# zuds-survey/zuds-pipeline

Hardware: AMD Instinct MI355X
Metric: Mpix/s resample->coadd->subtract, 3072x3072 frames (higher is better)
Workload: dtype f32; 1 GPU; configs[1]+[2]: 32x 3072x3072 TPV frames/GPU, mesh background + weight rescale + Lanczos-3 resample + WEIGHTED coadd (+ AND mask coadd, int16 masks); then 1 science frame/GPU: align ref, hotpants 3x3 regions x 10x10 stamps, r=10, ko=4, subtract; frames_per_gpu=32, size=3072, mask_dtype=int16, combine=WEIGHTED, subtract=True

## Files before the change

### include/zudsmi.h

```cpp
#ifndef ZUDSMI_H
#define ZUDSMI_H

#include <stdint.h>

#ifdef __cplusplus
extern "C" {
#endif

typedef struct zm_ctx zm_ctx;

#define ZM_NPV 40

typedef struct zm_wcs {
    double crpix[2];
    double crval[2];
    double cd[4];
    double pv1[ZM_NPV];
    double pv2[ZM_NPV];
    int32_t naxis[2];
    int32_t flags;
    int32_t pad_;
} zm_wcs;

enum { ZM_RESAMPLE_NEAREST = 0, ZM_RESAMPLE_BILINEAR = 1, ZM_RESAMPLE_LANCZOS3 = 3 };
// ... 130 lines not shown
int zm_aperture_photometry_dev(zm_ctx* ctx, const float* img, const float* rms,
                               const int32_t* mask, int nx, int ny, int npos,
                               const double* x, const double* y, double radius,
                               double* out_flux, double* out_err, int32_t* out_flags);

typedef struct zm_dframe {
    const float* img;
    const float* wgt;
    const void* mask;
    zm_wcs wcs;
    double flxscale;
    int32_t mask_type;
    int32_t pad_;
} zm_dframe;

int zm_coadd_dev(zm_ctx* ctx, int nframes, const zm_dframe* frames,
                 const zm_wcs* wout, const zm_coadd_params* params,
                 int partial, float* out_img, float* out_wgt, int32_t* out_mask,
                 float* out_mask_wgt);
int zm_coadd_finalize_dev(zm_ctx* ctx, float* s1_to_img, const float* s0,
                          int64_t npix);
int zm_mask_accum_dev(zm_ctx* ctx, int32_t* acc, const int32_t* m, int64_t npix,
                      int kind, int first);
int zm_mask_finalize_dev(zm_ctx* ctx, int32_t* acc, float* cov, int64_t npix);
#define ZM_COMM_ID_BYTES 128
typedef struct zm_comm zm_comm;
int zm_comm_unique_id(void* id128);
int zm_comm_init(zm_ctx* ctx, int nranks, int rank, const void* id128, zm_comm** out);
int zm_comm_destroy(zm_comm* comm);
int zm_coadd_reduce_dev(zm_ctx* ctx, zm_comm* comm, float* s1s0, int64_t npix);
int zm_mask_reduce_dev(zm_ctx* ctx, zm_comm* comm, int32_t* mask, int nx, int ny, int kind,
                       float* cov);
#define ZM_COMM_MAX_RANKS 64
typedef struct {
    int32_t world, rank;
    int64_t band_px;
    int64_t my_px;
    int64_t send_off[ZM_COMM_MAX_RANKS];
    int64_t send_cnt[ZM_COMM_MAX_RANKS];
    int64_t recv_off[ZM_COMM_MAX_RANKS];
    int64_t recv_cnt[ZM_COMM_MAX_RANKS];
    int64_t gather_off[ZM_COMM_MAX_RANKS];
} zm_mask_plan;
int zm_comm_band_bounds(int nrows, int world, int32_t* bounds);
int zm_comm_mask_plan(int nx, int ny, int world, int rank, zm_mask_plan* plan);
int zm_resample_stack_dev(zm_ctx* ctx, int nframes, const zm_dframe* frames,
                          const zm_wcs* wout, const zm_coadd_params* params,
                          float* stack, int32_t* out_mask_partial);
int zm_combine_stack_dev(zm_ctx* ctx, int nframes, const float* stack,
                         int64_t frame_stride_px, int64_t npix,
                         const zm_coadd_params* params, float* out_img,
                         float* out_wgt);
int zm_subtract_dev(zm_ctx* ctx, const float* sci, const float* sci_rms,
                    const float* ref, const float* ref_rms, const uint8_t* bpm,
                    int nx, int ny, const zm_hp_params* params, float* out_diff,
                    float* out_rms, zm_hp_info* out_info_host);
int zm_subtract_info(zm_ctx* ctx, zm_hp_info* out_info);
#define ZM_SUB_BATCH_MAX 64
typedef struct zm_sub_job {
    const float* sci;
    const float* sci_rms;
    const float* ref;
    const float* ref_rms;
    const uint8_t* bpm;
    const zm_hp_params* params;
    float* out_diff;
    float* out_rms;
} zm_sub_job;
int zm_subtract_batch_dev(zm_ctx* ctx, int njobs, const zm_sub_job* jobs, int nx, int ny,
                          zm_hp_info* out_info_host);
int zm_subtract_batch(zm_ctx* ctx, int njobs, const zm_sub_job* jobs, int nx, int ny,
                      zm_hp_info* out_info);
int zm_background_dev(zm_ctx* ctx, const float* img, const float* wgt, int nx,
                      int ny, int mesh, int filtersize, float* out_bkg,
                      float* out_rms, float* out_sub, double* out_stats_host);
int zm_resample_dev(zm_ctx* ctx, const float* img, const float* wgt,
                    const int32_t* mask, const zm_wcs* win, const zm_wcs* wout,
                    int kernel, double fscale, float* out_img, float* out_wgt,
                    int32_t* out_mask);

int zm_align_pair_dev(zm_ctx* ctx, const float* img_a, const float* img_b, const int32_t* mask,
                      const zm_wcs* win, const zm_wcs* wout, int kernel, double fscale_a, double fscale_b,
                      float* out_a, float* out_b, int32_t* out_mask);
int zm_resample_i16(zm_ctx* ctx, const float* img, const float* wgt,
                    const int16_t* mask, const zm_wcs* win, const zm_wcs* wout,
                    int kernel, double fscale, float* out_img, float* out_wgt,
                    int32_t* out_mask);
int zm_resample_i16_dev(zm_ctx* ctx, const float* img, const float* wgt,
                        const int16_t* mask, const zm_wcs* win, const zm_wcs* wout,
                        int kernel, double fscale, float* out_img, float* out_wgt,
                        int32_t* out_mask);
int zm_mask_widen_dev(zm_ctx* ctx, const int16_t* in, int64_t n, int32_t* out);

int zm_rms_from_weight_dev(zm_ctx* ctx, const float* wgt, const uint8_t* bad,
                           int64_t n, float big_rms, float* out);
int zm_weight_from_rms_dev(zm_ctx* ctx, const float* rms, const uint8_t* bad,
                           const float* img, float satur, int64_t n, float* out);
int zm_false_weight_dev(zm_ctx* ctx, const void* mask, int mask_type, int32_t badsum, int border,
                        int nx, int ny, float* out_wgt, uint8_t* out_bpm);
int zm_mask_bad_dev(zm_ctx* ctx, const int32_t* a, const int32_t* b,
                    int32_t badsum, int64_t n, int32_t* out_or, uint8_t* out_bpm);
int zm_mask_flag_dev(zm_ctx* ctx, int32_t* mask, const float* img, float value,
                     int32_t bit, int64_t n);
int zm_add_scalar_dev(zm_ctx* ctx, float* img, float v, int64_t n);
int zm_copy_probe_dev(zm_ctx* ctx, const void* src, void* dst, int64_t nbytes);

int zm_find_stars(zm_ctx* ctx, const float* img, const uint8_t* bad, int nx, int ny,
                  float thresh_lo, float thresh_hi, int isolation, int border,
                  int max_out, int* out_x, int* out_y, float* out_peak, int* out_n);
int zm_star_fwhm(zm_ctx* ctx, const float* img, int nx, int ny, int nstar,
                 const int* x, const int* y, int half, double* out_fwhm,
                 double* out_cx, double* out_cy);
int zm_negpix_test(zm_ctx* ctx, const float* img, int nx, int ny, int npos,
                   const double* x, const double* y, double median, double sigma,
                   int32_t* out_bad);
int zm_find_stars_dev(zm_ctx* ctx, const float* img, const uint8_t* bad, int nx, int ny,
                      float thresh_lo, float thresh_hi, int isolation, int border,
                      int max_out, int* out_x, int* out_y, float* out_peak, int* out_n);
int zm_star_fwhm_dev(zm_ctx* ctx, const float* img, int nx, int ny, int nstar,
                     const int* x, const int* y, int half, double* out_fwhm,
                     double* out_cx, double* out_cy);
int zm_candidate_cuts_dev(zm_ctx* ctx, const float* d_img, const float* d_rms, const int32_t* d_mask,
                          int32_t bad_bits, int nx, int ny, int npos, const double* x, const double* y,
                          double* out_bpmcut, double* out_rmscut, int32_t* out_negpix, double* out_stats);

typedef struct zm_extract_params {
    float detect_thresh;
    float satur_level;
    int32_t detect_minarea;
    int32_t filter;
    double aper_radius;
} zm_extract_params;
void zm_extract_params_default(zm_extract_params* p);

#define ZM_EXTRACT_CHAIN 1

typedef struct zm_object {
    int32_t number;
    int32_t npix;
    int32_t xmin, xmax, ymin, ymax;
    int32_t flags;
    int32_t flags_weight;
    int32_t imaflags_iso;
    int32_t first;
    int32_t nthresh;
    int32_t pad_;
    double x_image, y_image;
    double x2, y2, xy;
    double a_image, b_image, theta_image, elongation;
    double fwhm_image;
    double flux_iso, flux_max;
    double peak;
    double flux_aper, fluxerr_aper;
    double x_world, y_world;
} zm_object;

int zm_extract_dev(zm_ctx* ctx, const float* img, const float* sigma, const uint8_t* bad,
                   const int32_t* flag, int nx, int ny, const zm_wcs* wcs,
                   const zm_extract_params* params, int max_objects, zm_object* out_rows,
                   int32_t* segm_dev, float* filtered_dev, int* out_nwritten, int* out_nfound,
                   int* out_status);
int zm_extract(zm_ctx* ctx, const float* img, const float* sigma, const uint8_t* bad,
               const int32_t* flag, int nx, int ny, const zm_wcs* wcs,
               const zm_extract_params* params, int max_objects, zm_object* out_rows,
               int32_t* out_segm, float* out_filtered, int* out_nwritten, int* out_nfound,
               int* out_status);
// ... 113 lines not shown
```

### zuds-pipeline_amd/_lib.py

```python
import ctypes as C
from pathlib import Path

import numpy as np

HERE = Path(__file__).resolve().parent
LIBPATH = HERE / 'lib' / 'libzudsmi.so'

NPV = 40

RESAMPLE = {'NEAREST': 0, 'BILINEAR': 1, 'LANCZOS3': 3}
COMBINE = {'WEIGHTED': 0, 'MEDIAN': 1, 'CLIPPED': 2, 'AVERAGE': 3}
MASKCOMB = {'AND': 0, 'OR': 1}


class ZMError(RuntimeError):
    """A libzudsmi call returned non-zero (message from zm_last_error)."""


class zm_wcs(C.Structure):
    _fields_ = [('crpix', C.c_double * 2), ('crval', C.c_double * 2),
                ('cd', C.c_double * 4), ('pv1', C.c_double * NPV),
                ('pv2', C.c_double * NPV), ('naxis', C.c_int32 * 2),
                ('flags', C.c_int32), ('pad_', C.c_int32)]

# ... 61 lines not shown


class zm_extract_params(C.Structure):
    _fields_ = [('detect_thresh', C.c_float), ('satur_level', C.c_float),
                ('detect_minarea', C.c_int32), ('filter', C.c_int32),
                ('aper_radius', C.c_double)]


class zm_object(C.Structure):
    _fields_ = [('number', C.c_int32), ('npix', C.c_int32), ('xmin', C.c_int32), ('xmax', C.c_int32),
                ('ymin', C.c_int32), ('ymax', C.c_int32), ('flags', C.c_int32), ('flags_weight', C.c_int32),
                ('imaflags_iso', C.c_int32), ('first', C.c_int32), ('nthresh', C.c_int32), ('pad_', C.c_int32),
                ('x_image', C.c_double), ('y_image', C.c_double), ('x2', C.c_double), ('y2', C.c_double),
                ('xy', C.c_double), ('a_image', C.c_double), ('b_image', C.c_double), ('theta_image', C.c_double),
                ('elongation', C.c_double), ('fwhm_image', C.c_double), ('flux_iso', C.c_double),
                ('flux_max', C.c_double), ('peak', C.c_double), ('flux_aper', C.c_double),
                ('fluxerr_aper', C.c_double), ('x_world', C.c_double), ('y_world', C.c_double)]


class zm_measure_params(C.Structure):
    _fields_ = [('kron_fact', C.c_double), ('kron_min_radius', C.c_double), ('filter', C.c_int32), ('pad_', C.c_int32)]


class zm_object_ext(C.Structure):
    _fields_ = [('number', C.c_int32), ('npix_auto', C.c_int32), ('nskip_auto', C.c_int32), ('flags_auto', C.c_int32),
                ('flags_win', C.c_int32), ('niter_win', C.c_int32),
                ('kron_radius', C.c_double), ('flux_auto', C.c_double), ('fluxerr_auto', C.c_double),
                ('mag_auto', C.c_double), ('magerr_auto', C.c_double), ('sigma_win', C.c_double),
                ('xwin_image', C.c_double), ('ywin_image', C.c_double),
                ('x2win', C.c_double), ('y2win', C.c_double), ('xywin', C.c_double),
                ('errx2win', C.c_double), ('erry2win', C.c_double), ('errxywin', C.c_double),
                ('awin_image', C.c_double), ('bwin_image', C.c_double), ('thetawin_image', C.c_double),
                ('errawin_image', C.c_double), ('errbwin_image', C.c_double), ('errthetawin_image', C.c_double),
                ('errx2', C.c_double), ('erry2', C.c_double), ('errxy', C.c_double),
                ('xwin_world', C.c_double), ('ywin_world', C.c_double),
                ('erra_world', C.c_double), ('errb_world', C.c_double), ('errtheta_world', C.c_double)]


class zm_stamp_plane(C.Structure):
    _fields_ = [('img', C.c_void_p), ('wcs', zm_wcs), ('fscale', C.c_double),
                ('on_grid', C.c_int32), ('pad_', C.c_int32)]


class zm_rb_layer(C.Structure):
    _fields_ = [('type', C.c_int32), ('activation', C.c_int32), ('cin', C.c_int32), ('cout', C.c_int32),
                ('pool', C.c_int32), ('ksize', C.c_int32), ('stride', C.c_int32), ('padding', C.c_int32),
                ('w_off', C.c_int64), ('b_off', C.c_int64)]


RB_CHUNK = 128
RB_CONV2D, RB_MAXPOOL, RB_FLATTEN, RB_DENSE = 1, 2, 3, 4
RB_ACTIVATION = {'linear': 0, 'relu': 1, 'sigmoid': 2}
RB_VALID, RB_SAME = 0, 1
STAMP_MAX, STAMP_PLANES_MAX = 256, 8
STAMP_NOT_FINITE, STAMP_NO_OVERLAP = 1, 2
EXTRACT_CHAIN = 1
HP_UNSOLVED, HP_TIMEOUT, HP_PENDING = 1, 2, 4


_P = C.c_void_p
_SIGS = {
    'zm_ctx_create': (C.c_int, [C.c_int, C.POINTER(_P)]),
    'zm_ctx_destroy': (C.c_int, [_P]),
    'zm_ctx_set_stream': (C.c_int, [_P, _P]),
    'zm_ctx_synchronize': (C.c_int, [_P]),
    'zm_ctx_create_on_stream': (C.c_int, [C.c_int, _P, C.POINTER(C.c_void_p)]),
    'zm_ctx_set_share': (C.c_int, [_P, C.c_int]),
    'zm_ctx_query': (C.c_int, [_P, C.c_char_p, C.POINTER(C.c_int64)]),
    'zm_ctx_set_conventions': (C.c_int, [_P, C.c_int, C.c_int]),
    'zm_last_error': (C.c_char_p, []),
    'zm_version': (C.c_char_p, []),
    'zm_autogrid': (C.c_int, [C.c_int, C.POINTER(zm_wcs), C.POINTER(zm_wcs)]),
    'zm_wcs_pix2sky': (C.c_int, [C.POINTER(zm_wcs), C.c_int, _P, _P, _P, _P]),
    'zm_wcs_sky2pix': (C.c_int, [C.POINTER(zm_wcs), C.c_int, _P, _P, _P, _P]),
    'zm_wcs_map': (C.c_int, [C.POINTER(zm_wcs), C.POINTER(zm_wcs), C.c_int,
                             _P, _P, _P, _P]),
    'zm_flux_scale': (C.c_int, [C.POINTER(zm_wcs), C.POINTER(zm_wcs),
                                C.c_double, C.POINTER(C.c_double)]),
    'zm_resample': (C.c_int, [_P, _P, _P, _P, C.POINTER(zm_wcs),
                              C.POINTER(zm_wcs), C.c_int, C.c_double,
                              _P, _P, _P]),
    'zm_align_pair_dev': (C.c_int, [_P, _P, _P, _P, C.POINTER(zm_wcs), C.POINTER(zm_wcs), C.c_int, C.c_double,
                                    C.c_double, _P, _P, _P]),
    'zm_resample_dev': (C.c_int, [_P, _P, _P, _P, C.POINTER(zm_wcs),
                                  C.POINTER(zm_wcs), C.c_int, C.c_double,
                                  _P, _P, _P]),
    'zm_resample_i16': (C.c_int, [_P, _P, _P, _P, C.POINTER(zm_wcs),
                                  C.POINTER(zm_wcs), C.c_int, C.c_double,
                                  _P, _P, _P]),
    'zm_resample_i16_dev': (C.c_int, [_P, _P, _P, _P, C.POINTER(zm_wcs),
                                      C.POINTER(zm_wcs), C.c_int, C.c_double,
                                      _P, _P, _P]),
    'zm_mask_widen_dev': (C.c_int, [_P, _P, C.c_int64, _P]),
    'zm_coadd_params_default': (None, [C.POINTER(zm_coadd_params)]),
    'zm_coadd': (C.c_int, [_P, C.c_int, C.POINTER(zm_frame), C.POINTER(zm_wcs),
                           C.POINTER(zm_coadd_params), _P, _P, _P, _P]),
    'zm_coadd_dev': (C.c_int, [_P, C.c_int, C.POINTER(zm_frame),
                               C.POINTER(zm_wcs), C.POINTER(zm_coadd_params),
                               C.c_int, _P, _P, _P, _P]),
    'zm_coadd_finalize_dev': (C.c_int, [_P, _P, _P, C.c_int64]),
    'zm_resample_stack_dev': (C.c_int, [_P, C.c_int, C.POINTER(zm_frame),
                                        C.POINTER(zm_wcs),
                                        C.POINTER(zm_coadd_params), _P, _P]),
    'zm_combine_stack_dev': (C.c_int, [_P, C.c_int, _P, C.c_int64, C.c_int64,
                                       C.POINTER(zm_coadd_params), _P, _P]),
    'zm_background': (C.c_int, [_P, _P, _P, C.c_int, C.c_int, C.c_int, C.c_int,
                                _P, _P, _P, _P]),
    'zm_background_dev': (C.c_int, [_P, _P, _P, C.c_int, C.c_int, C.c_int,
                                    C.c_int, _P, _P, _P, _P]),
    'zm_hp_params_default': (None, [C.POINTER(zm_hp_params)]),
    'zm_subtract': (C.c_int, [_P, _P, _P, _P, _P, _P, C.c_int, C.c_int,
                              C.POINTER(zm_hp_params), _P, _P,
                              C.POINTER(zm_hp_info)]),
    'zm_subtract_dev': (C.c_int, [_P, _P, _P, _P, _P, _P, C.c_int, C.c_int,
                                  C.POINTER(zm_hp_params), _P, _P,
                                  C.POINTER(zm_hp_info)]),
    'zm_subtract_info': (C.c_int, [_P, C.POINTER(zm_hp_info)]),
    'zm_subtract_batch_dev': (C.c_int, [_P, C.c_int, C.POINTER(zm_sub_job), C.c_int, C.c_int,
                                        C.POINTER(zm_hp_info)]),
    'zm_subtract_batch': (C.c_int, [_P, C.c_int, C.POINTER(zm_sub_job), C.c_int, C.c_int,
                                    C.POINTER(zm_hp_info)]),
    'zm_median_mad': (C.c_int, [_P, _P, _P, C.c_int64, C.POINTER(C.c_double),
                                C.POINTER(C.c_double)]),
    'zm_median_mad_dev': (C.c_int, [_P, _P, _P, C.c_int64, C.POINTER(C.c_double),
                                    C.POINTER(C.c_double)]),
    'zm_find_stars': (C.c_int, [_P, _P, _P, C.c_int, C.c_int, C.c_float, C.c_float, C.c_int, C.c_int,
                                C.c_int, _P, _P, _P, C.POINTER(C.c_int)]),
    'zm_star_fwhm': (C.c_int, [_P, _P, C.c_int, C.c_int, C.c_int, _P, _P, C.c_int, _P, _P, _P]),
    'zm_find_stars_dev': (C.c_int, [_P, _P, _P, C.c_int, C.c_int, C.c_float, C.c_float, C.c_int, C.c_int,
                                    C.c_int, _P, _P, _P, C.POINTER(C.c_int)]),
    'zm_star_fwhm_dev': (C.c_int, [_P, _P, C.c_int, C.c_int, C.c_int, _P, _P, C.c_int, _P, _P, _P]),
    'zm_negpix_test': (C.c_int, [_P, _P, C.c_int, C.c_int, C.c_int, _P, _P, C.c_double, C.c_double, _P]),
    'zm_candidate_cuts_dev': (C.c_int, [_P, _P, _P, _P, C.c_int32, C.c_int, C.c_int, C.c_int, _P, _P, _P, _P, _P, _P]),
    'zm_fits_decode_dev': (C.c_int, [_P, _P, C.c_int, C.c_double, C.c_double, C.c_int64, C.c_int, _P]),
    'zm_fits_encode_dev': (C.c_int, [_P, _P, C.c_int, C.c_int64, _P]),
    'zm_mask_accum_dev': (C.c_int, [_P, _P, _P, C.c_int64, C.c_int, C.c_int]),
    'zm_mask_finalize_dev': (C.c_int, [_P, _P, _P, C.c_int64]),
    'zm_comm_unique_id': (C.c_int, [_P]),
    'zm_comm_init': (C.c_int, [_P, C.c_int, C.c_int, _P, C.POINTER(C.c_void_p)]),
    'zm_comm_destroy': (C.c_int, [_P]),
    'zm_coadd_reduce_dev': (C.c_int, [_P, _P, _P, C.c_int64]),
    'zm_mask_reduce_dev': (C.c_int, [_P, _P, _P, C.c_int, C.c_int, C.c_int, _P]),
    'zm_comm_band_bounds': (C.c_int, [C.c_int, C.c_int, _P]),
    'zm_comm_mask_plan': (C.c_int, [C.c_int, C.c_int, C.c_int, C.c_int, C.POINTER(zm_mask_plan)]),
    'zm_median_mad2_dev': (C.c_int, [_P, _P, _P, _P, _P, C.c_int64, C.POINTER(C.c_double)]),
    'zm_median_mad2_async_dev': (C.c_int, [_P, _P, _P, _P, _P, C.c_int64, _P]),
    'zm_rms_from_weight_dev': (C.c_int, [_P, _P, _P, C.c_int64, C.c_float, _P]),
    'zm_weight_from_rms_dev': (C.c_int, [_P, _P, _P, _P, C.c_float, C.c_int64, _P]),
    'zm_false_weight_dev': (C.c_int, [_P, _P, C.c_int, C.c_int32, C.c_int, C.c_int, C.c_int, _P, _P]),
    'zm_mask_bad_dev': (C.c_int, [_P, _P, _P, C.c_int32, C.c_int64, _P, _P]),
    'zm_mask_flag_dev': (C.c_int, [_P, _P, _P, C.c_float, C.c_int32, C.c_int64]),
    'zm_add_scalar_dev': (C.c_int, [_P, _P, C.c_float, C.c_int64]),
    'zm_copy_probe_dev': (C.c_int, [_P, _P, _P, C.c_int64]),
    'zm_aperture_photometry': (C.c_int, [_P, _P, _P, _P, C.c_int, C.c_int, C.c_int, _P, _P,
                                         C.c_double, _P, _P, _P]),
    'zm_aperture_photometry_dev': (C.c_int, [_P, _P, _P, _P, C.c_int, C.c_int, C.c_int, _P, _P,
                                             C.c_double, _P, _P, _P]),
    'zm_extract_params_default': (None, [C.POINTER(zm_extract_params)]),
    'zm_extract_dev': (C.c_int, [_P, _P, _P, _P, _P, C.c_int, C.c_int, C.POINTER(zm_wcs), C.POINTER(zm_extract_params),
                                 C.c_int, _P, _P, _P, C.POINTER(C.c_int), C.POINTER(C.c_int), C.POINTER(C.c_int)]),
    'zm_extract': (C.c_int, [_P, _P, _P, _P, _P, C.c_int, C.c_int, C.POINTER(zm_wcs), C.POINTER(zm_extract_params),
                             C.c_int, _P, _P, _P, C.POINTER(C.c_int), C.POINTER(C.c_int), C.POINTER(C.c_int)]),
    'zm_measure_params_default': (None, [C.POINTER(zm_measure_params)]),
    'zm_extract_measure_dev': (C.c_int, [_P, _P, _P, _P, _P, C.c_int, C.c_int, C.POINTER(zm_wcs),
                                         C.POINTER(zm_measure_params), C.c_int, _P, _P]),
    'zm_extract_measure': (C.c_int, [_P, _P, _P, _P, _P, C.c_int, C.c_int, C.POINTER(zm_wcs),
                                     C.POINTER(zm_measure_params), C.c_int, _P, _P]),
    'zm_stamp_origin': (C.c_int, [C.POINTER(zm_wcs), C.c_int, _P, _P, C.c_int, _P, _P, _P]),
    'zm_stamps_dev': (C.c_int, [_P, C.c_int, C.POINTER(zm_stamp_plane), C.POINTER(zm_wcs), C.c_int, C.c_int, _P, _P,
                                C.c_int, _P, _P]),
    'zm_stamps': (C.c_int, [_P, C.c_int, C.POINTER(zm_stamp_plane), C.POINTER(zm_wcs), C.c_int, C.c_int, _P, _P,
                            C.c_int, _P, _P]),
    'zm_rb_model_create': (C.c_int, [_P, C.c_int, C.c_int, C.c_int, C.POINTER(zm_rb_layer), _P, C.c_int64, C.POINTER(C.c_void_p)]),
    'zm_rb_model_destroy': (C.c_int, [_P]),
    'zm_rb_score_dev': (C.c_int, [_P, _P, C.c_int, _P, _P, C.c_int, _P, _P]),
    'zm_rb_score': (C.c_int, [_P, _P, C.c_int, _P, _P, C.c_int, _P, _P]),
    'zm_associate_dev': (C.c_int, [_P, C.c_int, _P, _P, _P, _P, C.c_double, _P, _P, _P, _P, _P, _P, _P]),
    'zm_associate': (C.c_int, [_P, C.c_int, _P, _P, _P, _P, C.c_double, _P, _P, _P, _P, _P, _P, _P]),
    'zm_crossmatch_dev': (C.c_int, [_P, C.c_int, _P, _P, C.c_int, _P, _P, C.c_double, _P, _P]),
    'zm_crossmatch': (C.c_int, [_P, C.c_int, _P, _P, C.c_int, _P, _P, C.c_double, _P, _P]),
    'zm_assoc_stats': (C.c_int, [_P, _P]),
    'zm_timing_enable': (C.c_int, [_P, C.c_int]),
    'zm_timing_filter': (C.c_int, [_P, C.c_char_p]),
    'zm_timing_reset': (C.c_int, [_P]),
    'zm_timing_read': (C.c_int, [_P, C.c_char_p, C.POINTER(C.c_double),
                                 C.POINTER(C.c_int64)]),
    'zm_debug_lanczos3': (None, [C.c_float, _P]),
}

_lib = None


def exported_symbols():
    return [k for k in _SIGS if k != 'zm_debug_lanczos3']


def _one_hip_runtime():
    import importlib.util
    import os
    import sys
    if 'torch' in sys.modules:
        return
    try:
        spec = importlib.util.find_spec('torch')
    except (ImportError, ValueError):
        spec = None
    if not spec or not spec.origin:
        return
    if not os.environ.get('ZM_NO_TORCH'):
        try:
            import torch
            return
        except Exception:
            pass
    d = os.path.join(os.path.dirname(spec.origin), 'lib')
    for name in ('libhsa-runtime64.so', 'libamdhip64.so'):
        p = os.path.join(d, name)
        if os.path.exists(p):
            try:
                C.CDLL(p, mode=C.RTLD_GLOBAL)
            except OSError:
                return


def lib():
    global _lib
    if _lib is not None:
        return _lib
    _one_hip_runtime()
    if not LIBPATH.exists():
        raise ZMError(f'{LIBPATH} is missing: run __graft_entry__.build() '
                      f'(python zuds-pipeline_amd/build.py). There is no CPU '
                      f'fallback for this path.')
    L = C.CDLL(str(LIBPATH))
    for name, (res, args) in _SIGS.items():
        try:
            fn = getattr(L, name)
        except AttributeError:
            raise ZMError(f'{LIBPATH} does not export {name}; rebuild it '
                          f'(python zuds-pipeline_amd/build.py --force)')
        fn.restype = res
        fn.argtypes = args
    _lib = L
    return L


def check(rc, what=''):
    if rc != 0:
        msg = lib().zm_last_error().decode('utf-8', 'replace')
        raise ZMError(f'{what}: {msg} (rc={rc})' if what else f'{msg} (rc={rc})')


def ptr(a):
    if a is None:
        return None
    if isinstance(a, int):
        return a
    return a.ctypes.data


def as_f32(a):
    return None if a is None else np.ascontiguousarray(a, dtype=np.float32)


def as_i32(a):
    return None if a is None else np.ascontiguousarray(a, dtype=np.int32)


def as_mask(a):
    if a is None:
        return None, MASKTYPE_I32
    a = np.asarray(a)
    if a.dtype == np.int16:
        return np.ascontiguousarray(a), MASKTYPE_I16
    return np.ascontiguousarray(a, dtype=np.int32), MASKTYPE_I32


# ... 19 lines not shown
```

### zuds-pipeline_amd/csrc/api_coadd.hip

```cpp
#include <algorithm>
#include <cmath>
#include <cstdlib>

#include "zm_internal.h"
#include "wcs_math.h"

extern "C" void zm_coadd_params_default(zm_coadd_params* p) {
    if (!p) return;
    memset(p, 0, sizeof(*p));
    p->combine = ZM_COMBINE_CLIPPED;
    p->mask_combine = ZM_MASK_AND;
    p->resample = ZM_RESAMPLE_LANCZOS3;
    p->subtract_back = 1;
    p->back_size = 128;
    p->back_filtersize = 3;
    p->rescale_weights = 1;
    p->clip_sigma = 4.0;
    p->clip_ampfrac = 0.3;
    p->weight_thresh = 1e-30;
}

static int check_wcs(const zm_wcs* w, const char* what) {
    ZM_CHECK(w != nullptr, "%s: WCS is NULL", what);
    ZM_CHECK(w->naxis[0] > 0 && w->naxis[1] > 0, "%s: NAXIS must be positive (got %d x %d)", what,
// ... 372 lines not shown
                                    const zm_coadd_params* params, float* out_img,
                                    float* out_wgt) {
    ZM_CHECK(ctx && stack && params && out_img && out_wgt, "zm_combine_stack_dev: null argument");
    ZM_HIP(hipSetDevice(ctx->device));
    return zm_launch_combine(ctx, nframes, (const float2*)stack, frame_stride_px, npix,
                             params->combine, (float)params->clip_sigma,
                             (float)params->clip_ampfrac, out_img, out_wgt, 0);
}

extern "C" int zm_coadd_dev(zm_ctx* ctx, int nframes, const zm_dframe* frames,
                            const zm_wcs* wout, const zm_coadd_params* params, int partial,
                            float* out_img, float* out_wgt, int32_t* out_mask,
                            float* out_mask_wgt) {
    ZM_CHECK(ctx && frames && wout && params && out_img && out_wgt, "zm_coadd_dev: null argument");
    ZM_CHECK(nframes >= 1, "zm_coadd_dev: need at least one frame");
    ZM_HIP(hipSetDevice(ctx->device));
    ZM_TRY(check_wcs(wout, "output grid"));
    const int64_t opix = (int64_t)wout->naxis[0] * wout->naxis[1];
    if (fused_ok(ctx, params))
        return coadd_fused(ctx, nframes, frames, wout, params, partial, out_img, out_wgt, out_mask, out_mask_wgt);
    float2* stack = nullptr;
    ZM_TRY(ctx->get("stack", sizeof(float2) * (size_t)opix * nframes, (void**)&stack));
    ZM_TRY(resample_frames(ctx, nframes, frames, wout, params, stack, out_mask, -1,
                           params->mask_combine));
    ZM_TRY(zm_launch_combine(ctx, nframes, stack, opix, opix, params->combine,
                             (float)params->clip_sigma, (float)params->clip_ampfrac, out_img,
                             out_wgt, partial));
    if (out_mask && !partial) ZM_TRY(zm_launch_mask_finalize(ctx, out_mask, out_mask_wgt, opix));
    return 0;
}

extern "C" int zm_mask_accum_dev(zm_ctx* ctx, int32_t* acc, const int32_t* m, int64_t npix, int kind,
                                 int first) {
    ZM_CHECK(ctx && acc && m, "zm_mask_accum_dev: null argument");
    ZM_CHECK(kind == ZM_MASK_AND || kind == ZM_MASK_OR, "zm_mask_accum_dev: unknown combine %d", kind);
    ZM_HIP(hipSetDevice(ctx->device));
    return zm_launch_mask_accum(ctx, acc, m, npix, kind, first);
}

extern "C" int zm_mask_finalize_dev(zm_ctx* ctx, int32_t* acc, float* cov, int64_t npix) {
    ZM_CHECK(ctx && acc, "zm_mask_finalize_dev: null argument");
    ZM_HIP(hipSetDevice(ctx->device));
    return zm_launch_mask_finalize(ctx, acc, cov, npix);
}

extern "C" int zm_resample_dev(zm_ctx* ctx, const float* img, const float* wgt,
                               const int32_t* mask, const zm_wcs* win, const zm_wcs* wout,
                               int kernel, double fscale, float* out_img, float* out_wgt,
                               int32_t* out_mask) {
    ZM_CHECK(ctx && win && wout, "zm_resample_dev: null argument");
    ZM_CHECK(img || mask, "zm_resample_dev: need an image or a mask");
    ZM_CHECK(!img || (out_img && out_wgt), "zm_resample_dev: out_img/out_wgt required");
    ZM_CHECK(!mask || out_mask, "zm_resample_dev: out_mask required");
    ZM_HIP(hipSetDevice(ctx->device));
    ZM_TRY(check_wcs(win, "input frame"));
    ZM_TRY(check_wcs(wout, "output grid"));
    ZM_CHECK(kernel == ZM_RESAMPLE_LANCZOS3 || kernel == ZM_RESAMPLE_BILINEAR ||
             kernel == ZM_RESAMPLE_NEAREST, "zm_resample_dev: unknown RESAMPLING_TYPE %d", kernel);
    const int onx = wout->naxis[0], ony = wout->naxis[1];
    const int nx = win->naxis[0], ny = win->naxis[1];
    const int64_t opix = (int64_t)onx * ony;
    const int lnx = (onx - 1) / ZM_LATTICE_STEP + 2, lny = (ony - 1) / ZM_LATTICE_STEP + 2;
    zm_map_params mp_host;
    zm_make_map(wout, win, &mp_host);
    int lds = std::min(plan_lds(&mp_host, onx, ony, ntaps_of(kernel)), 8000);
    double2* lat = nullptr;
    ZM_TRY(ctx->get("lattice", sizeof(double2) * (size_t)lnx * lny, (void**)&lat));
    ZM_TRY(zm_launch_lattice(ctx, &mp_host, lnx, lny, lat));
    if (img) {
        const int spitch = (nx + 1) & ~1;
        float2 *src = nullptr, *dst = nullptr;
        ZM_TRY(ctx->get("prep", sizeof(float2) * (size_t)spitch * ny, (void**)&src));
        ZM_TRY(ctx->get("stack", sizeof(float2) * (size_t)opix, (void**)&dst));
        ZM_TRY(zm_launch_prep(ctx, img, wgt, nx, ny, nullptr, 0, 0, 0, nullptr, 1e-30f, src, spitch));
        ZM_TRY(zm_launch_resample(ctx, src, nx, ny, spitch, lat, lnx, lny, kernel, (float)fscale,
                                  dst, onx, ony, lds, mask, out_mask, mask ? 1 : 0, 0, 1, out_img, out_wgt));
    } else if (mask) {
        ZM_TRY(zm_launch_resample_mask(ctx, mask, nx, ny, lat, lnx, lny, kernel, out_mask, onx,
                                       ony, 0));
    }
    return 0;
}

extern "C" int zm_align_pair_dev(zm_ctx* ctx, const float* img_a, const float* img_b, const int32_t* mask,
                                 const zm_wcs* win, const zm_wcs* wout, int kernel, double fscale_a, double fscale_b,
                                 float* out_a, float* out_b, int32_t* out_mask) {
    ZM_CHECK(ctx && img_a && img_b && win && wout && out_a && out_b, "zm_align_pair_dev: null argument");
    ZM_CHECK(!mask || out_mask, "zm_align_pair_dev: out_mask required");
    ZM_CHECK(kernel == ZM_RESAMPLE_LANCZOS3 || kernel == ZM_RESAMPLE_BILINEAR, "zm_align_pair_dev: LANCZOS3 or BILINEAR (got %d)", kernel);
    ZM_CHECK(fscale_b != 0.0, "zm_align_pair_dev: fscale_b must not be 0");
    ZM_CHECK(ctx->edge == ZM_EDGE_ZERO && ctx->mask_resample == ZM_MASKRES_OR, "zm_align_pair_dev: default conventions only");
    ZM_HIP(hipSetDevice(ctx->device));
    ZM_TRY(check_wcs(win, "input frame"));
    ZM_TRY(check_wcs(wout, "output grid"));
    const int onx = wout->naxis[0], ony = wout->naxis[1];
    const int nx = win->naxis[0], ny = win->naxis[1];
    const int lnx = (onx - 1) / ZM_LATTICE_STEP + 2, lny = (ony - 1) / ZM_LATTICE_STEP + 2;
    zm_map_params mp_host;
    zm_make_map(wout, win, &mp_host);
    const int lds = std::min(plan_lds(&mp_host, onx, ony, ntaps_of(kernel)), 8000);
    double2* lat = nullptr;
    ZM_TRY(ctx->get("lattice", sizeof(double2) * (size_t)lnx * lny, (void**)&lat));
    ZM_TRY(zm_launch_lattice(ctx, &mp_host, lnx, lny, lat));
    const int spitch = (nx + 1) & ~1;
    float2* src = nullptr;
    ZM_TRY(ctx->get("prep", sizeof(float2) * (size_t)spitch * ny, (void**)&src));
    ZM_TRY(zm_launch_prep_pair(ctx, img_a, img_b, nx, ny, src, spitch));
    return zm_launch_resample(ctx, src, nx, ny, spitch, lat, lnx, lny, kernel, (float)fscale_a, nullptr, onx, ony, lds,
                              mask, out_mask, mask ? 1 : 0, 0, 1, out_a, out_b, (float)fscale_b);
}

extern "C" int zm_resample_i16_dev(zm_ctx* ctx, const float* img, const float* wgt, const int16_t* mask,
                                   const zm_wcs* win, const zm_wcs* wout, int kernel, double fscale,
                                   float* out_img, float* out_wgt, int32_t* out_mask) {
    ZM_CHECK(ctx && win && wout, "zm_resample_i16_dev: null argument");
    ZM_HIP(hipSetDevice(ctx->device));
    int32_t* w = nullptr;
    if (mask) {
        ZM_TRY(check_wcs(win, "input frame"));
        const int64_t n = (int64_t)win->naxis[0] * win->naxis[1];
        ZM_TRY(ctx->get("mask_widen", sizeof(int32_t) * (size_t)n, (void**)&w));
        ZM_TRY(zm_launch_mask_widen(ctx, mask, n, w));
    }
    return zm_resample_dev(ctx, img, wgt, w, win, wout, kernel, fscale, out_img, out_wgt, out_mask);
}

static int resample_host(zm_ctx* ctx, const float* img, const float* wgt, const void* mask, int mask_type,
                         const zm_wcs* win, const zm_wcs* wout, int kernel, double fscale,
                         float* out_img, float* out_wgt, int32_t* out_mask);
extern "C" int zm_resample(zm_ctx* ctx, const float* img, const float* wgt, const int32_t* mask,
                           const zm_wcs* win, const zm_wcs* wout, int kernel, double fscale,
                           float* out_img, float* out_wgt, int32_t* out_mask) {
    return resample_host(ctx, img, wgt, mask, ZM_MASKTYPE_I32, win, wout, kernel, fscale, out_img, out_wgt, out_mask);
}
extern "C" int zm_resample_i16(zm_ctx* ctx, const float* img, const float* wgt, const int16_t* mask,
                               const zm_wcs* win, const zm_wcs* wout, int kernel, double fscale,
                               float* out_img, float* out_wgt, int32_t* out_mask) {
    return resample_host(ctx, img, wgt, mask, ZM_MASKTYPE_I16, win, wout, kernel, fscale, out_img, out_wgt, out_mask);
}
static int resample_host(zm_ctx* ctx, const float* img, const float* wgt, const void* mask, int mask_type,
                         const zm_wcs* win, const zm_wcs* wout, int kernel, double fscale,
                         float* out_img, float* out_wgt, int32_t* out_mask) {
    ZM_CHECK(ctx && win && wout, "zm_resample: null argument");
    ZM_HIP(hipSetDevice(ctx->device));
    ZM_TRY(check_wcs(win, "input frame"));
    ZM_TRY(check_wcs(wout, "output grid"));
    const size_t ipix = (size_t)win->naxis[0] * win->naxis[1];
    const size_t opix = (size_t)wout->naxis[0] * wout->naxis[1];
    const size_t mb = mask_type == ZM_MASKTYPE_I16 ? 2 : 4;
    float *d_img = nullptr, *d_wgt = nullptr, *d_oimg = nullptr, *d_owgt = nullptr;
    void* d_mask = nullptr;
    int32_t* d_omask = nullptr;
    if (img) {
        ZM_TRY(ctx->get("h_img", ipix * 4, (void**)&d_img));
        ZM_HIP(hipMemcpyAsync(d_img, img, ipix * 4, hipMemcpyHostToDevice, ctx->stream));
        if (wgt) {
            ZM_TRY(ctx->get("h_wgt", ipix * 4, (void**)&d_wgt));
            ZM_HIP(hipMemcpyAsync(d_wgt, wgt, ipix * 4, hipMemcpyHostToDevice, ctx->stream));
        }
        ZM_TRY(ctx->get("h_oimg", opix * 4, (void**)&d_oimg));
        ZM_TRY(ctx->get("h_owgt", opix * 4, (void**)&d_owgt));
    }
    if (mask) {
        ZM_TRY(ctx->get("h_mask", ipix * mb, &d_mask));
        ZM_HIP(hipMemcpyAsync(d_mask, mask, ipix * mb, hipMemcpyHostToDevice, ctx->stream));
        ZM_TRY(ctx->get("h_omask", opix * 4, (void**)&d_omask));
    }
    if (mask_type == ZM_MASKTYPE_I16)
        ZM_TRY(zm_resample_i16_dev(ctx, d_img, d_wgt, (const int16_t*)d_mask, win, wout, kernel, fscale, d_oimg,
                                   d_owgt, d_omask));
    else
        ZM_TRY(zm_resample_dev(ctx, d_img, d_wgt, (const int32_t*)d_mask, win, wout, kernel, fscale, d_oimg, d_owgt,
                               d_omask));
    if (img) {
        ZM_HIP(hipMemcpyAsync(out_img, d_oimg, opix * 4, hipMemcpyDeviceToHost, ctx->stream));
        ZM_HIP(hipMemcpyAsync(out_wgt, d_owgt, opix * 4, hipMemcpyDeviceToHost, ctx->stream));
    }
    if (mask)
        ZM_HIP(hipMemcpyAsync(out_mask, d_omask, opix * 4, hipMemcpyDeviceToHost, ctx->stream));
    ZM_HIP(hipStreamSynchronize(ctx->stream));
    return 0;
}

extern "C" int zm_coadd(zm_ctx* ctx, int nframes, const zm_frame* frames, const zm_wcs* wout,
                        const zm_coadd_params* params, float* out_img, float* out_wgt,
                        int32_t* out_mask, float* out_mask_wgt) {
    ZM_CHECK(ctx && frames && wout && params && out_img && out_wgt, "zm_coadd: null argument");
    ZM_CHECK(nframes >= 1, "zm_coadd: need at least one frame");
    ZM_HIP(hipSetDevice(ctx->device));
    ZM_TRY(check_wcs(wout, "output grid"));
    std::vector<zm_dframe> df(nframes);
    size_t total = 0;
// ... 55 lines not shown
```

### zuds-pipeline_amd/csrc/ctx.hip

```cpp
#include <cstdarg>

#include "zm_internal.h"

static thread_local char g_err[1024] = "";

void zm_set_error(const char* fmt, ...) {
    va_list ap;
    va_start(ap, fmt);
    vsnprintf(g_err, sizeof(g_err), fmt, ap);
    va_end(ap);
}

extern "C" const char* zm_last_error(void) { return g_err; }
extern "C" const char* zm_version(void) { return "zudsmi 0.1.0 (gfx950)"; }

int zm_ctx::get(const char* name, size_t bytes, void** out) {
    auto it = scratch.find(name);
    if (it != scratch.end() && it->second.second >= bytes) {
        *out = it->second.first;
        return 0;
    }
    if (it != scratch.end()) {
        ZM_HIP(hipStreamSynchronize(stream));
        ZM_HIP(hipFree(it->second.first));
// ... 59 lines not shown
    ZM_HIP(hipSetDevice(device));
    zm_ctx* c = new zm_ctx();
    c->device = device;
    ZM_HIP(hipStreamCreateWithFlags(&c->stream, hipStreamNonBlocking));
    c->own_stream = true;
    *out = c;
    return 0;
}

extern "C" int zm_ctx_create_on_stream(int device, void* hip_stream, zm_ctx** out) {
    ZM_CHECK(out != nullptr && hip_stream != nullptr, "zm_ctx_create_on_stream: null argument");
    int ndev = 0;
    hipError_t e = hipGetDeviceCount(&ndev);
    if (e != hipSuccess || ndev == 0) {
        zm_set_error("zm_ctx_create_on_stream: no HIP device available (%s)",
                     e != hipSuccess ? hipGetErrorString(e) : "device count 0");
        return 3;
    }
    ZM_CHECK(device >= 0 && device < ndev, "zm_ctx_create_on_stream: device %d out of range [0,%d)", device, ndev);
    ZM_HIP(hipSetDevice(device));
    zm_ctx* c = new zm_ctx();
    c->device = device;
    c->stream = (hipStream_t)hip_stream;
    c->own_stream = false;
    *out = c;
    return 0;
}

extern "C" int zm_ctx_destroy(zm_ctx* ctx) {
    if (!ctx) return 0;
    (void)hipSetDevice(ctx->device);
    (void)hipStreamSynchronize(ctx->stream);
    ctx->release_all();
    if (ctx->aux) { (void)hipStreamSynchronize(ctx->aux); (void)hipStreamDestroy(ctx->aux); }
    if (ctx->own_stream && ctx->stream) (void)hipStreamDestroy(ctx->stream);
    delete ctx;
    return 0;
}

extern "C" int zm_ctx_set_stream(zm_ctx* ctx, void* hip_stream) {
    ZM_CHECK(ctx != nullptr, "zm_ctx_set_stream: ctx is NULL");
    ZM_HIP(hipSetDevice(ctx->device));
    if (ZM_DEVENV("ZM_SET_STREAM_SYNC")) ZM_HIP(hipStreamSynchronize(ctx->stream));
    if (hip_stream != nullptr && (hipStream_t)hip_stream == ctx->stream) return 0;
    if (hip_stream == nullptr && ctx->own_stream) return 0;
    hipStream_t old = ctx->stream, next = (hipStream_t)hip_stream;
    const bool old_owned = ctx->own_stream;
    if (next == nullptr) ZM_HIP(hipStreamCreateWithFlags(&next, hipStreamNonBlocking));
    if (old) {
        hipEvent_t* ev = nullptr;
        ZM_TRY(zm_get_sync_events(ctx, 11, &ev));
        ZM_HIP(hipEventRecord(ev[10], old));
        ZM_HIP(hipStreamWaitEvent(next, ev[10], 0));
    }
    if (old_owned && old) ZM_HIP(hipStreamDestroy(old));
    ctx->stream = next;
    ctx->own_stream = hip_stream == nullptr;
    return 0;
}

extern "C" int zm_ctx_set_share(zm_ctx* ctx, int nctx) {
    ZM_CHECK(ctx != nullptr, "zm_ctx_set_share: ctx is NULL");
    ZM_CHECK(nctx >= 1 && nctx <= 64, "zm_ctx_set_share: %d contexts (1 .. 64)", nctx);
    ctx->share = nctx;
    return 0;
}

extern "C" int zm_ctx_set_conventions(zm_ctx* ctx, int edge, int mask_resample) {
    ZM_CHECK(ctx != nullptr, "zm_ctx_set_conventions: ctx is NULL");
    ZM_CHECK(edge == ZM_EDGE_ZERO || edge == ZM_EDGE_TRUNCATE, "zm_ctx_set_conventions: unknown edge rule %d", edge);
    ZM_CHECK(mask_resample == ZM_MASKRES_OR || mask_resample == ZM_MASKRES_LANCZOS_ROUND,
             "zm_ctx_set_conventions: unknown mask rule %d", mask_resample);
    ctx->edge = edge;
    ctx->mask_resample = mask_resample;
    return 0;
}

extern "C" int zm_ctx_query(zm_ctx* ctx, const char* what, int64_t* out) {
    ZM_CHECK(ctx && what && out, "zm_ctx_query: null argument");
    if (!strcmp(what, "fused_form")) *out = ctx->ff_last_form;
    else if (!strcmp(what, "dev_build")) *out = ZM_DEV_BUILD;
    else if (!strcmp(what, "edge")) *out = ctx->edge;
    else if (!strcmp(what, "mask_resample")) *out = ctx->mask_resample;
    else ZM_CHECK(false, "zm_ctx_query: unknown item \"%s\"", what);
    return 0;
}

hipStream_t zm_ctx_aux(zm_ctx* ctx) {
    if (!ctx->aux) {
        (void)hipSetDevice(ctx->device);
        if (hipStreamCreateWithFlags(&ctx->aux, hipStreamNonBlocking) != hipSuccess) ctx->aux = nullptr;
    }
    return ctx->aux;
}

int zm_get_sync_events(zm_ctx* ctx, int n, hipEvent_t** out) {
    while ((int)ctx->sync_events.size() < n) {
        hipEvent_t e = nullptr;
        ZM_HIP(hipEventCreateWithFlags(&e, hipEventDisableTiming));
        ctx->sync_events.push_back(e);
    }
    *out = ctx->sync_events.data();
    return 0;
}

extern "C" int zm_ctx_synchronize(zm_ctx* ctx) {
    ZM_CHECK(ctx != nullptr, "zm_ctx_synchronize: ctx is NULL");
    ZM_HIP(hipSetDevice(ctx->device));
    ZM_HIP(hipStreamSynchronize(ctx->stream));
    return 0;
}

zm_scope_timer::zm_scope_timer(zm_ctx* c, const char* n) : ctx(c), name(n) {
    if (!ctx->timing) return;
    if (!ctx->timing_only.empty() && ctx->timing_only != n) return;
    auto take = [&]() -> hipEvent_t {
        if (!ctx->event_pool.empty()) {
            hipEvent_t e = ctx->event_pool.back();
            ctx->event_pool.pop_back();
            return e;
        }
        hipEvent_t e = nullptr;
        (void)hipEventCreate(&e);
        return e;
    };
    a = take();
    b = take();
    (void)hipEventRecord(a, ctx->stream);
}

zm_scope_timer::~zm_scope_timer() {
    if (!ctx->timing || !a) return;
    (void)hipEventRecord(b, ctx->stream);
    ctx->timers[name].pending.push_back({a, b});
}

extern "C" int zm_timing_enable(zm_ctx* ctx, int on) {
    ZM_CHECK(ctx != nullptr, "zm_timing_enable: ctx is NULL");
    ctx->timing = on != 0;
    return 0;
}

static int drain(zm_ctx* ctx, zm_timer_slot& s) {
    for (auto& p : s.pending) {
        ZM_HIP(hipEventSynchronize(p.second));
        float ms = 0.f;
        ZM_HIP(hipEventElapsedTime(&ms, p.first, p.second));
        s.total_ms += ms;
        s.launches += 1;
        ctx->event_pool.push_back(p.first);
        ctx->event_pool.push_back(p.second);
    }
    s.pending.clear();
    return 0;
}

extern "C" int zm_timing_filter(zm_ctx* ctx, const char* only_or_null) {
    ZM_CHECK(ctx != nullptr, "zm_timing_filter: ctx is NULL");
    ctx->timing_only = only_or_null ? only_or_null : "";
    return 0;
}

extern "C" int zm_timing_reset(zm_ctx* ctx) {
    ZM_CHECK(ctx != nullptr, "zm_timing_reset: ctx is NULL");
    for (auto& kv : ctx->timers) {
        ZM_TRY(drain(ctx, kv.second));
// ... 21 lines not shown
```

### zuds-pipeline_amd/csrc/hotpants.hip

```cpp
#include "hp_dev.h"
#include <sched.h>
#include "chol_diag.h"

__global__ void k_hp_valid(const float* __restrict__ sci, const float* __restrict__ ref,
                           const uint8_t* __restrict__ bpm, int64_t n, float il, float iu,
                           float tl, float tu, uint8_t* __restrict__ bad,
                           const double* __restrict__ lim, double nsig) {
    int64_t p = (int64_t)blockIdx.x * blockDim.x + threadIdx.x;
    if (lim) {
        il = (float)(lim[0] - nsig * lim[1]);
        tl = (float)(lim[3] - nsig * lim[4]);
    }
    if (p >= n) return;
    float s = sci[p], t = ref[p];
    bool ok = (s == s) && (t == t) && fabsf(s) < 3e38f && fabsf(t) < 3e38f;
    ok = ok && s >= il && s <= iu && t >= tl && t <= tu;
    if (bpm) ok = ok && bpm[p] == 0;
    bad[p] = ok ? 0 : 1;
}

#define HP_ROWMAX 16384
__global__ __launch_bounds__(256) void k_hp_rowany(const uint8_t* __restrict__ in, int nx, int ny, int hw,
                                                   uint8_t* __restrict__ out) {
    extern __shared__ int ra_pre[];
// ... 24 lines not shown
        out[(size_t)y * nx + x] = (ra_pre[b + 1] - ra_pre[a]) > 0;
    }
}

__global__ __launch_bounds__(256) void k_hp_valid_rows(const float* __restrict__ sci, const float* __restrict__ ref,
                                                       const uint8_t* __restrict__ bpm, int nx, int ny, float il, float iu,
                                                       float tl, float tu, const double* __restrict__ lim, double nsig,
                                                       int hw1, int hw2, uint8_t* __restrict__ bad,
                                                       uint8_t* __restrict__ out1, uint8_t* __restrict__ out2) {
    extern __shared__ int ra_pre[];
    __shared__ int wsum[HP_ROWMAX / 64], wtot[4];
    if (lim) {
        il = (float)(lim[0] - nsig * lim[1]);
        tl = (float)(lim[3] - nsig * lim[4]);
    }
    const int y = blockIdx.x, tid = threadIdx.x;
    const size_t r0 = (size_t)y * nx;
    const int lane = tid & 63, wave = tid >> 6;
    const int nch = (nx + 255) / 256;
    for (int c = 0; c < nch; ++c) {
        const int x = 256 * c + tid;
        bool b = false;
        if (x < nx) {
            const float s = sci[r0 + x], t = ref[r0 + x];
            bool ok = (s == s) && (t == t) && fabsf(s) < 3e38f && fabsf(t) < 3e38f;
            ok = ok && s >= il && s <= iu && t >= tl && t <= tu;
            if (bpm) ok = ok && bpm[r0 + x] == 0;
            b = !ok;
            bad[r0 + x] = b ? 1 : 0;
        }
        const unsigned long long m = __ballot(b);
        if (x < nx) ra_pre[x + 1] = __popcll(m & ((2ull << lane) - 1ull));
        if (lane == 0) wsum[4 * c + wave] = __popcll(m);
    }
    if (tid == 0) ra_pre[0] = 0;
    __syncthreads();
    {
        const int v = tid < 4 * nch ? wsum[tid] : 0;
        int inc = v;
#pragma unroll
        for (int o = 1; o < 64; o <<= 1) {
            const int t = __shfl_up(inc, o);
            if (lane >= o) inc += t;
        }
        if (lane == 63) wtot[wave] = inc;
        __syncthreads();
        int off = inc - v;
        for (int w = 0; w < wave; ++w) off += wtot[w];
        if (tid < 4 * nch) wsum[tid] = off;
    }
    __syncthreads();
    for (int c = 0; c < nch; ++c) {
        const int x = 256 * c + tid;
        if (x < nx) ra_pre[x + 1] += wsum[4 * c + wave];
    }
    __syncthreads();
    for (int x = tid; x < nx; x += 256) {
        const int a1 = max(x - hw1, 0), b1 = min(x + hw1, nx - 1);
        const int a2 = max(x - hw2, 0), b2 = min(x + hw2, nx - 1);
        out1[r0 + x] = (ra_pre[b1 + 1] - ra_pre[a1]) > 0;
        out2[r0 + x] = (ra_pre[b2 + 1] - ra_pre[a2]) > 0;
    }
}

#define HP_COLSTRIP 96
__global__ __launch_bounds__(256) void k_hp_colany(const uint8_t* __restrict__ in, int nx, int ny, int hw,
                                                   int edge, uint8_t* __restrict__ out) {
    const int x = blockIdx.x * blockDim.x + threadIdx.x;
    const int y0 = blockIdx.y * HP_COLSTRIP, y1 = min(y0 + HP_COLSTRIP, ny);
    if (x >= nx) return;
    int cnt = 0;
    for (int j = max(y0 - hw, 0); j <= min(y0 + hw, ny - 1); ++j) cnt += in[(size_t)j * nx + x] ? 1 : 0;
    for (int y = y0; y < y1; ++y) {
        uint8_t v = cnt > 0;
        if (edge && (x < hw || x >= nx - hw || y < hw || y >= ny - hw)) v = 1;
        out[(size_t)y * nx + x] = v;
        const int add = y + 1 + hw, sub = y - hw;
        if (add < ny) cnt += in[(size_t)add * nx + x] ? 1 : 0;
        if (sub >= 0) cnt -= in[(size_t)sub * nx + x] ? 1 : 0;
    }
}

#define HP_COLSTRIP4 32
__global__ __launch_bounds__(256) void k_hp_colany4(const uint8_t* __restrict__ in, int nx, int ny, int hw,
                                                    int edge, uint8_t* __restrict__ out) {
    const int x = (blockIdx.x * blockDim.x + threadIdx.x) * 4;
    const int y0 = blockIdx.y * HP_COLSTRIP4, y1 = min(y0 + HP_COLSTRIP4, ny);
    if (x >= nx) return;
    const unsigned* in4 = reinterpret_cast<const unsigned*>(in + x);
    const size_t pitch = (size_t)nx / 4;
    auto nz = [](unsigned w, int k) -> int { return ((w >> (8 * k)) & 0xffu) ? 1 : 0; };
    int cnt[4] = {0, 0, 0, 0};
    {
        const int j0 = max(y0 - hw, 0), j1 = min(y0 + hw, ny - 1);
        for (int jb = j0; jb <= j1; jb += 8) {
            unsigned w[8];
#pragma unroll
            for (int u = 0; u < 8; ++u) w[u] = (jb + u <= j1) ? in4[(size_t)(jb + u) * pitch] : 0u;
#pragma unroll
            for (int u = 0; u < 8; ++u)
#pragma unroll
                for (int k = 0; k < 4; ++k) cnt[k] += nz(w[u], k);
        }
    }
    for (int yb = y0; yb < y1; yb += 8) {
        unsigned wa[8], ws[8];
#pragma unroll
        for (int u = 0; u < 8; ++u) {
            const int add = yb + u + 1 + hw, sub = yb + u - hw;
            wa[u] = (add < ny) ? in4[(size_t)add * pitch] : 0u;
            ws[u] = (sub >= 0) ? in4[(size_t)sub * pitch] : 0u;
        }
#pragma unroll
        for (int u = 0; u < 8; ++u) {
            const int y = yb + u;
            if (y < y1) {
                unsigned o = 0;
#pragma unroll
                for (int k = 0; k < 4; ++k) {
                    unsigned v = cnt[k] > 0;
                    if (edge && (x + k < hw || x + k >= nx - hw || y < hw || y >= ny - hw)) v = 1;
                    o |= v << (8 * k);
                }
                *reinterpret_cast<unsigned*>(out + (size_t)y * nx + x) = o;
            }
#pragma unroll
            for (int k = 0; k < 4; ++k) cnt[k] += nz(wa[u], k) - nz(ws[u], k);
        }
    }
}

__global__ __launch_bounds__(256) void k_hp_cells(const hp_plan P, const float* __restrict__ ref,
                                                  const uint8_t* __restrict__ bad,
                                                  const uint8_t* __restrict__ dirty,
                                                  int2* __restrict__ centres) {
    __shared__ double red[4];
    __shared__ float bval[4];
    __shared__ int bidx[4];
    __shared__ int2 chosen[HP_MAXNSS];
    const int cell = blockIdx.x, tid = threadIdx.x;
    const int r = cell / P.ncellr, c = cell - r * P.ncellr;
    const int sy = c / P.nsx, sx = c - sy * P.nsx;
    const int cw = (P.rx1[r] - P.rx0[r]) / P.nsx, ch = (P.ry1[r] - P.ry0[r]) / P.nsy;
    const int cx0 = P.rx0[r] + sx * cw, cy0 = P.ry0[r] + sy * ch;
    const int n = cw * ch;
    double m = 0.0, s = 0.0;
    for (int pass = 0; pass < 4; ++pass) {
        double s0 = 0, s1 = 0;
        for (int k = tid; k < n; k += 256) {
            int yy = k / cw, xx = k - yy * cw;
            size_t idx = (size_t)(cy0 + yy) * P.nx + cx0 + xx;
            if (bad[idx]) continue;
            double v = ref[idx];
            if (pass == 0 || fabs(v - m) <= 3.0 * s) { s0 += 1.0; s1 += v; }
        }
        s0 = block_sum256(s0, red);
        s1 = block_sum256(s1, red);
        if (s0 < 1.0) break;
        double mn = s1 / s0;
        double s2 = 0;
        for (int k = tid; k < n; k += 256) {
            int yy = k / cw, xx = k - yy * cw;
            size_t idx = (size_t)(cy0 + yy) * P.nx + cx0 + xx;
            if (bad[idx]) continue;
            double v = ref[idx];
            if (pass == 0 || fabs(v - m) <= 3.0 * s) s2 += (v - mn) * (v - mn);
        }
        s2 = block_sum256(s2, red);
// ... 2016 lines not shown
    if (guard && *guard == 0) return;
    const int reg = blockIdx.y % nreg;
    if (HPJ_REGION_IDLE(J, round, reg, ncell, ncellr)) return;
    const double* __restrict__ dd = J.dsc + (size_t)reg * n;
    const double* __restrict__ A0 = J.A0 + (size_t)reg * (size_t)(n + 1) * n;
    const double* __restrict__ rhs0 = J.rhs0 + (size_t)reg * n;
    double* __restrict__ A = J.A + (size_t)reg * (size_t)(n + 1) * lda;
#pragma unroll 1
    for (int k = 0; k < HSB_ROWS; ++k) {
        const int c1 = blockIdx.x * HSB_ROWS + k;
        if (c1 >= n) break;
        const double r1 = 1.0 / dd[c1];
        for (int c2 = threadIdx.x; c2 <= c1; c2 += 256) {
            const double r2 = 1.0 / dd[c2];
            double v = __dmul_rn(A0[(size_t)c1 * n + c2], __dmul_rn(r1, r2));
            if (c1 == c2) v = __dadd_rn(v, HP_RIDGE);
            A[(size_t)c1 * lda + c2] = v;
        }
        if (threadIdx.x == 0) A[(size_t)n * lda + c1] = __dmul_rn(rhs0[c1], r1);
    }
}

__global__ __launch_bounds__(CT_THREADS) void k_chol_tp(int n, int lda, int ldt, double* Aall, double* ATall, int* fail,
                                                        long long* prof, const int* __restrict__ guard) {
    chol_tp_body(n, lda, ldt, Aall, ATall, fail, prof, guard);
}
__global__ __launch_bounds__(CT_THREADS) void k_chol_tp_b(int n, int lda, int ldt, const hp_job* __restrict__ jobs, int round,
                                                          int ncell, int ncellr) {
    const hp_job& J = jobs[blockIdx.z];
    if (HPJ_REGION_IDLE(J, round, (int)blockIdx.x, ncell, ncellr)) return;
    chol_tp_body(n, lda, ldt, J.A, J.AT, HPJ_FAIL(J), nullptr, HPJ_GUARD(J, round));
}

__global__ __launch_bounds__(CBC_THREADS) void k_chol_back_cols(int n, int lda, const double* __restrict__ Aall,
                                                                const double* __restrict__ dall,
                                                                double* __restrict__ xall, const int* __restrict__ guard) {
    chol_back_cols_body(n, lda, Aall, dall, xall, guard);
}
__global__ __launch_bounds__(CBC_THREADS) void k_chol_back_cols_b(int n, int lda, const hp_job* __restrict__ jobs, int round,
                                                                  int ncell, int ncellr) {
    const hp_job& J = jobs[blockIdx.z];
    if (HPJ_REGION_IDLE(J, round, (int)blockIdx.x, ncell, ncellr)) return;
    chol_back_cols_body(n, lda, J.A, J.dsc, J.rhs, HPJ_GUARD(J, round));
}

__global__ __launch_bounds__(64) void k_hp_merit(const hp_plan P, const double* __restrict__ G,
                                                 const double* __restrict__ phi, const double* __restrict__ vbar,
                                                 const int* __restrict__ active, const double* __restrict__ xsol,
                                                 double* __restrict__ merit, const int* __restrict__ guard,
                                                 int* __restrict__ needlist) {
    hp_merit_body(P, G, phi, vbar, active, xsol, merit, guard, needlist);
}
__global__ __launch_bounds__(64) void k_hp_merit_b(const hp_plan P, const hp_job* __restrict__ jobs, int round) {
    const hp_job& J = jobs[blockIdx.z];
    hp_merit_body(P, J.G, J.phi, J.vbar, J.active, J.rhs, J.merit, HPJ_GUARD(J, round), J.needlist);
}

__global__ __launch_bounds__(64) void k_hp_reject_wave(const hp_plan P, const double* __restrict__ merit,
                                                       const int2* __restrict__ centres, int* __restrict__ active,
                                                       int* __restrict__ need, int* __restrict__ chg,
                                                       int* __restrict__ nrej, double* __restrict__ stats,
                                                       const int* __restrict__ guard, int* __restrict__ round_flag,
                                                       int* __restrict__ needlist, const int* __restrict__ tmo,
                                                       const hp_sig sig) {
    hp_reject_wave_body(P, merit, centres, active, need, chg, nrej, stats, guard, round_flag, needlist, tmo);
    hp_round_signal(sig, round_flag, gridDim.x);
}
__global__ __launch_bounds__(64) void k_hp_reject_wave_b(const hp_plan P, const hp_job* __restrict__ jobs, int round) {
    const hp_job& J = jobs[blockIdx.z];
    hp_reject_wave_body(P, J.merit, J.centres, J.active, J.need, J.chg, HPJ_NREJ(J), J.stats, HPJ_GUARD(J, round),
                        J.rflags + round, J.needlist);
}

__global__ void k_hp_flag(int32_t* __restrict__ mask, const float* __restrict__ img, float value, int32_t bit,
                          int64_t n, const int* __restrict__ tmo, int nreg) {
    int gaveup = 0;
    for (int r = 0; r < nreg; ++r) gaveup |= tmo[r];
    if (gaveup) return;
    int64_t p = (int64_t)blockIdx.x * blockDim.x + threadIdx.x;
    if (p >= n) return;
    if (img[p] == value) mask[p] |= bit;
}

extern "C" void zm_hp_params_default(zm_hp_params* p) {
    if (!p) return;
    memset(p, 0, sizeof(*p));
    p->tu = 5e3; p->tl = 0.0; p->iu = 5e3; p->il = 0.0;
    p->r = 10.0; p->rss = 15.0;
    p->fin = sqrt(50000.0); p->fi = 1e-30;
    p->nsx = p->nsy = 10; p->nrx = p->nry = 1;
    p->ko = 4; p->bgo = 0; p->nss = 3; p->normalize = 0;
    p->ft = 20.0; p->ks = 2.0;
    p->ngauss = 3;
    p->deg[0] = 6; p->deg[1] = 4; p->deg[2] = 2;
    p->sigma[0] = 0.7; p->sigma[1] = 1.5; p->sigma[2] = 3.0;
    p->limits_dev = nullptr; p->limits_nsigma = 10.0;
}

static int make_plan(const zm_hp_params* hp, int nx, int ny, hp_plan* P, std::vector<double>* filt,
                     std::vector<double>* basis) {
    memset(P, 0, sizeof(*P));
    P->nx = nx; P->ny = ny;
    P->hwk = (int)hp->r; P->hwss = (int)hp->rss;
    ZM_CHECK(P->hwk >= 1 && P->hwk <= HP_MAX_HWK, "zm_subtract: kernel half width int(r) = %d outside [1, %d]", P->hwk, HP_MAX_HWK);
    ZM_CHECK(P->hwss >= 1 && P->hwss <= HP_MAX_HWSS, "zm_subtract: substamp half width int(rss) = %d outside [1, %d]", P->hwss, HP_MAX_HWSS);
    P->hw = P->hwk + P->hwss;
    P->step = 2 * P->hwk + 1; P->sw = 2 * P->hwss + 1; P->pw = 2 * P->hw + 1;
    P->npix = P->sw * P->sw;
    P->npixp = (P->npix + GR_KT - 1) / GR_KT * GR_KT;
    ZM_CHECK(hp->ngauss >= 1 && hp->ngauss <= 4, "zm_subtract: ngauss %d outside [1, 4]", hp->ngauss);
    ZM_CHECK(hp->ko >= 0 && hp->ko <= 6, "zm_subtract: -ko %d outside [0, 6]", hp->ko);
    ZM_CHECK(hp->bgo >= 0 && hp->bgo <= 3, "zm_subtract: -bgo %d outside [0, 3]", hp->bgo);
    ZM_CHECK(hp->nss >= 1 && hp->nss <= HP_MAXNSS, "zm_subtract: nss %d outside [1, %d]", hp->nss, HP_MAXNSS);
    ZM_CHECK(hp->nrx >= 1 && hp->nry >= 1 && hp->nrx * hp->nry <= HP_MAXREG, "zm_subtract: bad -nrx/-nry");
    ZM_CHECK(hp->nsx >= 1 && hp->nsy >= 1 && hp->nsx * hp->nsy <= 4096, "zm_subtract: bad -nsx/-nsy");
    P->ko = hp->ko; P->bgo = hp->bgo; P->nss = hp->nss; P->normalize = hp->normalize;
    P->nrx = hp->nrx; P->nry = hp->nry; P->nsx = hp->nsx; P->nsy = hp->nsy;
    P->nreg = hp->nrx * hp->nry; P->ncellr = hp->nsx * hp->nsy; P->ncell = P->nreg * P->ncellr;
    P->tu = hp->tu; P->tl = hp->tl; P->iu = hp->iu; P->il = hp->il; P->ft = hp->ft; P->ks = hp->ks;
    P->fi = (float)hp->fi; P->fin = (float)hp->fin;
    ZM_CHECK(nx / hp->nrx / hp->nsx >= 1 && ny / hp->nry / hp->nsy >= 1, "zm_subtract: stamps smaller than a pixel");
    for (int ry = 0; ry < hp->nry; ++ry)
        for (int rx = 0; rx < hp->nrx; ++rx) {
            int r = ry * hp->nrx + rx;
            P->rx0[r] = rx * (nx / hp->nrx);
            P->rx1[r] = rx == hp->nrx - 1 ? nx : (rx + 1) * (nx / hp->nrx);
            P->ry0[r] = ry * (ny / hp->nry);
            P->ry1[r] = ry == hp->nry - 1 ? ny : (ry + 1) * (ny / hp->nry);
        }
    const int step = P->step, hwk = P->hwk;
    std::vector<int> fidx;
    int nf1 = 0, nc = 0;
    std::vector<double> fsum;
    filt->clear();
    int base[4] = {0, 0, 0, 0};
    for (int g = 0; g < hp->ngauss; ++g) {
        ZM_CHECK(hp->deg[g] >= 0 && hp->deg[g] <= 8 && hp->sigma[g] > 0, "zm_subtract: bad basis");
        base[g] = nf1;
        P->gdeg[g] = hp->deg[g];
        P->gbase[g] = nf1;
        for (int a = 0; a <= hp->deg[g]; ++a) {
            double s = 0.0;
            for (int u = -hwk; u <= hwk; ++u) {
                double v = exp(-(double)u * u / (2.0 * hp->sigma[g] * hp->sigma[g])) * pow((double)u, (double)a);
                filt->push_back(v);
                s += v;
            }
            fsum.push_back(s);
            ++nf1;
        }
    }
    ZM_CHECK(nf1 <= HP_MAXF1, "zm_subtract: too many 1-D filters");
    P->nf1 = nf1;
    P->ngauss = hp->ngauss;
    for (int g = 0; g < hp->ngauss; ++g)
        for (int a = 0; a <= hp->deg[g]; ++a)
            for (int b = 0; b <= hp->deg[g] - a; ++b) {
                ZM_CHECK(nc < HP_MAXX, "zm_subtract: basis too large");
                if (a == 0 && b == 0) P->gterm0[g] = nc;
                P->tfx[nc] = base[g] + a;
                P->tfy[nc] = base[g] + b;
                bool ee = (a % 2 == 0) && (b % 2 == 0);
                P->tscale[nc] = ee ? 1.0 / (fsum[base[g] + a] * fsum[base[g] + b]) : 1.0;
                P->tsub0[nc] = (ee && nc > 0) ? 1 : 0;
                ++nc;
            }
    P->nc = nc;
    for (int f = 0; f < HP_MAXF1; ++f) { P->tf0[f] = 0; P->tfn[f] = 0; }
    for (int n = 0; n < nc; ++n) {
        const int f = P->tfx[n];
        if (P->tfn[f] == 0) P->tf0[f] = n;
        P->tfn[f] += 1;
    }
    int nkp = 0;
    for (int i = 0; i <= P->ko; ++i)
        for (int j = 0; j <= P->ko - i; ++j) { P->kpi[nkp] = i; P->kpj[nkp] = j; ++nkp; }
    P->nkp = nkp;
    int nbg = 0;
    for (int i = 0; i <= P->bgo; ++i)
        for (int j = 0; j <= P->bgo - i; ++j) { P->bpi[nbg] = i; P->bpj[nbg] = j; ++nbg; }
    P->nbg = nbg;
    P->nE = nc + nbg;
    P->nX = P->nE + 1;
    ZM_CHECK(P->nX <= HP_MAXX, "zm_subtract: %d basis + %d background terms exceed the %d-row Gram tile", nc, nbg, HP_MAXX);
    P->nunk = 1 + (nc - 1) * nkp + nbg;
    basis->assign((size_t)nc * step * step, 0.0);
    for (int n = 0; n < nc; ++n) {
        const double* fx = filt->data() + (size_t)P->tfx[n] * step;
        const double* fy = filt->data() + (size_t)P->tfy[n] * step;
        for (int v = 0; v < step; ++v)
            for (int u = 0; u < step; ++u) {
                double k = fy[v] * fx[u] * P->tscale[n];
                if (P->tsub0[n]) k -= (*basis)[(size_t)v * step + u];
                (*basis)[((size_t)n * step + v) * step + u] = k;
            }
    }
    return 0;
}

static __device__ __forceinline__ void hp_solved_body(int nreg, int nunk, const double* __restrict__ stats, const int* __restrict__ fail,
                            const int* __restrict__ tmo, const double* __restrict__ x,
                            unsigned long long* __restrict__ mask, double* __restrict__ x0out = nullptr) {
    unsigned long long m = 0;
    const int reg = threadIdx.x;
    if (reg < nreg) {
        const double x0 = x[(size_t)reg * nunk];
        if (x0out) x0out[reg] = x0;
        const bool ok = stats[2 * reg + 1] >= 1.0 && fail[reg] == 0 && tmo[reg] == 0 && isfinite(x0);
        m = ok ? 1ull << reg : 0ull;
    }
#pragma unroll
    for (int o = 32; o >= 1; o >>= 1) m |= __shfl_xor(m, o);
    if (threadIdx.x == 0) *mask = m;
}
__global__ void k_hp_solved(int nreg, int nunk, const double* __restrict__ stats, const int* __restrict__ fail,
                            const int* __restrict__ tmo, const double* __restrict__ x,
                            unsigned long long* __restrict__ mask, double* __restrict__ x0out = nullptr) {
    hp_solved_body(nreg, nunk, stats, fail, tmo, x, mask, x0out);
}


static int hp_launch_masks(zm_ctx* ctx, const hp_plan& P, const zm_hp_params* hp, const float* sci, const float* ref,
                           const uint8_t* bpm, uint8_t* bad, uint8_t* tmp8, uint8_t* dirty, uint8_t* outbad) {
    const int nx = P.nx, ny = P.ny;
    const int64_t np = (int64_t)nx * ny;
    hipStream_t st = ctx->stream;
    const dim3 b256(256);
    zm_scope_timer t(ctx, "hp_masks");
    ZM_CHECK(nx <= HP_ROWMAX, "zm_subtract: frames wider than %d pixels are not supported", HP_ROWMAX);
    const size_t rsh = sizeof(int) * ((size_t)nx + 1);
    dim3 gc(zm_div_up(nx, 256), zm_div_up(ny, HP_COLSTRIP));
    if (!ctx->hp_rset && rsh > 65536) {
        ZM_HIP(hipFuncSetAttribute((const void*)k_hp_rowany, hipFuncAttributeMaxDynamicSharedMemorySize,
                                   (int)(sizeof(int) * (HP_ROWMAX + 1))));
        ZM_HIP(hipFuncSetAttribute((const void*)k_hp_valid_rows, hipFuncAttributeMaxDynamicSharedMemorySize,
                                   (int)(sizeof(int) * (HP_ROWMAX + 1))));
        ctx->hp_rset = true;
    }
    const bool col4 = (nx % 4 == 0) && (((uintptr_t)tmp8 | (uintptr_t)dirty | (uintptr_t)outbad) & 3) == 0;
    dim3 gc4(zm_div_up(nx / 4, 256), zm_div_up(ny, HP_COLSTRIP4));
    static const bool split = ZM_DEVENV("ZM_HP_MASKS") && !strcmp(ZM_DEVENV("ZM_HP_MASKS"), "split");
    uint8_t* tmp8b = nullptr;
    if (!split) ZM_TRY(ctx->get("hp_tmp8b", np, (void**)&tmp8b));
    if (!split && (((uintptr_t)tmp8b & 3) == 0)) {
        hipLaunchKernelGGL(k_hp_valid_rows, dim3(ny), b256, rsh, st, sci, ref, bpm, nx, ny, (float)P.il, (float)P.iu,
                           (float)P.tl, (float)P.tu, hp->limits_dev, hp->limits_nsigma, P.hw, P.hwk, bad, tmp8, tmp8b);
        if (col4) {
            hipLaunchKernelGGL(k_hp_colany4, gc4, b256, 0, st, tmp8, nx, ny, P.hw, 1, dirty);
            hipLaunchKernelGGL(k_hp_colany4, gc4, b256, 0, st, tmp8b, nx, ny, P.hwk, 1, outbad);
        } else {
            hipLaunchKernelGGL(k_hp_colany, gc, b256, 0, st, tmp8, nx, ny, P.hw, 1, dirty);
            hipLaunchKernelGGL(k_hp_colany, gc, b256, 0, st, tmp8b, nx, ny, P.hwk, 1, outbad);
        }
    } else {
        hipLaunchKernelGGL(k_hp_valid, dim3((unsigned)((np + 255) / 256)), b256, 0, st, sci, ref, bpm, np,
                           (float)P.il, (float)P.iu, (float)P.tl, (float)P.tu, bad, hp->limits_dev, hp->limits_nsigma);
        hipLaunchKernelGGL(k_hp_rowany, dim3(ny), b256, rsh, st, bad, nx, ny, P.hw, tmp8);
        if (col4) hipLaunchKernelGGL(k_hp_colany4, gc4, b256, 0, st, tmp8, nx, ny, P.hw, 1, dirty);
        else hipLaunchKernelGGL(k_hp_colany, gc, b256, 0, st, tmp8, nx, ny, P.hw, 1, dirty);
        hipLaunchKernelGGL(k_hp_rowany, dim3(ny), b256, rsh, st, bad, nx, ny, P.hwk, tmp8);
        if (col4) hipLaunchKernelGGL(k_hp_colany4, gc4, b256, 0, st, tmp8, nx, ny, P.hwk, 1, outbad);
        else hipLaunchKernelGGL(k_hp_colany, gc, b256, 0, st, tmp8, nx, ny, P.hwk, 1, outbad);
    }
    ZM_HIP(hipGetLastError());
    return 0;
}

static int hp_launch_cells(zm_ctx* ctx, const hp_plan& P, const float* ref, const uint8_t* bad, const uint8_t* dirty,
                           int2* centres, int* active, int* need, int* ntotal) {
    hipStream_t st = ctx->stream;
    const dim3 b256(256);
    zm_scope_timer t(ctx, "hp_cells");
    int maxcell = 0;
    for (int r = 0; r < P.nreg; ++r)
        maxcell = std::max(maxcell, ((P.rx1[r] - P.rx0[r]) / P.nsx) * ((P.ry1[r] - P.ry0[r]) / P.nsy));
    const char* cf = getenv("ZM_CELLS_FORM");
    if (maxcell <= HC_THREADS * HC_PX && !(cf && !strcmp(cf, "global")))
        hipLaunchKernelGGL(k_hp_cells_reg, dim3(P.ncell), dim3(HC_THREADS), 0, st, P, ref, bad, dirty, centres);
    else
        hipLaunchKernelGGL(k_hp_cells, dim3(P.ncell), b256, 0, st, P, ref, bad, dirty, centres);
    hipLaunchKernelGGL(k_hp_init_active, dim3(zm_div_up(P.ncell, 256)), b256, 0, st, P, centres, active, need, ntotal);
    ZM_HIP(hipGetLastError());
    return 0;
}

static std::atomic<int> g_hp_fitting[64];
struct hp_fit_guard {
    std::atomic<int>* c;
    int others;
    explicit hp_fit_guard(std::atomic<int>* cc) : c(cc), others(cc->fetch_add(1)) {}
    bool shared() const { return c && (others > 0 || c->load(std::memory_order_relaxed) > 1); }
    void release() { if (c) c->fetch_sub(1); c = nullptr; }
    ~hp_fit_guard() { release(); }
};

#define HP_NIBUF_ (4 * HP_MAXREG + 4)
#define HP_SUMBYTES_ (sizeof(int) * HP_NIBUF_ + sizeof(double) * 3 * HP_MAXREG)
static void hp_fill_info(const char* h_sum, int nreg, int nunk, int rounds, int retries, zm_hp_info* info) {
    const int* h_int = reinterpret_cast<const int*>(h_sum);
    const double* h_stats = reinterpret_cast<const double*>(h_sum + sizeof(int) * HP_NIBUF_);
    const double* h_x0 = h_stats + 2 * HP_MAXREG;
    auto reg_solved = [&](int reg) {
        return h_stats[2 * reg + 1] >= 1.0 && h_int[2 * HP_MAXREG + reg] == 0 &&
               h_int[3 * HP_MAXREG + 4 + reg] == 0 && std::isfinite(h_x0[reg]);
    };
    memset(info, 0, sizeof(*info));
    double ks = 0, chi = 0;
    int nsolved = 0;
    for (int r = 0; r < nreg; ++r) {
        info->nstamps_total += h_int[HP_MAXREG + r];
        info->nstamps_used += (int)h_stats[2 * r + 1];
        if (reg_solved(r)) {
            ks += h_x0[r];
            chi += h_stats[2 * r];
            ++nsolved;
        }
    }
    info->niter = rounds;
    info->ncoeff = nunk;
    info->kernel_sum = nsolved ? ks / nsolved : 0.0;
    info->chi2 = nsolved ? chi / nsolved : 0.0;
    info->nmasked = h_int[3 * HP_MAXREG];
    info->status = (nsolved == nreg ? 0 : ZM_HP_UNSOLVED);
    info->nunsolved = nreg - nsolved;
    info->retries = retries;
}

extern "C" int zm_subtract_dev(zm_ctx* ctx, const float* sci, const float* sci_rms, const float* ref,
                               const float* ref_rms, const uint8_t* bpm, int nx, int ny,
                               const zm_hp_params* hp, float* out_diff, float* out_rms,
                               zm_hp_info* info) {
    ZM_CHECK(ctx && sci && sci_rms && ref && ref_rms && hp && out_diff && out_rms,
             "zm_subtract_dev: null argument");
    ZM_CHECK(nx > 0 && ny > 0, "zm_subtract_dev: empty image");
    ZM_HIP(hipSetDevice(ctx->device));
    hp_plan P;
    std::vector<double> filt, basis;
    ZM_TRY(make_plan(hp, nx, ny, &P, &filt, &basis));
    ZM_CHECK(nx > 2 * P.hw + 1 && ny > 2 * P.hw + 1, "zm_subtract_dev: image smaller than a substamp");
    const int64_t np = (int64_t)nx * ny;
    hipStream_t st = ctx->stream;

    uint8_t *bad = nullptr, *tmp8 = nullptr, *dirty = nullptr, *outbad = nullptr;
    ZM_TRY(ctx->get("hp_bad", np, (void**)&bad));
// ... 246 lines not shown
                        fprintf(stderr, "chol wg %3d:", wg);
                        for (int k = 0; k < nprof; ++k)
                            fprintf(stderr, " %s %.1f us", df ? nm8[k] : nm6[k], hp[(size_t)wg * nprof + k] * 0.01);
                        fprintf(stderr, "\n");
                    }
                    if (df && ZM_DEVENV("ZM_CHOL_PROF") && atoi(ZM_DEVENV("ZM_CHOL_PROF")) >= 2) {
                        const long long* ts = hp.data() + (size_t)8 * P.nreg * W;
                        for (int kb = 0; kb < nblkp; ++kb) {
                            fprintf(stderr, "chol kb %2d:", kb);
                            for (int e = 0; e < 6; ++e) fprintf(stderr, " %7.2f", (ts[kb * 8 + e] - ts[0]) * 0.01);
                            fprintf(stderr, "\n");
                        }
                    }
                }
                }
            }
            {
                const size_t bsh = sizeof(double) * (((size_t)P.nunk + 1) & ~(size_t)1) +
                                   sizeof(double) * CH_NB * (CH_NB + 1);
                if (!ctx->hp_bset && bsh > 65536) {
                    ZM_HIP(hipFuncSetAttribute((const void*)k_chol_back,
                                               hipFuncAttributeMaxDynamicSharedMemorySize, 160 * 1024 - 64));
                    ctx->hp_bset = true;
                }
                ZM_CHECK(bsh <= 160 * 1024 - 64, "zm_subtract: %d unknowns exceed the solver's LDS", P.nunk);
                if (P.nunk <= CBC_COLS)
                    hipLaunchKernelGGL(k_chol_back_cols, dim3(P.nreg), dim3(CBC_THREADS), 0, st, P.nunk, lda, A, dsc, rhs, guard);
                else
                    hipLaunchKernelGGL(k_chol_back, dim3(P.nreg), dim3(1024), bsh, st, P.nunk, lda, A, dsc, rhs, guard);
            }
            hipLaunchKernelGGL(k_hp_merit, dim3(P.ncell), dim3(64), 0, st, P, G, phi, vbar, active, rhs, merit, guard, needlist);
            const hp_sig sig = sig_off ? hp_sig{nullptr, nullptr, 0u} : hp_sig{rflags + 16 + rounds, ctx->hp_sig_d + rounds, seq};
            if (P.ncellr <= 256)
                hipLaunchKernelGGL(k_hp_reject_wave, dim3(P.nreg), dim3(64), 0, st, P, merit, centres, active, need,
                                   chg, nrej, stats, guard, rflags + rounds, needlist, (const int*)tmo, sig);
            else
                hipLaunchKernelGGL(k_hp_reject, dim3(P.nreg), b256, 0, st, P, merit, centres, active, need, chg,
                                   nrej, stats, guard, rflags + rounds, needlist, (const int*)tmo, sig);
            ZM_HIP(hipGetLastError());
        }
        if (sig_off) {
            ZM_HIP(hipMemcpyAsync(h_rflags + rounds, rflags + rounds, sizeof(int), hipMemcpyDeviceToHost, st));
            ZM_HIP(hipEventRecord(evs[1 + (rounds & 1)], st));
        }
        return 0;
    };
    auto wait_round = [&](int r, int* flag) -> int {
        if (sig_off) {
            ZM_HIP(hipEventSynchronize(evs[1 + (r & 1)]));
            *flag = h_rflags[r];
            return 0;
        }
        for (unsigned long spins = 1;; ++spins) {
            const unsigned long long w = __atomic_load_n(&ctx->hp_sig_h[r], __ATOMIC_ACQUIRE);
            if ((unsigned)(w >> 32) == seq && ((unsigned)w & HP_RFLAG_DONE)) {
                *flag = (int)((unsigned)w & ~HP_RFLAG_DONE);
                return 0;
            }
            if ((spins & 0x3ffff) == 0) {
                const hipError_t e = hipStreamQuery(st);
                if (e == hipSuccess) {
                    const unsigned long long w2 = __atomic_load_n(&ctx->hp_sig_h[r], __ATOMIC_ACQUIRE);
                    ZM_CHECK((unsigned)(w2 >> 32) == seq && ((unsigned)w2 & HP_RFLAG_DONE),
                             "zm_subtract: round %d finished without signalling the host", r);
                } else if (e != hipErrorNotReady) {
                    ZM_HIP(e);
                }
            }
            if (spins < 4096) __builtin_ia32_pause();
            else sched_yield();
        }
    };
    rounds = 0;
    ZM_TRY(enqueue_round(1));
    bool tmo_seen = false;
    for (int r = 1; r <= 8; ++r) {
        if (r < 8) ZM_TRY(enqueue_round(r + 1));
        int flag = 0;
        ZM_TRY(wait_round(r, &flag));
        rounds = r;
        tmo_seen = tmo_seen || (flag & HP_RFLAG_TMO);
        if ((flag & ~HP_RFLAG_TMO) == 0 || tmo_seen) break;
    }
    {
        zm_scope_timer t(ctx, "hp_apply");
        unsigned long long* smask = nullptr;
        ZM_TRY(ctx->get("hp_smask", sizeof(unsigned long long), (void**)&smask));
        hipLaunchKernelGGL(k_hp_solved, dim3(1), dim3(64), 0, st, P.nreg, P.nunk, stats, fail, tmo, rhs, smask, x0sum);
        {
            ZM_TRY(zm_hp_launch_apply(ctx, P, smask, sci, ref, sci_rms, ref_rms, outbad, d_filt, rhs, out_diff, out_rms, nmasked));
        }
    }
    if (hp->flag_mask_dev) {
        hipLaunchKernelGGL(k_hp_flag, dim3((unsigned)((np + 255) / 256)), b256, 0, st, hp->flag_mask_dev, out_diff, 1e-30f,
                           hp->flag_bit, np, tmo, P.nreg);
        ZM_HIP(hipGetLastError());
    }
    ZM_HIP(hipMemcpyAsync(h_sum, sumbuf, HP_SUMBYTES, hipMemcpyDeviceToHost, st));
    if (hp->async_info && !tmo_seen) {
        if (!ctx->hp_done) ZM_HIP(hipEventCreateWithFlags(&ctx->hp_done, hipEventDisableTiming));
        ZM_HIP(hipEventRecord(ctx->hp_done, st));
        ctx->hp_pending = true;
        ctx->hp_pend_rounds = rounds;
        ctx->hp_pend_retries = retries;
        ctx->hp_pend_nreg = P.nreg;
        ctx->hp_pend_nunk = P.nunk;
        fitting.release();
        if (info) {
            memset(info, 0, sizeof(*info));
            info->status = ZM_HP_PENDING;
            info->niter = rounds;
            info->ncoeff = P.nunk;
            info->retries = retries;
        }
        return 0;
    }
    ZM_HIP(hipStreamSynchronize(st));
    ntimeouts = 0;
    for (int reg = 0; reg < P.nreg; ++reg) ntimeouts += h_int[3 * HP_MAXREG + 4 + reg];
    if (ntimeouts == 0) break;
    if (!safe) {
        ++retries;
        if (getenv("ZM_VERBOSE"))
            fprintf(stderr, "zm_subtract: %d barrier time-out(s) in the fused factorisation; repeating the fit on the "
                            "one-workgroup form\n", ntimeouts);
    }
    }
    fitting.release();
    ctx->hp_pending = false;
    if (info) hp_fill_info(h_sum, P.nreg, P.nunk, rounds, retries, info);
    return 0;
}

extern "C" int zm_subtract_info(zm_ctx* ctx, zm_hp_info* info) {
    ZM_CHECK(ctx && info, "zm_subtract_info: null argument");
    ZM_CHECK(ctx->hp_pending, "zm_subtract_info: no subtraction with async_info is pending on this context");
    ZM_HIP(hipSetDevice(ctx->device));
    ZM_HIP(hipEventSynchronize(ctx->hp_done));
    ctx->hp_pending = false;
    char* h_sum = nullptr;
    ZM_TRY(ctx->get_pinned("hp_summary_h", HP_SUMBYTES_, (void**)&h_sum));
    const int* h_int = reinterpret_cast<const int*>(h_sum);
    for (int reg = 0; reg < ctx->hp_pend_nreg; ++reg)
        ZM_CHECK(h_int[3 * HP_MAXREG + 4 + reg] == 0, "zm_subtract_info: a barrier time-out went unnoticed (region %d)", reg);
    hp_fill_info(h_sum, ctx->hp_pend_nreg, ctx->hp_pend_nunk, ctx->hp_pend_rounds, ctx->hp_pend_retries, info);
    return 0;
}

static bool hp_plans_agree(const hp_plan& a, const hp_plan& b) {
    hp_plan x = a, y = b;
    x.tu = x.tl = x.iu = x.il = 0; y.tu = y.tl = y.iu = y.il = 0;
    x.fi = x.fin = 0; y.fi = y.fin = 0;
    return memcmp(&x, &y, sizeof(hp_plan)) == 0;
}

extern "C" int zm_subtract_batch_dev(zm_ctx* ctx, int njobs, const zm_sub_job* jobs, int nx, int ny,
                                     zm_hp_info* infos) {
    ZM_CHECK(ctx && jobs && njobs >= 1 && njobs <= ZM_SUB_BATCH_MAX, "zm_subtract_batch_dev: 1 .. %d jobs", ZM_SUB_BATCH_MAX);
    ZM_CHECK(nx > 0 && ny > 0, "zm_subtract_batch_dev: empty image");
    ZM_HIP(hipSetDevice(ctx->device));
    std::vector<hp_plan> Pj(njobs);
    std::vector<double> filt, basis, filt_j, basis_j;
    for (int j = 0; j < njobs; ++j) {
        const zm_sub_job& jb = jobs[j];
        ZM_CHECK(jb.sci && jb.sci_rms && jb.ref && jb.ref_rms && jb.params && jb.out_diff && jb.out_rms,
                 "zm_subtract_batch_dev: null argument in job %d", j);
        ZM_TRY(make_plan(jb.params, nx, ny, &Pj[j], j == 0 ? &filt : &filt_j, j == 0 ? &basis : &basis_j));
        ZM_CHECK(j == 0 || (hp_plans_agree(Pj[0], Pj[j]) && filt_j == filt),
                 "zm_subtract_batch_dev: job %d asks for a different fit (half widths, basis, orders, regions, stamps or "
                 "thresholds) than job 0 - batch jobs of one configuration", j);
    }
    const hp_plan& P = Pj[0];
    ZM_CHECK(nx > 2 * P.hw + 1 && ny > 2 * P.hw + 1, "zm_subtract_batch_dev: image smaller than a substamp");
    if (P.nkp > 15 || P.nunk > CBC_COLS || P.ncellr > 256 || njobs == 1 || P.hwk > 15 || hp_vectors_cfg(P.pw, P.sw, P.npix).big) {
        for (int j = 0; j < njobs; ++j)
            ZM_TRY(zm_subtract_dev(ctx, jobs[j].sci, jobs[j].sci_rms, jobs[j].ref, jobs[j].ref_rms, jobs[j].bpm, nx, ny,
                                   jobs[j].params, jobs[j].out_diff, jobs[j].out_rms, infos ? &infos[j] : nullptr));
        return 0;
    }
    const int64_t np = (int64_t)nx * ny;
    hipStream_t st = ctx->stream;
    const int lda = (P.nunk + 15) & ~15;
    const int ldt = (P.nunk + 1 + 15) & ~15;
    constexpr int HP_NIBUF = 4 * HP_MAXREG + 4;

    size_t off = 0;
    auto take = [&](size_t bytes) { const size_t o = off; off += (bytes + 255) & ~(size_t)255; return o; };
    const size_t o_bad = take(np), o_dirty = take(np), o_outbad = take(np);
    const size_t o_centres = take(sizeof(int2) * P.ncell * P.nss);
    const size_t o_active = take(sizeof(int) * P.ncell), o_need = take(sizeof(int) * P.ncell);
    const size_t o_needlist = take(sizeof(int) * ((size_t)P.ncell + 1));
    const size_t o_chg = take(sizeof(int) * (2 * (size_t)P.ncell + P.nreg));
    const size_t o_X = take(sizeof(double) * (size_t)P.ncell * P.nX * P.npixp);
    const size_t o_G = take(sizeof(double) * (size_t)P.ncell * HP_MAXX * HP_MAXX);
    const size_t o_Gp = take(sizeof(double) * (size_t)P.ncell * GR_SPLIT * HP_MAXX * HP_MAXX);
    const size_t o_Gold = take(sizeof(double) * (size_t)P.ncell * HP_MAXX * HP_MAXX);
    const size_t o_phi = take(sizeof(double) * (size_t)P.ncell * P.nkp);
    const size_t o_phiold = take(sizeof(double) * (size_t)P.ncell * P.nkp);
    const size_t o_vbar = take(sizeof(double) * P.ncell);
    const size_t o_A = take(sizeof(double) * (size_t)P.nreg * (P.nunk + 1) * lda);
    const size_t o_AT = take(sizeof(double) * (size_t)P.nreg * P.nunk * ldt);
    const size_t o_rhs = take(sizeof(double) * (size_t)P.nreg * P.nunk);
    const size_t o_A0 = take(sizeof(double) * (size_t)P.nreg * (P.nunk + 1) * P.nunk);
    const size_t o_rhs0 = take(sizeof(double) * (size_t)P.nreg * P.nunk);
    const size_t o_dsc = take(sizeof(double) * (size_t)P.nreg * P.nunk);
    const size_t o_merit = take(sizeof(double) * P.ncell);
    const size_t o_smask = take(sizeof(unsigned long long));
    const size_t slab = off;
    char* base = nullptr;
    ZM_TRY(ctx->get("hpb_slab", slab * (size_t)njobs, (void**)&base));
    uint8_t* tmp8 = nullptr;
    ZM_TRY(ctx->get("hp_tmp8", np, (void**)&tmp8));
    int *ibuf_all = nullptr, *rflags_all = nullptr, *h_rflags = nullptr;
    ZM_TRY(ctx->get("hpb_ibuf", sizeof(int) * HP_NIBUF * (size_t)njobs, (void**)&ibuf_all));
    ZM_TRY(ctx->get("hpb_rflags", sizeof(int) * 16 * (size_t)njobs, (void**)&rflags_all));
    double* sum_all = nullptr;
    ZM_TRY(ctx->get("hpb_sum", sizeof(double) * 3 * HP_MAXREG * (size_t)njobs, (void**)&sum_all));
    ZM_TRY(ctx->get_pinned("hpb_rflags_h", sizeof(int) * 32 * (size_t)njobs, (void**)&h_rflags));
    hp_job *h_jobs = nullptr, *d_jobs = nullptr;
    ZM_TRY(ctx->get_pinned("hpb_jobs_h", sizeof(hp_job) * (size_t)njobs * 9, (void**)&h_jobs));
    ZM_TRY(ctx->get("hpb_jobs", sizeof(hp_job) * (size_t)njobs * 9, (void**)&d_jobs));
    double* d_filt = nullptr;
    ZM_TRY(ctx->get("hp_filt", sizeof(double) * filt.size(), (void**)&d_filt));
    hipEvent_t* evs = nullptr;
    ZM_TRY(zm_get_sync_events(ctx, 3, &evs));
    ZM_HIP(hipStreamSynchronize(st));
    if (!(ctx->hp_filt_dev == (const void*)d_filt && ctx->hp_filt_host == filt)) {
        double* h_tab = nullptr;
// ... 225 lines not shown
```

### zuds-pipeline_amd/csrc/hp_apply.hip

```cpp
#include "hp_dev.h"

__device__ inline double xs_bg(const double* __restrict__ xsol, int reg, const hp_plan& P, int t) {
    return xsol[(size_t)reg * P.nunk + 1 + (size_t)(P.nc - 1) * P.nkp + t];
}

constexpr int apply_bank_passes(int pitch, int lpr, int r, int step) {
    int worst = 0;
    for (int half = 0; half < 2; ++half) {
        int cnt[64] = {};
        for (int l = 32 * half; l < 32 * half + 32; ++l) {
            const int row = l / lpr, strip = l % lpr;
            if (row >= step) continue;
            const int e = row * pitch + strip * r;
            ++cnt[(2 * e) % 64];
            ++cnt[(2 * e + 1) % 64];
        }
        for (int b = 0; b < 64; ++b) worst = cnt[b] > worst ? cnt[b] : worst;
    }
    return worst;
}
constexpr int apply_pitch(int width, int lpr, int r, int step) {
    int best = width, bw = apply_bank_passes(width, lpr, r, step);
    for (int p = width + 1; p <= width + 16; ++p) {
        const int w = apply_bank_passes(p, lpr, r, step);
        if (w < bw) { bw = w; best = p; }
    }
    return best;
}

constexpr int apply_pitch_n(int width, int lpr, int r, int step, int range) {
    int best = width, bw = apply_bank_passes(width, lpr, r, step);
    for (int p = width + 1; p <= width + range; ++p) {
        const int w = apply_bank_passes(p, lpr, r, step);
        if (w < bw) { bw = w; best = p; }
    }
    return best;
}

template <int HWK> struct apply_cfg {
    enum { STEP = 2 * HWK + 1,
           LPR = (STEP <= 11) ? 1 : (STEP <= 22 ? 2 : 3),
           R = (STEP + LPR - 1) / LPR,
           LPB = STEP * LPR,
           NB = 256 / LPB > 0 ? 256 / LPB : 1,
           TW = NB * STEP + 2 * HWK,
           TP = apply_pitch(NB * STEP + 2 * HWK, LPR, (STEP + LPR - 1) / LPR, STEP) };
};

template <int HWK>
__global__ __launch_bounds__(256) void k_hp_apply(const hp_plan P, const unsigned long long* __restrict__ solved_mask,
                                                  const float* __restrict__ sci,
                                                  const float* __restrict__ ref,
                                                  const float* __restrict__ srms,
                                                  const float* __restrict__ trms,
                                                  const uint8_t* __restrict__ outbad,
                                                  const double* __restrict__ filt,
                                                  const double* __restrict__ xsol,
                                                  float* __restrict__ diff,
                                                  float* __restrict__ noise,
                                                  int* __restrict__ nmasked) {
    const int reg = blockIdx.z;
    const int solved = (int)((*solved_mask >> reg) & 1ull);
    typedef apply_cfg<HWK> C;
    constexpr int STEP = C::STEP, R = C::R, LPR = C::LPR, LPB = C::LPB, NB = C::NB;
    constexpr int TW = C::TW;
    constexpr int TP = C::TP;
    constexpr int TH = STEP + 2 * HWK;
    typedef float ap_v2f __attribute__((ext_vector_type(2)));
    extern __shared__ float ap_smem[];
    ap_v2f* tTV = reinterpret_cast<ap_v2f*>(ap_smem);
    const int tvn = max(TH * TP, P.nunk + 2 * P.nc + (NB + 1) * P.nf1 * STEP + NB + 2 * NB * P.nkp);
    ap_v2f* kc = tTV + tvn;
    double* cf = reinterpret_cast<double*>(kc + NB * STEP * STEP);
    __shared__ int wmask[4];
    double* xs = reinterpret_cast<double*>(ap_smem);
    double* ts = xs + P.nunk;
    double* sb = ts + P.nc;
    double* fl = sb + P.nc;
    double* gf = fl + P.nf1 * STEP;
    double* s0v = gf + NB * P.nf1 * STEP;
    double* pxy = s0v + NB;
    const int tid = threadIdx.x;
    const int x0r = P.rx0[reg], x1r = P.rx1[reg], y0r = P.ry0[reg], y1r = P.ry1[reg];
    const int gx0 = x0r + blockIdx.x * NB * STEP;
    const int gy0 = y0r + blockIdx.y * STEP;
    if (gx0 >= x1r || gy0 >= y1r) return;
    const double xc = x0r + 0.5 * (x1r - x0r), hx = 0.5 * (x1r - x0r);
    const double yc = y0r + 0.5 * (y1r - y0r), hy = 0.5 * (y1r - y0r);
    const double* x = xsol + (size_t)reg * P.nunk;
    for (int e0 = tid; e0 < P.nunk; e0 += 256 * 4) {
        double t[4];
#pragma unroll
        for (int u = 0; u < 4; ++u) t[u] = (e0 + 256 * u < P.nunk) ? x[e0 + 256 * u] : 0.0;
#pragma unroll
        for (int u = 0; u < 4; ++u)
            if (e0 + 256 * u < P.nunk) xs[e0 + 256 * u] = t[u];
    }
    for (int e0 = tid; e0 < P.nf1 * STEP; e0 += 256 * 4) {
        double t[4];
#pragma unroll
        for (int u = 0; u < 4; ++u) t[u] = (e0 + 256 * u < P.nf1 * STEP) ? filt[e0 + 256 * u] : 0.0;
#pragma unroll
        for (int u = 0; u < 4; ++u)
            if (e0 + 256 * u < P.nf1 * STEP) fl[e0 + 256 * u] = t[u];
    }
    for (int e = tid; e < P.nc; e += 256) { ts[e] = P.tscale[e]; sb[e] = P.tsub0[e] ? 1.0 : 0.0; }
    for (int e = tid; e < NB * P.nkp; e += 256) {
        const int b = e / P.nkp, pp = e - b * P.nkp;
        const double fx = (gx0 + b * STEP + HWK - xc) / hx, fy = (gy0 + HWK - yc) / hy;
        pxy[2 * e] = ipowd(fx, P.kpi[pp]);
        pxy[2 * e + 1] = ipowd(fy, P.kpj[pp]);
    }
    __syncthreads();
    for (int e = tid; e < NB * P.nc; e += 256) {
        int b = e / P.nc, n = e - b * P.nc;
        double v;
        if (n == 0) v = xs[0];
        else {
            v = 0.0;
            const double* xb = xs + 1 + (n - 1) * P.nkp;
            const double* pb = pxy + 2 * b * P.nkp;
            for (int p = 0; p < P.nkp; ++p) v += xb[p] * pb[2 * p] * pb[2 * p + 1];
        }
        cf[e] = v;
    }
    __syncthreads();
    if (tid < NB) {
        double t = 0.0;
        for (int n = 0; n < P.nc; ++n) t += cf[tid * P.nc + n] * sb[n];
        s0v[tid] = t;
    }
    __syncthreads();
    for (int e = tid; e < NB * STEP * P.ngauss; e += 256) {
        const int g = e / (NB * STEP), r = e - g * NB * STEP;
        const int b = r / STEP, v = r - b * STEP;
        const double* cb = cf + b * P.nc;
        const int deg = P.gdeg[g], fb = P.gbase[g];
        int n = P.gterm0[g];
        for (int a = 0; a <= deg; ++a) {
            double acc = 0.0;
            for (int bb = 0; bb <= deg - a; ++bb, ++n) acc += cb[n] * ts[n] * fl[(fb + bb) * STEP + v];
            if (fb + a == P.tfx[0])
                acc -= s0v[b] * ts[0] * fl[P.tfy[0] * STEP + v];
            gf[((size_t)b * P.nf1 + fb + a) * STEP + v] = acc;
        }
    }
    __syncthreads();
    for (int e = tid; e < NB * STEP * STEP; e += 256) {
        const int b = e / (STEP * STEP), tap = e - b * STEP * STEP;
        const int v = tap / STEP, u = tap - v * STEP;
        const double* gb = gf + (size_t)b * P.nf1 * STEP + v;
        double acc = 0.0;
#pragma unroll 5
        for (int f = 0; f < P.nf1; ++f) acc += fl[f * STEP + u] * gb[f * STEP];
        const float k = (float)acc;
        kc[e] = (ap_v2f){k, k * k};
    }
    const double bg0 = xs[1 + (size_t)(P.nc - 1) * P.nkp];
    const float norm = P.normalize ? (float)(1.0 / xs[0]) : 1.f;
    __syncthreads();
    {
        constexpr int NIT = (TH * TW + 255) / 256;
        float tt[NIT], tr[NIT];
#pragma unroll
        for (int it = 0; it < NIT; ++it) {
            const int e = tid + 256 * it;
            const int yy = e / TW, xx = e - yy * TW;
            const int gx = gx0 - HWK + xx, gy = gy0 - HWK + yy;
            tt[it] = 0.f;
            tr[it] = 0.f;
            if (e < TH * TW && gx >= 0 && gx < P.nx && gy >= 0 && gy < P.ny) {
                const size_t idx = (size_t)gy * P.nx + gx;
                tt[it] = ref[idx];
                tr[it] = trms[idx];
            }
        }
#pragma unroll
        for (int it = 0; it < NIT; ++it) {
            const int e = tid + 256 * it;
            float t = tt[it], v = tr[it] * tr[it];
            if (!(fabsf(t) < 3e38f)) t = 0.f;
            if (!(fabsf(v) < 3e38f)) v = 0.f;
            if (e < TH * TW) tTV[(e / TW) * TP + e % TW] = (ap_v2f){t, v};
        }
    }
    __syncthreads();
    const int b = tid / LPB;
    const int l = tid - b * LPB;
    const int row = l / LPR, strip = l - row * LPR;
    const int ox0 = b * STEP + strip * R;
    const bool live = b < NB && gy0 + row < y1r && gy0 + row < P.ny;
    ap_v2f acc2[R];
#pragma unroll
    for (int q = 0; q < R; ++q) acc2[q] = (ap_v2f){0.f, 0.f};
    if (live) {
        const ap_v2f* kb = kc + b * STEP * STEP;
        for (int v = -HWK; v <= HWK; ++v) {
            const ap_v2f* rt = tTV + (row + HWK - v) * TP + ox0;
            ap_v2f w2[R + 2 * HWK];
#pragma unroll
            for (int q = 0; q < R + 2 * HWK; ++q) w2[q] = rt[q];
            const ap_v2f* kr = kb + (v + HWK) * STEP;
#pragma unroll
            for (int u = -HWK; u <= HWK; ++u) {
                const ap_v2f k2 = kr[u + HWK];
#pragma unroll
                for (int q = 0; q < R; ++q) acc2[q] = __builtin_elementwise_fma(k2, w2[q + HWK - u], acc2[q]);
            }
        }
    }
    constexpr int OW = NB * STEP;
    __syncthreads();
    if (live) {
#pragma unroll
        for (int q = 0; q < R; ++q)
            if (strip * R + q < STEP) tTV[row * OW + ox0 + q] = acc2[q];
    }
    __syncthreads();
    int masked = 0;
    {
        constexpr int NE = (STEP * OW + 255) / 256;
        float es[NE], er[NE];
        bool eb[NE], ein[NE];
#pragma unroll
        for (int it = 0; it < NE; ++it) {
            const int e = tid + 256 * it;
            const int orow = e / OW, ocol = e - orow * OW;
            const int gx = gx0 + ocol, gy = gy0 + orow;
            ein[it] = e < STEP * OW && gx < x1r && gx < P.nx && gy < y1r && gy < P.ny;
            es[it] = er[it] = 0.f;
            eb[it] = true;
            if (ein[it]) {
                const size_t idx = (size_t)gy * P.nx + gx;
                eb[it] = outbad[idx] != 0;
                es[it] = sci[idx];
                er[it] = srms[idx];
            }
        }
#pragma unroll
        for (int it = 0; it < NE; ++it) {
            if (!ein[it]) continue;
            const int e = tid + 256 * it;
            const int orow = e / OW, ocol = e - orow * OW;
            const int gx = gx0 + ocol, gy = gy0 + orow;
            const size_t idx = (size_t)gy * P.nx + gx;
            float d = P.fi, nz = P.fin;
            if (solved && !eb[it]) {
                double bg = bg0;
                if (P.nbg > 1) {
                    const double xf = (gx - xc) / hx, yf = (gy - yc) / hy;
                    bg = 0.0;
                    for (int t = 0; t < P.nbg; ++t)
                        bg += xs_bg(xsol, reg, P, t) * ipowd(xf, P.bpi[t]) * ipowd(yf, P.bpj[t]);
                }
                const ap_v2f a = tTV[e];
                d = (es[it] - a.x - (float)bg) * norm;
                nz = sqrtf(fmaxf(er[it] * er[it] + a.y, 0.f)) * fabsf(norm);
            } else {
                masked += 1;
            }
            diff[idx] = d;
            noise[idx] = nz;
        }
    }
#pragma unroll
    for (int o = 32; o >= 1; o >>= 1) masked += __shfl_xor(masked, o);
    if ((tid & 63) == 0) wmask[tid >> 6] = masked;
    __syncthreads();
    if (tid == 0) {
        const int tot = wmask[0] + wmask[1] + wmask[2] + wmask[3];
        if (tot) atomicAdd(nmasked, tot);
    }
}

template <int HWK> struct applyw_cfg {
    enum { STEP = 2 * HWK + 1,
           LPR = 64 / STEP > 0 ? 64 / STEP : 1,
           R = (STEP + LPR - 1) / LPR,
           NBW = 4,
           TW = NBW * STEP + 2 * HWK,
           TH = STEP + 2 * HWK,
           TP = apply_pitch_n(NBW * STEP + 2 * HWK, 64 / STEP > 0 ? 64 / STEP : 1,
                              (STEP + (64 / STEP > 0 ? 64 / STEP : 1) - 1) / (64 / STEP > 0 ? 64 / STEP : 1), STEP, 32) };
    enum { EFF = (100 * STEP * LPR / 64) * STEP / (LPR * R) };
};

#define HPK_MAXP 15
#define HPK_NBK 16
template <int HWK>
__global__ __launch_bounds__(256) void k_hp_kbasis(const hp_plan P, const double* __restrict__ filt,
                                                   const double* __restrict__ xsol, double* __restrict__ Mt) {
    constexpr int STEP = 2 * HWK + 1, NT = STEP * STEP;
    const int reg = blockIdx.y, p = blockIdx.x;
    const double* x = xsol + (size_t)reg * P.nunk;
    __shared__ double xq[HP_MAXX], sn[HP_MAXX], flt[HP_MAXF1 * STEP];
    __shared__ int txn[HP_MAXX], tyn[HP_MAXX], sbn[HP_MAXX];
    const int tid = threadIdx.x;
    for (int n = tid; n < P.nc; n += 256) {
        sn[n] = P.tscale[n];
        txn[n] = P.tfx[n] * STEP;
        tyn[n] = P.tfy[n] * STEP;
        sbn[n] = P.tsub0[n];
        xq[n] = (n >= 1 && p < P.nkp) ? x[1 + (size_t)(n - 1) * P.nkp + p] : 0.0;
    }
    for (int e = tid; e < P.nf1 * STEP; e += 256) flt[e] = filt[e];
    __syncthreads();
    for (int tap = tid; tap < NT; tap += 256) {
        const int v = tap / STEP, u = tap - v * STEP;
        const double b0 = sn[0] * flt[tyn[0] + v] * flt[txn[0] + u];
        double acc = 0.0;
        if (p == HPK_MAXP) {
            acc = x[0] * (b0 - (sbn[0] ? b0 : 0.0));
        } else if (p < P.nkp) {
#pragma unroll 8
            for (int n = 1; n < P.nc; ++n) {
                const double bn = sn[n] * flt[tyn[n] + v] * flt[txn[n] + u];
                acc += xq[n] * (bn - (sbn[n] ? b0 : 0.0));
            }
        }
        Mt[((size_t)reg * (HPK_MAXP + 1) + p) * NT + tap] = acc;
    }
}

template <int HWK>
__global__ __launch_bounds__(512) void k_hp_ktable(const hp_plan P, const double* __restrict__ Mt, int maxbx, int maxby,
                                                   float2* __restrict__ kcg) {
    constexpr int STEP = 2 * HWK + 1, NT = STEP * STEP, TPT = (NT + 511) / 512;
    __shared__ double W[HPK_NBK][HPK_MAXP + 1];
    const int reg = blockIdx.z, tid = threadIdx.x;
    const int x0r = P.rx0[reg], x1r = P.rx1[reg], y0r = P.ry0[reg], y1r = P.ry1[reg];
    const int bx0 = blockIdx.x * HPK_NBK;
    const int gx0 = x0r + bx0 * STEP, gy0 = y0r + blockIdx.y * STEP;
    if (gx0 >= x1r || gy0 >= y1r) return;
    const double xc = x0r + 0.5 * (x1r - x0r), hx = 0.5 * (x1r - x0r);
    const double yc = y0r + 0.5 * (y1r - y0r), hy = 0.5 * (y1r - y0r);
    for (int e = tid; e < HPK_NBK * (HPK_MAXP + 1); e += 512) {
        const int b = e / (HPK_MAXP + 1), pp = e - b * (HPK_MAXP + 1);
        double w = 0.0;
        if (pp < P.nkp) {
            const double fx = (gx0 + b * STEP + HWK - xc) / hx, fy = (gy0 + HWK - yc) / hy;
            w = ipowd(fx, P.kpi[pp]) * ipowd(fy, P.kpj[pp]);
        }
        W[b][pp] = w;
    }
    double m[TPT][HPK_MAXP + 1];
#pragma unroll
    for (int t = 0; t < TPT; ++t)
#pragma unroll
        for (int pp = 0; pp <= HPK_MAXP; ++pp) {
            const int tap = min(tid + 512 * t, NT - 1);
            m[t][pp] = Mt[((size_t)reg * (HPK_MAXP + 1) + pp) * NT + tap];
        }
    __syncthreads();
    for (int b = 0; b < HPK_NBK; ++b) {
        const int bx = bx0 + b;
        if (bx >= maxbx || gx0 + b * STEP >= x1r) break;
        float2* out = kcg + (((size_t)reg * maxby + blockIdx.y) * maxbx + bx) * NT;
        double w[HPK_MAXP];
#pragma unroll
        for (int pp = 0; pp < HPK_MAXP; ++pp) w[pp] = W[b][pp];
#pragma unroll
        for (int t = 0; t < TPT; ++t) {
            double acc = m[t][HPK_MAXP];
#pragma unroll
            for (int pp = 0; pp < HPK_MAXP; ++pp) acc = fma(w[pp], m[t][pp], acc);
            const float k = (float)acc;
            const int tap = tid + 512 * t;
            if (tap < NT) out[tap] = make_float2(k, k * k);
        }
    }
}

template <int HWK>
__global__ __launch_bounds__(256) void k_hp_apply_w(const hp_plan P, const unsigned long long* __restrict__ solved_mask,
                                                    const float* __restrict__ sci,
                                                    const float* __restrict__ ref,
                                                    const float* __restrict__ srms,
                                                    const float* __restrict__ trms,
                                                    const uint8_t* __restrict__ outbad,
                                                    const double* __restrict__ xsol,
                                                    const float2* __restrict__ kcg, int maxbx, int maxby,
                                                    float* __restrict__ diff,
                                                    float* __restrict__ noise,
                                                    int* __restrict__ nmasked) {
    const int reg = blockIdx.z;
    const int solved = (int)((*solved_mask >> reg) & 1ull);
    typedef applyw_cfg<HWK> C;
    constexpr int STEP = C::STEP, R = C::R, LPR = C::LPR, NB = C::NBW, TW = C::TW, TP = C::TP, TH = C::TH;
    typedef float ap_v2f __attribute__((ext_vector_type(2)));
    extern __shared__ float apw_smem[];
    ap_v2f* tTV = reinterpret_cast<ap_v2f*>(apw_smem);
    __shared__ int wmask[4];
    const int tid = threadIdx.x;
    const int x0r = P.rx0[reg], x1r = P.rx1[reg], y0r = P.ry0[reg], y1r = P.ry1[reg];
    const int gx0 = x0r + blockIdx.x * NB * STEP;
    const int gy0 = y0r + blockIdx.y * STEP;
    if (gx0 >= x1r || gy0 >= y1r) return;
    const double xc = x0r + 0.5 * (x1r - x0r), hx = 0.5 * (x1r - x0r);
    const double yc = y0r + 0.5 * (y1r - y0r), hy = 0.5 * (y1r - y0r);
    const double bg0 = xsol[(size_t)reg * P.nunk + 1 + (size_t)(P.nc - 1) * P.nkp];
    const float norm = P.normalize ? (float)(1.0 / xsol[(size_t)reg * P.nunk]) : 1.f;
    {
        constexpr int NIT = (TH * TW + 255) / 256;
        float tt[NIT], tr[NIT];
#pragma unroll
        for (int it = 0; it < NIT; ++it) {
            const int e = tid + 256 * it;
            const int yy = e / TW, xx = e - yy * TW;
            const int gx = gx0 - HWK + xx, gy = gy0 - HWK + yy;
            tt[it] = 0.f;
            tr[it] = 0.f;
            if (e < TH * TW && gx >= 0 && gx < P.nx && gy >= 0 && gy < P.ny) {
                const size_t idx = (size_t)gy * P.nx + gx;
                tt[it] = ref[idx];
                tr[it] = trms[idx];
            }
        }
#pragma unroll
        for (int it = 0; it < NIT; ++it) {
            const int e = tid + 256 * it;
            float t = tt[it], v = tr[it] * tr[it];
            if (!(fabsf(t) < 3e38f)) t = 0.f;
            if (!(fabsf(v) < 3e38f)) v = 0.f;
            if (e < TH * TW) tTV[(e / TW) * TP + e % TW] = (ap_v2f){t, v};
        }
    }
    __syncthreads();
    const int b = __builtin_amdgcn_readfirstlane(tid >> 6);
    const int l = tid & 63;
    const int row = l / LPR, strip = l - row * LPR;
    const int ox0 = b * STEP + strip * R;
    const bool live = row < STEP && gx0 + b * STEP < x1r && gy0 + row < y1r && gy0 + row < P.ny;
    ap_v2f acc2[R];
#pragma unroll
    for (int q = 0; q < R; ++q) acc2[q] = (ap_v2f){0.f, 0.f};
    {
        const int bxi = min((int)blockIdx.x * NB + b, maxbx - 1);
        const ap_v2f* kb = reinterpret_cast<const ap_v2f*>(kcg) +
                           (((size_t)reg * maxby + blockIdx.y) * maxbx + bxi) * (STEP * STEP);
        const int rowc = min(row, STEP - 1);
#pragma unroll 1
        for (int v = -HWK; v <= HWK; ++v) {
            const ap_v2f* rt = tTV + (rowc + HWK - v) * TP + ox0;
            ap_v2f w2[R + 2 * HWK];
#pragma unroll
            for (int q = 0; q < R + 2 * HWK; ++q) w2[q] = rt[(LPR * R == STEP) ? q : min(q, TW - 1 - ox0)];
            const ap_v2f* kr = kb + (v + HWK) * STEP;
#pragma unroll
            for (int u = -HWK; u <= HWK; ++u) {
                const ap_v2f k2 = kr[u + HWK];
#pragma unroll
                for (int q = 0; q < R; ++q) acc2[q] = __builtin_elementwise_fma(k2, w2[q + HWK - u], acc2[q]);
            }
        }
    }
    constexpr int OW = NB * STEP;
    __syncthreads();
    if (live) {
#pragma unroll
        for (int q = 0; q < R; ++q)
            if (strip * R + q < STEP) tTV[row * OW + ox0 + q] = acc2[q];
    }
    __syncthreads();
    int masked = 0;
    {
        constexpr int NE = (STEP * OW + 255) / 256;
        float es[NE], er[NE];
        bool eb[NE], ein[NE];
#pragma unroll
        for (int it = 0; it < NE; ++it) {
            const int e = tid + 256 * it;
            const int orow = e / OW, ocol = e - orow * OW;
            const int gx = gx0 + ocol, gy = gy0 + orow;
            ein[it] = e < STEP * OW && gx < x1r && gx < P.nx && gy < y1r && gy < P.ny;
            es[it] = er[it] = 0.f;
            eb[it] = true;
            if (ein[it]) {
                const size_t idx = (size_t)gy * P.nx + gx;
                eb[it] = outbad[idx] != 0;
                es[it] = sci[idx];
                er[it] = srms[idx];
            }
        }
#pragma unroll
        for (int it = 0; it < NE; ++it) {
            if (!ein[it]) continue;
            const int e = tid + 256 * it;
            const int orow = e / OW, ocol = e - orow * OW;
            const int gx = gx0 + ocol, gy = gy0 + orow;
            const size_t idx = (size_t)gy * P.nx + gx;
            float d = P.fi, nz = P.fin;
            if (solved && !eb[it]) {
                double bg = bg0;
                if (P.nbg > 1) {
                    const double xf = (gx - xc) / hx, yf = (gy - yc) / hy;
                    bg = 0.0;
                    for (int t = 0; t < P.nbg; ++t)
                        bg += xs_bg(xsol, reg, P, t) * ipowd(xf, P.bpi[t]) * ipowd(yf, P.bpj[t]);
                }
                const ap_v2f a = tTV[e];
                d = (es[it] - a.x - (float)bg) * norm;
                nz = sqrtf(fmaxf(er[it] * er[it] + a.y, 0.f)) * fabsf(norm);
            } else {
                masked += 1;
            }
            diff[idx] = d;
            noise[idx] = nz;
        }
    }
#pragma unroll
    for (int o = 32; o >= 1; o >>= 1) masked += __shfl_xor(masked, o);
    if ((tid & 63) == 0) wmask[tid >> 6] = masked;
    __syncthreads();
    if (tid == 0) {
        const int tot = wmask[0] + wmask[1] + wmask[2] + wmask[3];
        if (tot) atomicAdd(nmasked, tot);
    }
}

template <int HWK>
static int launch_apply(zm_ctx* ctx, const hp_plan& P, const unsigned long long* solved_mask, const float* sci,
                        const float* ref, const float* srms, const float* trms, const uint8_t* outbad,
                        const double* filt, const double* xsol, float* diff, float* noise,
                        int* nmasked) {
    typedef apply_cfg<HWK> C;
    constexpr int STEP = C::STEP, NB = C::NB;
    constexpr int TP = C::TP, TH = STEP + 2 * HWK;
    const size_t tvn = std::max((size_t)TH * TP, (size_t)P.nunk + 2 * (size_t)P.nc + (size_t)(NB + 1) * P.nf1 * STEP + NB + (size_t)2 * NB * P.nkp);
    size_t fl = 2 * tvn + (size_t)2 * NB * STEP * STEP;
    size_t shmem = fl * sizeof(float) + (size_t)NB * P.nc * sizeof(double);
    size_t& set_max = ctx->hp_set_max[HWK];
    if (set_max < 65536) set_max = 65536;
    if (shmem > set_max) {
        ZM_HIP(hipFuncSetAttribute((const void*)k_hp_apply<HWK>,
                                   hipFuncAttributeMaxDynamicSharedMemorySize, (int)shmem));
        set_max = shmem;
    }
    int W = 0, H = 0;
    for (int reg = 0; reg < P.nreg; ++reg) {
        W = std::max(W, P.rx1[reg] - P.rx0[reg]);
        H = std::max(H, P.ry1[reg] - P.ry0[reg]);
    }
    typedef applyw_cfg<HWK> CW;
    const char* form = getenv("ZM_APPLY_FORM");
    const bool wave_form = (form ? !strcmp(form, "wave") : (CW::EFF >= 60 && HWK >= 4)) && P.nkp <= HPK_MAXP;
    if (wave_form && !(form && !strcmp(form, "tile"))) {
        const int maxbx = zm_div_up(W, STEP), maxby = zm_div_up(H, STEP);
        float2* kcg = nullptr;
        ZM_TRY(ctx->get("hp_kcg", sizeof(float2) * (size_t)P.nreg * maxby * maxbx * STEP * STEP, (void**)&kcg));
        double* Mt = nullptr;
        ZM_TRY(ctx->get("hp_kmt", sizeof(double) * (size_t)P.nreg * (HPK_MAXP + 1) * STEP * STEP, (void**)&Mt));
        hipLaunchKernelGGL(k_hp_kbasis<HWK>, dim3(HPK_MAXP + 1, P.nreg), dim3(256), 0, ctx->stream, P, filt, xsol, Mt);
        hipLaunchKernelGGL(k_hp_ktable<HWK>, dim3(zm_div_up(maxbx, HPK_NBK), maxby, P.nreg), dim3(512), 0, ctx->stream,
                           P, Mt, maxbx, maxby, kcg);
        const size_t wsh = sizeof(float2) * (size_t)CW::TH * CW::TP;
        static bool wset[HP_MAX_HWK + 1][64] = {};
        if (wsh > 65536 && !wset[HWK][ctx->device & 63]) {
            ZM_HIP(hipFuncSetAttribute((const void*)k_hp_apply_w<HWK>, hipFuncAttributeMaxDynamicSharedMemorySize, (int)wsh));
            wset[HWK][ctx->device & 63] = true;
        }
        hipLaunchKernelGGL(k_hp_apply_w<HWK>, dim3(zm_div_up(maxbx, CW::NBW), maxby, P.nreg), dim3(256), wsh, ctx->stream,
                           P, solved_mask, sci, ref, srms, trms, outbad, xsol, kcg, maxbx, maxby, diff, noise, nmasked);
        ZM_HIP(hipGetLastError());
        return 0;
    }
    dim3 grd(zm_div_up(zm_div_up(W, STEP), NB), zm_div_up(H, STEP), P.nreg);
    hipLaunchKernelGGL(k_hp_apply<HWK>, grd, dim3(256), shmem, ctx->stream, P, solved_mask, sci, ref, srms,
                       trms, outbad, filt, xsol, diff, noise, nmasked);
    ZM_HIP(hipGetLastError());
    return 0;
}


int zm_hp_launch_apply(zm_ctx* ctx, const hp_plan& P, const unsigned long long* solved_mask, const float* sci,
                       const float* ref, const float* srms, const float* trms, const uint8_t* outbad,
                       const double* filt, const double* xsol, float* diff, float* noise, int* nmasked) {
#define C(H) case H: return launch_apply<H>(ctx, P, solved_mask, sci, ref, srms, trms, outbad, filt, xsol, diff, noise, nmasked);
    switch (P.hwk) {
        C(1) C(2) C(3) C(4) C(5) C(6) C(7) C(8) C(9) C(10) C(11) C(12) C(13) C(14) C(15) C(16) C(17) C(18) C(19) C(20)
        default: zm_set_error("zm_subtract: unsupported kernel half width %d", P.hwk); return 2;
    }
#undef C
}
```

### zuds-pipeline_amd/csrc/hp_dev.h

```cpp
#pragma once
#include <algorithm>
#include <atomic>
#include <cmath>

#include "zm_internal.h"

#define HP_MAXX 64
#define HP_MAXPOLY 28
#define HP_MAXNSS 8
#define HP_MAXREG 64
#define CF_BAR_STRIDE 32
#define HP_MAXF1 32
#define HP_RIDGE 1e-10

struct hp_plan {
    int nx, ny, hwk, hwss, hw, step, sw, npix, npixp, pw;
    int nc, nbg, nE, nX, nkp, nunk, ko, bgo;
    int nrx, nry, nsx, nsy, nss, nreg, ncellr, ncell, nf1;
    int normalize;
    double tu, tl, iu, il, ft, ks;
    float fi, fin;
    int rx0[HP_MAXREG], rx1[HP_MAXREG], ry0[HP_MAXREG], ry1[HP_MAXREG];
    int tfx[HP_MAXX], tfy[HP_MAXX], tsub0[HP_MAXX];
    double tscale[HP_MAXX];
// ... 3 lines not shown
    int tf0[HP_MAXF1], tfn[HP_MAXF1];
};


__device__ inline double wave_sum_d(double v) {
#pragma unroll
    for (int o = 32; o >= 1; o >>= 1) v += __shfl_xor(v, o);
    return v;
}

template <int NW>
__device__ inline double block_sum_waves(double v, double* red) {
    v = wave_sum_d(v);
    __syncthreads();
    if ((threadIdx.x & 63) == 0) red[threadIdx.x >> 6] = v;
    __syncthreads();
    double t[NW];
#pragma unroll
    for (int w = 0; w < NW; ++w) t[w] = red[w];
#pragma unroll
    for (int step = 1; step < NW; step *= 2)
#pragma unroll
        for (int w = 0; w + step < NW; w += 2 * step) t[w] += t[w + step];
    return t[0];
}

__device__ inline double block_sum256(double v, double* red) {
    v = wave_sum_d(v);
    __syncthreads();
    if ((threadIdx.x & 63) == 0) red[threadIdx.x >> 6] = v;
    __syncthreads();
    return (red[0] + red[1]) + (red[2] + red[3]);
}

__device__ inline double ipowd(double x, int n) {
    double r = 1.0;
    for (int k = 0; k < n; ++k) r *= x;
    return r;
}

#define HV_R 8
#define HV_SPLIT_ALL 5
#define HV_SPLIT_FEW 16

#define HV_THREADS 512
#define HP_MAX_HWK 20
#define HP_MAX_HWSS 60
struct hv_cfg { bool big; bool w0_global; int cw; size_t shmem; };
static inline hv_cfg hp_vectors_cfg(int pw, int sw, int npix) {
    const size_t lim = 160 * 1024, patch = sizeof(float) * (size_t)pw * (pw + 8) + 16;
    const size_t fast = sizeof(double) * ((size_t)(pw + 8) * sw + npix + 8) + patch;
    if (fast <= lim) return {false, false, sw, fast};
    const size_t full = sizeof(double) * ((size_t)(pw + 8) * sw + 8) + patch;
    if (full <= lim) return {true, true, sw, full};
    if (patch + sizeof(double) * 8 + sizeof(double) * (size_t)(pw + 8) * 8 > lim) return {true, true, 0, 0};
    int cw = (int)((lim - patch - sizeof(double) * 8) / (sizeof(double) * (size_t)(pw + 8)));
    cw &= ~7;
    return {true, true, cw, sizeof(double) * ((size_t)(pw + 8) * cw + 8) + patch};
}

struct hp_job {
    const float *sci, *ref, *srms, *trms;
    int2* centres;
    int *active, *need, *needlist, *chg, *ibuf, *rflags;
    double *X, *G, *Gp, *Gold, *phi, *phiold, *vbar, *A, *AT, *rhs, *A0, *rhs0, *dsc, *merit, *stats;
    unsigned long long* smask;
};
#define HPJ_NREJ(J) ((J).ibuf)
#define HPJ_NTOTAL(J) ((J).ibuf + HP_MAXREG)
#define HPJ_FAIL(J) ((J).ibuf + 2 * HP_MAXREG)
#define HPJ_NMASKED(J) ((J).ibuf + 3 * HP_MAXREG)
#define HPJ_TMO(J) ((J).ibuf + 3 * HP_MAXREG + 4)
#define HPJ_GUARD(J, round) ((round) > 1 ? (J).rflags + ((round) - 1) : nullptr)
#define HPJ_REGION_IDLE(J, round, reg, ncell, ncellr) ((round) > 1 && (J).chg[(ncell) + (reg) * ((ncellr) + 1)] == 0)

int zm_hp_launch_vectors(zm_ctx* ctx, hipStream_t st, const hp_plan& P, const hv_cfg& hvc, int rounds, int ncl_grid, int hv_gx,
                         const float* sci, const float* ref, const float* sci_rms, const float* ref_rms, const double* filt,
                         const int2* centres, const int* active, const int* need, double* X, double* phi, double* vbar,
                         const int* guard, double* phiold, const int* needlist, double* hv_w0g);
int zm_hp_launch_vectors_b(zm_ctx* ctx, hipStream_t st, const hp_plan& P, size_t vsh, unsigned gcells, unsigned njobs,
                           const hp_job* d_tab, const double* filt, int round);
int zm_hp_launch_apply(zm_ctx* ctx, const hp_plan& P, const unsigned long long* solved_mask, const float* sci,
                       const float* ref, const float* srms, const float* trms, const uint8_t* outbad,
                       const double* filt, const double* xsol, float* diff, float* noise, int* nmasked);
```

### zuds-pipeline_amd/csrc/resample.hip

```cpp
#include "resample_dev.h"

__global__ __launch_bounds__(256) void k_lattice(const zm_map_params mp, int lnx, int lny, double2* __restrict__ lat) {
    int gx = blockIdx.x * blockDim.x + threadIdx.x;
    int gy = blockIdx.y * blockDim.y + threadIdx.y;
    if (gx >= lnx || gy >= lny) return;
    double xi, yi;
    zm_map_out_to_in(&mp.wout, &mp.win, mp.rot, 1.0 + (double)gx * LSTEP,
                     1.0 + (double)gy * LSTEP, &xi, &yi);
    lat[(size_t)gy * lnx + gx] = make_double2(xi - 1.0, yi - 1.0);
}

__global__ void k_lattice_batch(const zm_map_params* __restrict__ mps, int lnx, int lny,
                                double2* __restrict__ lat) {
    int gx = blockIdx.x * blockDim.x + threadIdx.x;
    int gy = blockIdx.y * blockDim.y + threadIdx.y;
    if (gx >= lnx || gy >= lny) return;
    const zm_map_params* mp = mps + blockIdx.z;
    double xi, yi;
    zm_map_out_to_in(&mp->wout, &mp->win, mp->rot, 1.0 + (double)gx * LSTEP,
                     1.0 + (double)gy * LSTEP, &xi, &yi);
    lat[((size_t)blockIdx.z * lny + gy) * lnx + gx] = make_double2(xi - 1.0, yi - 1.0);
}

int zm_launch_lattice_batch(zm_ctx* ctx, const zm_map_params* mp_host, int n, int lnx, int lny,
// ... 177 lines not shown
        if (y < ny && x < spitch) {
            float4 o[2];
            prep_quad(img, wgt, nx, bk, nbx, nby, invmesh, var_scale, wthresh, vec_ok, x, y, o);
            typedef float zm_nt4 __attribute__((ext_vector_type(4)));
            zm_nt4* d4 = reinterpret_cast<zm_nt4*>(dst + (size_t)y * spitch + x);
            __builtin_nontemporal_store((zm_nt4){o[0].x, o[0].y, o[0].z, o[0].w}, &d4[0]);
            if (x + 2 < spitch) __builtin_nontemporal_store((zm_nt4){o[1].x, o[1].y, o[1].z, o[1].w}, &d4[1]);
        }
    }
#pragma unroll
    for (int q = 0; q < NLD; ++q) {
        const int e = tid + 256 * q;
        if (e < IH * IW) t0[(e / IW) * IP + (e % IW)] = mm[q];
    }
    __syncthreads();
    for (int e = tid; e < IH * TWB; e += 256) {
        const int r = e / TWB, c = e - r * TWB;
        int32_t o = 0;
#pragma unroll
        for (int k = 0; k < NT; ++k) o |= t0[r * IP + c + k];
        h[e] = o;
    }
    __syncthreads();
    for (int e = tid; e < THB * TWB; e += 256) {
        const int r = e / TWB, c = e - r * TWB;
        const int x = x0 + c, y = y0 + r;
        if (x + NT <= nx && y + NT <= ny) {
            int32_t o = 0;
#pragma unroll
            for (int k = 0; k < NT; ++k) o |= h[(r + k) * TWB + c];
            B[(size_t)y * bpitch + x] = box_entry(o);
        }
    }
}

int zm_launch_prep(zm_ctx* ctx, const float* img, const float* wgt, int nx, int ny,
                   const float* bknodes, int nbx, int nby, int mesh, const float* var_scale_dev,
                   float wthresh, float2* dst, int spitch, const int32_t* mask_for_box, int box_nt,
                   uint16_t* mbox_out, int mbox_pitch) {
    if (mbox_pitch <= 0) mbox_pitch = nx;
    const float invmesh = mesh > 0 ? 1.0f / mesh : 0.f;
    const int vec_ok = (nx % 4 == 0) && (((uintptr_t)img & 15) == 0) && (((uintptr_t)wgt & 15) == 0);
    ctx->box_ready_for = nullptr;
    if (mask_for_box && (box_nt == 6 || box_nt == 2)) {
        uint16_t* mbox = mbox_out;
        if (!mbox) ZM_TRY(ctx->get("mask_box", sizeof(uint16_t) * (size_t)nx * ny, (void**)&mbox));
        dim3 grd(zm_div_up(spitch, 64), zm_div_up(ny, 16), 1);
        zm_scope_timer t(ctx, "prep");
        if (box_nt == 6)
            hipLaunchKernelGGL(k_prep_box<6>, grd, dim3(256), 0, ctx->stream, img, wgt, nx, ny, bknodes, nbx,
                               nby, invmesh, var_scale_dev, wthresh, vec_ok, dst, spitch, mask_for_box, mbox, mbox_pitch);
        else
            hipLaunchKernelGGL(k_prep_box<2>, grd, dim3(256), 0, ctx->stream, img, wgt, nx, ny, bknodes, nbx,
                               nby, invmesh, var_scale_dev, wthresh, vec_ok, dst, spitch, mask_for_box, mbox, mbox_pitch);
        ZM_HIP(hipGetLastError());
        if (!mbox_out) {
            ctx->box_ready_for = mask_for_box;
            ctx->box_ready_nt = box_nt;
        }
        return 0;
    }
    dim3 blk(256, 1, 1), grd(zm_div_up(zm_div_up(spitch, 4), 256), ny, 1);
    zm_scope_timer t(ctx, "prep");
    hipLaunchKernelGGL(k_prep, grd, blk, 0, ctx->stream, img, wgt, nx, ny, bknodes, nbx, nby, invmesh,
                       var_scale_dev, wthresh, vec_ok, dst, spitch);
    ZM_HIP(hipGetLastError());
    return 0;
}

__global__ __launch_bounds__(256) void k_prep_pair(const float* __restrict__ a, const float* __restrict__ b, int nx, int ny,
                                                   float2* __restrict__ dst, int spitch) {
    const int x = blockIdx.x * 256 + threadIdx.x, y = blockIdx.y;
    if (x >= spitch) return;
    const size_t k = (size_t)y * nx + x;
    dst[(size_t)y * spitch + x] = x < nx ? make_float2(a[k], b[k]) : make_float2(0.f, 0.f);
}
int zm_launch_prep_pair(zm_ctx* ctx, const float* a, const float* b, int nx, int ny, float2* dst, int spitch) {
    zm_scope_timer t(ctx, "prep");
    hipLaunchKernelGGL(k_prep_pair, dim3(zm_div_up(spitch, 256), ny), dim3(256), 0, ctx->stream, a, b, nx, ny, dst, spitch);
    ZM_HIP(hipGetLastError());
    return 0;
}

template <int KIND, int MASKOP>
__global__ __launch_bounds__(256, 4) void k_resample(
    const float2* __restrict__ src, int nx, int ny, int spitch, const double2* __restrict__ lat,
    int lnx, int lny, float fscale, float2* __restrict__ dst, int onx, int ony, int lds_cap,
    const int32_t* __restrict__ mask, const uint16_t* __restrict__ mbox, int32_t* __restrict__ macc,
    int mkind, int mfirst, int ntx, int ntiles, const float* __restrict__ taptab,
    float* __restrict__ plane_a, float* __restrict__ plane_b, float pair_scale) {
    extern __shared__ float4 smem4[];
    rs_hdr* HR = reinterpret_cast<rs_hdr*>(smem4);
    constexpr int TABF = (KIND == ZM_RESAMPLE_LANCZOS3) ? LZ_FLOATS : 0;
    const float* ltab = reinterpret_cast<const float*>(smem4) + HDR_FLOATS;
    float2* tile = reinterpret_cast<float2*>(smem4) + (HDR_FLOATS + TABF) / 2;
    constexpr int NT = taps_traits<KIND>::N;
    constexpr int OFF = taps_traits<KIND>::OFF;
    constexpr int CI = -OFF;
    const int tid = threadIdx.x;
    const int G = gridDim.x;
    const float fscale2 = fscale * fscale;
    const float4 fill = make_float4(0.f, ZM_BIGVAR, 0.f, ZM_BIGVAR);

    float4 pf[RS_PF];
    auto prefetch = [&](const rs_hdr* H) {
        if (!H->use_lds) return;
        const int bx0 = H->h.bx0, by0 = H->h.by0, bw2 = H->h.bw >> 1;
        const int n4 = bw2 * H->h.bh;
        const float inv = 1.0f / (float)bw2;
#pragma unroll
        for (int k = 0; k < RS_PF; ++k) {
            const int e = tid + 256 * k;
            pf[k] = fill;
            if (e < n4) {
                const int r = (int)(((float)e + 0.5f) * inv);
                const int c2 = e - r * bw2;
                const int gy = by0 + r, gx = bx0 + 2 * c2;
                if (gy >= 0 && gy < ny && gx >= 0 && gx < spitch)
                    pf[k] = *reinterpret_cast<const float4*>(src + (size_t)gy * spitch + gx);
            }
        }
    };
    auto store = [&](const rs_hdr* H) {
        if (!H->use_lds) return;
        const int n4 = (H->h.bw >> 1) * H->h.bh;
#pragma unroll
        for (int k = 0; k < RS_PF; ++k) {
            const int e = tid + 256 * k;
            if (e < n4)
                *reinterpret_cast<float4*>(tile + 2 * e) = pf[k];
        }
    };

    int t = blockIdx.x;
    if (t >= ntiles) return;
    if (KIND == ZM_RESAMPLE_LANCZOS3) {
        for (int e = tid; e < LZ_FLOATS / 4; e += 256)
            smem4[HDR_FLOATS / 4 + e] = reinterpret_cast<const float4*>(taptab)[e];
    }
    if (tid < 64) {
        rs_build_header<KIND>(lat, lnx, lny, t, ntx, nx, ny, lds_cap, &HR[0]);
        if (t + G < ntiles) rs_build_header<KIND>(lat, lnx, lny, t + G, ntx, nx, ny, lds_cap, &HR[1]);
    }
    __syncthreads();
    prefetch(&HR[0]);
    int slot = 0;
    for (; t < ntiles; t += G) {
        const rs_hdr* H = &HR[slot];
        const int nslot = slot == 2 ? 0 : slot + 1;
        const int nnslot = nslot == 2 ? 0 : nslot + 1;
        store(H);
        __syncthreads();
        const bool use_lds = H->use_lds, touches = H->touches;
        const int bx0 = H->h.bx0, by0 = H->h.by0, bw = H->h.bw, bh = H->h.bh;
        const int tyi = t / ntx, txi = t - tyi * ntx;
        const int ox0 = txi * TW, oy0 = tyi * RTH;
        const int tx = tid & 63, tyb = tid >> 6;
        const int ox = ox0 + tx;
        int32_t aprev[RTH / 4];
#pragma unroll
        for (int q = 0; q < RTH / 4; ++q) aprev[q] = -1;
        if (MASKOP == 2 && !mfirst) {
#pragma unroll
            for (int q = 0; q < RTH / 4; ++q) {
                const int oy = oy0 + tyb + 4 * q;
                if (ox < onx && oy < ony) aprev[q] = macc[(size_t)oy * onx + ox];
            }
        }
        if (t + G < ntiles) prefetch(&HR[nslot]);
        if (tid < 64 && t + 2 * G < ntiles)
            rs_build_header<KIND>(lat, lnx, lny, t + 2 * G, ntx, nx, ny, lds_cap, &HR[nnslot]);

        float xr[3], yr[3];
        {
            const int cell = tx >> 4;
            const float fx = (float)(tx & 15) * (1.f / LSTEP);
#pragma unroll
            for (int r = 0; r < 3; ++r) {
                const float x0 = H->h.nrel[r][cell][0], x1 = H->h.nrel[r][cell + 1][0];
                const float y0 = H->h.nrel[r][cell][1], y1 = H->h.nrel[r][cell + 1][1];
                xr[r] = x0 + fx * (x1 - x0);
                yr[r] = y0 + fx * (y1 - y0);
            }
        }
#pragma unroll 1
        for (int q = 0; q < RTH / 4; ++q) {
            const int ty = tyb + 4 * q;
            const int oy = oy0 + ty;
            if (ox >= onx || oy >= ony) continue;
            const int cr = q >> 2;
            const float fy = (float)(ty & 15) * (1.f / LSTEP);
            const float xa = cr ? xr[1] : xr[0], xb = cr ? xr[2] : xr[1];
            const float ya = cr ? yr[1] : yr[0], yb = cr ? yr[2] : yr[1];
            const float px = xa + fy * (xb - xa), py = ya + fy * (yb - ya);
            int ixr, iyr;
            float dx, dy;
            bool ddx, ddy;
            split_pos(px, &ixr, &dx, &ddx);
            split_pos(py, &iyr, &dy, &ddy);
            const int ix = bx0 + ixr + OFF, iy = by0 + iyr + OFF;
            const bool inbx = ddx ? (ix + CI >= 0 && ix + CI < nx) : (ix >= 0 && ix + NT <= nx);
            const bool inby = ddy ? (iy + CI >= 0 && iy + CI < ny) : (iy >= 0 && iy + NT <= ny);
            const bool inb = touches && inbx && inby;
            float2 res = make_float2(0.f, 0.f);
            int32_t mres = 0;
            uint32_t m16 = 0;
            if (inb) {
                if (MASKOP) {
                    if (!(ddx || ddy)) {
                        m16 = mbox[(size_t)iy * nx + ix];
                    } else {
                        const int c0 = ddx ? CI : 0, c1 = ddx ? CI + 1 : NT;
                        const int r0 = ddy ? CI : 0, r1 = ddy ? CI + 1 : NT;
                        for (int r = r0; r < r1; ++r) {
                            const int32_t* mp = mask + (size_t)(iy + r) * nx + ix;
                            for (int c = c0; c < c1; ++c) mres |= mp[c];
                        }
                    }
                }
                zm_v2f tw[NT];
                float acc = 0.f, vacc = 0.f;
                if (KIND == ZM_RESAMPLE_LANCZOS3) {
                    zm_v2f txp[3], typ[3];
                    zm_lz3_lookup(ltab, ddx ? 0.5f : dx, txp);
                    zm_lz3_lookup(ltab, ddy ? 0.5f : dy, typ);
                    if (__any(ddx || ddy)) {
#pragma unroll
                        for (int j = 0; j < 3; ++j) {
                            const zm_v2f dl = (zm_v2f){j == 1 ? 1.f : 0.f, 0.f};
                            txp[j] = ddx ? dl : txp[j];
                            typ[j] = ddy ? dl : typ[j];
                        }
                    }
#pragma unroll
                    for (int k = 0; k < NT; ++k)
                        tw[k] = (zm_v2f){(k & 1) ? txp[k >> 1].y : txp[k >> 1].x,
                                         (k & 1) ? typ[k >> 1].y : typ[k >> 1].x};
                } else {
                    make_taps2<KIND>(dx, dy, ddx, ddy, tw);
                }
                if (use_lds) {
                    const float2* p = tile + (iyr + OFF) * bw + (ixr + OFF);
                    zm_v2f av = (zm_v2f){0.f, 0.f};
#pragma unroll
                    for (int r = 0; r < NT; ++r) {
                        float2 s[NT];
                        lds_row<NT>::read(p, s);
                        zm_v2f rv2 = (zm_v2f){0.f, 0.f};
#pragma unroll
                        for (int c = 0; c < NT; ++c)
                            rv2 = __builtin_elementwise_fma((zm_v2f){tw[c].x, tw[c].x},
                                                            (zm_v2f){s[c].x, s[c].y}, rv2);
                        av = __builtin_elementwise_fma((zm_v2f){tw[r].y, tw[r].y}, rv2, av);
                        p += bw;
                    }
                    acc = av.x;
                    vacc = av.y;
                } else {
                    const float2* p = src + (size_t)iy * spitch + ix;
#pragma unroll
                    for (int r = 0; r < NT; ++r) {
                        float ra = 0.f, rv = 0.f;
                        if (tw[r].y != 0.f) {
#pragma unroll
                            for (int c = 0; c < NT; ++c) {
                                if (tw[c].x != 0.f) {
                                    float2 s = p[c];
                                    ra = fmaf(tw[c].x, s.x, ra);
                                    rv = fmaf(tw[c].x, s.y, rv);
                                }
                            }
                        }
                        acc = fmaf(tw[r].y, ra, acc);
                        vacc = fmaf(tw[r].y, rv, vacc);
                        p += spitch;
                    }
                }
                if (MASKOP != 2 && pair_scale != 0.f) {
                    bool bada = false, badb = false;
                    if (!(__builtin_isfinite(acc) && __builtin_isfinite(vacc))) {
                        if (use_lds) {
                            const float2* p = tile + (iyr + OFF) * bw + (ixr + OFF);
                            zm_v2f av = (zm_v2f){0.f, 0.f};
#pragma unroll
                            for (int r = 0; r < NT; ++r) {
                                float2 s[NT];
                                lds_row<NT>::read(p, s);
                                zm_v2f rv2 = (zm_v2f){0.f, 0.f};
#pragma unroll
                                for (int c = 0; c < NT; ++c) {
                                    const bool nz = tw[c].x != 0.f && tw[r].y != 0.f;
                                    const bool fa = __builtin_isfinite(s[c].x), fb = __builtin_isfinite(s[c].y);
                                    bada = bada || (nz && !fa);
                                    badb = badb || (nz && !fb);
                                    rv2 = __builtin_elementwise_fma((zm_v2f){tw[c].x, tw[c].x},
                                                                    (zm_v2f){fa ? s[c].x : 0.f, fb ? s[c].y : 0.f}, rv2);
                                }
                                av = __builtin_elementwise_fma((zm_v2f){tw[r].y, tw[r].y}, rv2, av);
                                p += bw;
                            }
                            acc = av.x;
                            vacc = av.y;
                        } else {
                            const float2* p = src + (size_t)iy * spitch + ix;
                            acc = 0.f;
                            vacc = 0.f;
                            for (int r = 0; r < NT; ++r) {
                                float ra = 0.f, rv = 0.f;
                                if (tw[r].y != 0.f) {
                                    for (int c = 0; c < NT; ++c) {
                                        if (tw[c].x != 0.f) {
                                            const float2 s = p[c];
                                            const bool fa = __builtin_isfinite(s.x), fb = __builtin_isfinite(s.y);
                                            bada = bada || !fa;
                                            badb = badb || !fb;
                                            ra = fmaf(tw[c].x, fa ? s.x : 0.f, ra);
                                            rv = fmaf(tw[c].x, fb ? s.y : 0.f, rv);
                                        }
                                    }
                                }
                                acc = fmaf(tw[r].y, ra, acc);
                                vacc = fmaf(tw[r].y, rv, vacc);
                                p += spitch;
                            }
                        }
                    }
                    res.x = bada ? 0.f : acc * fscale;
                    res.y = badb ? 0.f : vacc * pair_scale;
                } else if (vacc > 0.f && vacc < ZM_BADVAR_TEST) {
                    res.x = acc * fscale;
                    res.y = __builtin_amdgcn_rcpf(vacc * fscale2);
                }
                if (MASKOP && !(ddx || ddy)) {
                    if (m16 != ZM_BOX_RAW) {
                        mres = (int32_t)m16;
                    } else {
                        for (int r = 0; r < NT; ++r) {
                            const int32_t* mp = mask + (size_t)(iy + r) * nx + ix;
                            for (int c = 0; c < NT; ++c) mres |= mp[c];
                        }
                    }
                }
            }
            const size_t oidx = (size_t)oy * onx + ox;
            if (plane_a) {
                plane_a[oidx] = res.x;
                plane_b[oidx] = res.y;
            } else {
                dst[oidx] = res;
            }
            if (MASKOP == 1) {
                macc[oidx] = mres;
            } else if (MASKOP == 2) {
                int32_t a = aprev[0];
#pragma unroll
                for (int k = 1; k < RTH / 4; ++k) a = (q == k) ? aprev[k] : a;
                if (inb) {
                    if (a == -1) a = mres;
                    else a = (mkind == ZM_MASK_AND) ? (a & mres) : (a | mres);
                }
                macc[oidx] = a;
            }
        }
        __syncthreads();
        slot = nslot;
    }
}

__global__ __launch_bounds__(256) void k_resample_nearest(const float2* __restrict__ src, int nx,
                                                          int ny, int spitch,
                                                          const double2* __restrict__ lat,
                                                          int lnx, int lny, float fscale,
                                                          float2* __restrict__ dst, int onx,
                                                          int ony) {
    __shared__ tile_hdr hdr;
    const int tid = threadIdx.x;
    const int ox0 = blockIdx.x * TW, oy0 = blockIdx.y * TH;
    if (tid < 64) build_tile_header(lat, lnx, lny, ox0 / LSTEP, oy0 / LSTEP, 0, 0, &hdr);
    __syncthreads();
    const int tx = tid & 63, tyb = tid >> 6;
    const int ox = ox0 + tx;
    for (int q = 0; q < 4; ++q) {
        const int ty = tyb + 4 * q, oy = oy0 + ty;
        if (ox >= onx || oy >= ony) continue;
        float px, py;
        tile_position(&hdr, tx, ty, &px, &py);
        int ix = hdr.bx0 + (int)floorf(px + 0.5f), iy = hdr.by0 + (int)floorf(py + 0.5f);
        float2 res = make_float2(0.f, 0.f);
        if (ix >= 0 && ix < nx && iy >= 0 && iy < ny) {
            float2 s = src[(size_t)iy * spitch + ix];
            if (s.y > 0.f && s.y < ZM_BADVAR_TEST) {
                res.x = s.x * fscale;
                res.y = 1.f / (s.y * fscale * fscale);
            }
        }
        dst[(size_t)oy * onx + ox] = res;
    }
}

template <int KIND>
static int launch_resample_kind(zm_ctx* ctx, dim3 grd, size_t shmem, const float2* src, int nx, int ny,
                                int spitch, const double2* lat, int lnx, int lny, float fscale,
                                float2* dst, int onx, int ony, int lds_elems, const int32_t* mask,
                                int32_t* macc, int mop, int mkind, int mfirst, float* plane_a, float* plane_b,
                                float pair_scale) {
    dim3 blk(256, 1, 1);
    const int ntx = grd.x, ntiles = grd.x * grd.y;
    uint16_t* mbox = nullptr;
    if (mop) {
        constexpr int NT = taps_traits<KIND>::N;
        ZM_TRY(ctx->get("mask_box", sizeof(uint16_t) * (size_t)nx * ny, (void**)&mbox));
        if (ctx->box_ready_for != (const void*)mask || ctx->box_ready_nt != NT) {
            zm_scope_timer tb(ctx, "mask_box");
            hipLaunchKernelGGL(k_mask_box<NT>, dim3(zm_div_up(nx, 64), zm_div_up(ny, 16)), blk, 0, ctx->stream,
                               mask, nx, ny, mbox);
        }
        ctx->box_ready_for = nullptr;
    }
    const float* taptab = nullptr;
    if (KIND == ZM_RESAMPLE_LANCZOS3) {
        ZM_TRY(zm_get_lanczos_table(ctx, &taptab));
        shmem += sizeof(float) * LZ_FLOATS;
    }
    zm_scope_timer t(ctx, "resample");
    dim3 pgrd(std::min(ntiles, 256 * 4), 1, 1);
    if (mop == 0)
        hipLaunchKernelGGL((k_resample<KIND, 0>), pgrd, blk, shmem, ctx->stream, src, nx, ny, spitch, lat,
                           lnx, lny, fscale, dst, onx, ony, lds_elems, mask, mbox, macc, mkind, mfirst, ntx, ntiles, taptab, plane_a, plane_b, pair_scale);
    else if (mop == 1)
        hipLaunchKernelGGL((k_resample<KIND, 1>), pgrd, blk, shmem, ctx->stream, src, nx, ny, spitch, lat,
                           lnx, lny, fscale, dst, onx, ony, lds_elems, mask, mbox, macc, mkind, mfirst, ntx, ntiles, taptab, plane_a, plane_b, pair_scale);
    else
        hipLaunchKernelGGL((k_resample<KIND, 2>), pgrd, blk, shmem, ctx->stream, src, nx, ny, spitch, lat,
                           lnx, lny, fscale, dst, onx, ony, lds_elems, mask, mbox, macc, mkind, mfirst, ntx, ntiles, taptab, plane_a, plane_b, pair_scale);
    ZM_HIP(hipGetLastError());
    return 0;
}

int zm_launch_resample(zm_ctx* ctx, const float2* src, int nx, int ny, int spitch,
                       const double2* lat, int lnx, int lny, int kernel, float fscale,
                       float2* dst, int onx, int ony, int lds_elems, const int32_t* mask,
                       int32_t* macc, int mop, int mkind, int mfirst, float* plane_a, float* plane_b, float pair_scale) {
    dim3 blk(256, 1, 1), grd(zm_div_up(onx, TW), zm_div_up(ony, TH), 1);
    ZM_CHECK(pair_scale == 0.f || (kernel != ZM_RESAMPLE_NEAREST && plane_a && plane_b && ctx->edge == ZM_EDGE_ZERO && mop != 2),
             "zm_launch_resample: a pair of images takes LANCZOS3 / BILINEAR, two output planes, the default edge rule and no mask accumulation");
    dim3 rgrd(zm_div_up(onx, TW), zm_div_up(ony, RTH), 1);
    if (!mask || !macc) mop = 0;
    if (lds_elems > RS_PFCAP) lds_elems = RS_PFCAP;
    size_t shmem = (size_t)HDR_FLOATS * 4 + (size_t)lds_elems * sizeof(float2);
    if (kernel == ZM_RESAMPLE_LANCZOS3 || kernel == ZM_RESAMPLE_BILINEAR) {
        const bool lz = mop && ctx->mask_resample == ZM_MASKRES_LANCZOS_ROUND, trunc = ctx->edge == ZM_EDGE_TRUNCATE;
        const int mop_img = lz ? 0 : mop;
        if (kernel == ZM_RESAMPLE_LANCZOS3)
            ZM_TRY(launch_resample_kind<ZM_RESAMPLE_LANCZOS3>(ctx, rgrd, shmem, src, nx, ny, spitch, lat, lnx,
                                                              lny, fscale, dst, onx, ony, lds_elems, mask,
                                                              macc, mop_img, mkind, mfirst, plane_a, plane_b, pair_scale));
        else
            ZM_TRY(launch_resample_kind<ZM_RESAMPLE_BILINEAR>(ctx, rgrd, shmem, src, nx, ny, spitch, lat, lnx,
                                                              lny, fscale, dst, onx, ony, lds_elems, mask,
                                                              macc, mop_img, mkind, mfirst, plane_a, plane_b, pair_scale));
        if (trunc)
            ZM_TRY(zm_launch_resample_rim(ctx, src, nx, ny, spitch, lat, lnx, lny, kernel, fscale, dst, plane_a, plane_b, onx,
                                          ony, mask, macc, mop_img, mkind));
        if (lz) {
            const int64_t opix = (int64_t)onx * ony;
            if (mop == 1) return zm_launch_resample_mask_opts(ctx, mask, nx, ny, lat, lnx, lny, kernel, macc, onx, ony, 0, 1, trunc);
            int32_t* tmp = nullptr;
            ZM_TRY(ctx->get("mask_tmp", sizeof(int32_t) * opix, (void**)&tmp));
            ZM_TRY(zm_launch_resample_mask_opts(ctx, mask, nx, ny, lat, lnx, lny, kernel, tmp, onx, ony, -1, 1, trunc));
            return zm_launch_mask_accum(ctx, macc, tmp, opix, mkind, mfirst);
        }
        return 0;
    }
    if (kernel == ZM_RESAMPLE_NEAREST) {
        zm_scope_timer t(ctx, "resample");
        hipLaunchKernelGGL(k_resample_nearest, grd, blk, 0, ctx->stream, src, nx, ny, spitch, lat, lnx,
                           lny, fscale, dst, onx, ony);
        ZM_HIP(hipGetLastError());
        if (plane_a) ZM_TRY(zm_launch_split_pairs(ctx, dst, (int64_t)onx * ony, plane_a, plane_b));
        if (mop) {
            int32_t* tmp = nullptr;
            const int64_t opix = (int64_t)onx * ony;
            if (mop == 1) return zm_launch_resample_mask(ctx, mask, nx, ny, lat, lnx, lny, kernel, macc,
                                                         onx, ony, 0);
            ZM_TRY(ctx->get("mask_tmp", sizeof(int32_t) * opix, (void**)&tmp));
            ZM_TRY(zm_launch_resample_mask(ctx, mask, nx, ny, lat, lnx, lny, kernel, tmp, onx, ony, -1));
            return zm_launch_mask_accum(ctx, macc, tmp, opix, mkind, mfirst);
        }
        return 0;
    }
    zm_set_error("zm_launch_resample: unknown kernel %d", kernel);
    return 2;
}

template <int KIND>
__global__ __launch_bounds__(256) void k_resample_mask(const int32_t* __restrict__ mask, int nx,
                                                       int ny, const double2* __restrict__ lat,
                                                       int lnx, int lny,
                                                       int32_t* __restrict__ dst, int onx,
                                                       int ony, int32_t fill) {
    __shared__ tile_hdr hdr;
    constexpr int NT = taps_traits<KIND>::N;
    constexpr int OFF = taps_traits<KIND>::OFF;
    const int tid = threadIdx.x;
    const int ox0 = blockIdx.x * TW, oy0 = blockIdx.y * TH;
    if (tid < 64) build_tile_header(lat, lnx, lny, ox0 / LSTEP, oy0 / LSTEP, OFF, OFF + NT - 1, &hdr);
    __syncthreads();
    const int tx = tid & 63, tyb = tid >> 6;
    const int ox = ox0 + tx;
    for (int q = 0; q < 4; ++q) {
        const int ty = tyb + 4 * q, oy = oy0 + ty;
        if (ox >= onx || oy >= ony) continue;
        float px, py;
        tile_position(&hdr, tx, ty, &px, &py);
        int ixr, iyr;
        float dx, dy;
        bool ddx, ddy;
        split_pos(px, &ixr, &dx, &ddx);
        split_pos(py, &iyr, &dy, &ddy);
        const int ix = hdr.bx0 + ixr + OFF, iy = hdr.by0 + iyr + OFF;
        int32_t m = fill;
        const bool inbx = ddx ? (ix - OFF >= 0 && ix - OFF < nx) : (ix >= 0 && ix + NT <= nx);
        const bool inby = ddy ? (iy - OFF >= 0 && iy - OFF < ny) : (iy >= 0 && iy + NT <= ny);
        if (inbx && inby) {
            m = 0;
            int c0 = ddx ? -OFF : 0, c1 = ddx ? -OFF + 1 : NT;
            int r0 = ddy ? -OFF : 0, r1 = ddy ? -OFF + 1 : NT;
            if (KIND == ZM_RESAMPLE_BILINEAR) {
                c0 = 0; c1 = ddx ? 1 : 2; r0 = 0; r1 = ddy ? 1 : 2;
            }
            for (int r = r0; r < r1; ++r) {
                const int32_t* p = mask + (size_t)(iy + r) * nx + ix;
                for (int c = c0; c < c1; ++c) m |= p[c];
            }
        }
        dst[(size_t)oy * onx + ox] = m;
    }
}

__global__ __launch_bounds__(256) void k_resample_mask_nearest(const int32_t* __restrict__ mask,
                                                               int nx, int ny,
                                                               const double2* __restrict__ lat,
                                                               int lnx, int lny,
// ... 47 lines not shown
```

### zuds-pipeline_amd/csrc/zm_internal.h

```cpp
#pragma once
#include <hip/hip_runtime.h>
#include <cstdint>
#include <cstdio>
#include <cstring>
#include <map>
#include <string>
#include <vector>
#include <stdexcept>

#include "../../include/zudsmi.h"

#define ZM_BIGVAR 1e30f
#define ZM_BADVAR_TEST 1e14f
#define ZM_SNAP 1e-5f

void zm_set_error(const char* fmt, ...);

#ifdef ZM_DEV
#define ZM_DEVENV(name) getenv(name)
#define ZM_DEV_BUILD 1
#else
#define ZM_DEVENV(name) ((const char*)nullptr)
#define ZM_DEV_BUILD 0
#endif

#define ZM_HIP(call)                                                         \
    do {                                                                     \
        hipError_t e_ = (call);                                              \
        if (e_ != hipSuccess) {                                              \
            zm_set_error("%s failed: %s (%s:%d)", #call, hipGetErrorString(e_), \
                         __FILE__, __LINE__);                                \
            return 1;                                                        \
        }                                                                    \
    } while (0)

#define ZM_CHECK(cond, ...)                                                  \
    do {                                                                     \
        if (!(cond)) {                                                       \
            zm_set_error(__VA_ARGS__);                                       \
            return 2;                                                        \
        }                                                                    \
    } while (0)

#define ZM_TRY(expr)                                                         \
    do {                                                                     \
        int r_ = (expr);                                                     \
        if (r_) return r_;                                                   \
    } while (0)

struct zm_timer_slot {
    double total_ms = 0.0;
    int64_t launches = 0;
    std::vector<std::pair<hipEvent_t, hipEvent_t>> pending;
};

struct zm_ctx {
    int device = 0;
    hipStream_t stream = nullptr;
    bool own_stream = true;
    std::map<std::string, std::pair<void*, size_t>> scratch;
    std::map<std::string, std::pair<void*, size_t>> pinned;
    hipStream_t aux = nullptr;
    std::vector<hipEvent_t> sync_events;
    const void* box_ready_for = nullptr;
    int box_ready_nt = 0;
    int share = 1;
    int hp_wg_cap = 0;
    bool hp_rset = false, hp_bset = false;
    hipEvent_t hp_done = nullptr;
    unsigned long long *hp_sig_h = nullptr, *hp_sig_d = nullptr;
    unsigned hp_seq = 0;
    bool hp_pending = false;
    int hp_pend_rounds = 0, hp_pend_retries = 0, hp_pend_nreg = 0, hp_pend_nunk = 0;
    std::map<int, size_t> hp_set_max;
    std::vector<double> hp_filt_host;
    const void* hp_filt_dev = nullptr;
    bool ff_pre_valid = false;
    int ff_pre_nfr = 0, ff_pre_onx = 0, ff_pre_ony = 0, ff_pre_lds = 0;
    bool ff_pre_own = false;
    int edge = 0;
    int mask_resample = 0;
    int ff_last_form = 0;
    bool bk_stats_set = false, bk_filter_set = false;
    hipEvent_t bk_stats_event = nullptr;
    bool bk_stats_event_valid = false;
    bool timing = false;
    std::string timing_only;
    std::map<std::string, zm_timer_slot> timers;
    std::vector<hipEvent_t> event_pool;

    int get(const char* name, size_t bytes, void** out);
    int get_pinned(const char* name, size_t bytes, void** out);
    void release_all();
};

struct zm_scope_timer {
    zm_ctx* ctx;
    const char* name;
    hipEvent_t a = nullptr, b = nullptr;
    zm_scope_timer(zm_ctx* c, const char* n);
    ~zm_scope_timer();
};

static inline int zm_div_up(int a, int b) { return (a + b - 1) / b; }

#define ZM_LATTICE_STEP 16

struct zm_map_params {
    zm_wcs wout;
    zm_wcs win;
    double rot[9];
};

void zm_wcs_frame(const zm_wcs* w, double fr[9]);
void zm_make_map(const zm_wcs* wout, const zm_wcs* win, zm_map_params* mp);
void zm_map_point(const zm_map_params* mp, double xo, double yo, double* xi, double* yi);
double zm_pixel_area(const zm_wcs* w, double x, double y);

int zm_launch_lattice(zm_ctx* ctx, const zm_map_params* mp, int lnx, int lny, double2* lat_dev);
int zm_launch_lattice_batch(zm_ctx* ctx, const zm_map_params* mp_host, int n, int lnx, int lny,
                            double2* lat_dev, hipEvent_t after = nullptr);
int zm_launch_prep(zm_ctx* ctx, const float* img, const float* wgt, int nx, int ny,
                   const float* bknodes, int nbx, int nby, int mesh,
                   const float* var_scale_dev, float wthresh, float2* dst, int spitch,
                   const int32_t* mask_for_box = nullptr, int box_nt = 0, uint16_t* mbox_out = nullptr,
                   int mbox_pitch = 0);
struct zm_ff {
    const float* img;
    const float* wgt;
    const float4* ytab;
    const float4* xtab;
    const float* vscale;
    const float2* src;
    const double2* lat;
    const void* mask;
    const uint16_t* mbox;
    const float* bk;
    const int* mboxflag;
    int nx, ny, spitch, nbx, nby, ytp;
    float invmesh, wthresh, fscale, fscale2;
    int vec_ok, mpitch;
    int mask16, pad_;
};
struct zm_bkrows {
    const float* bk;
    float4* out;
    int nbx, nby, ny, ytp;
    float invmesh;
    int nx;
    float4* xout;
};
struct zm_boxjob {
    const void* m;
    uint16_t* B;
    int* rawflag;
    int nx, ny, pitch, is16;
};
void zm_fused_geometry(int* tile_h, int* lds_cap);
int zm_launch_fused_prepass(zm_ctx* ctx, const zm_bkrows* rows, int nrows);
int zm_launch_mask_boxes(zm_ctx* ctx, const zm_boxjob* boxes, int nboxes, hipEvent_t after, hipEvent_t* joined,
                         hipEvent_t after2 = nullptr);
int zm_launch_fused_headers_early(zm_ctx* ctx, const zm_ff* frames_host, int nfr, int lnx, int lny, int onx, int ony,
                                  int lds_elems, bool fits_own);
int zm_launch_coadd_fused(zm_ctx* ctx, const zm_ff* frames_host, int nfr, int lnx, int lny, int onx, int ony,
                          int lds_elems, int combine, int mask_kind, float* out_img, float* out_wgt,
                          int32_t* out_mask, float* out_cov, int partial, int32_t* unmasked_out,
                          float2* stack = nullptr, int64_t fstride = 0, bool fits_own = false);
int zm_get_lanczos_table(zm_ctx* ctx, const float** out);
int zm_check_wcs(const zm_wcs* w, const char* what);
int zm_resample_lds_plan(const zm_map_params* mp, int onx, int ony, int kernel);
int zm_frame_background(zm_ctx* ctx, const float* img, const float* wgt, int nx, int ny,
                        int mesh, int fsize, float wthresh, int mode0, int nmode,
                        float** nodes_dev, float** stats_dev, int* nbx_out, int* nby_out,
                        const char* slot, int index = 0, int count = 1);
int zm_batch_stats(zm_ctx* ctx, int nf, const float* const* imgs, const float* const* wgts, int nx,
                   int ny, int mesh, float wthresh, int mode0, int nmode, const char* slot, int index0,
                   int count, int nslot);
int zm_batch_filter(zm_ctx* ctx, int nf, int nx, int ny, int mesh, int fsize, int nmode,
                    const char* slot, int index0, int count, int nslot);
int zm_frame_products(zm_ctx* ctx, int nx, int ny, int mesh, const char* slot, int index, int count,
                      int nslot, float** nodes_dev, float** stats_dev, int* nbx_out, int* nby_out);
int zm_batch_var_scale(zm_ctx* ctx, int nf, const float* stats, float* out);
int zm_frame_stats(zm_ctx* ctx, const float* img, const float* wgt, int nx, int ny, int mesh,
                   float wthresh, int mode0, int nmode, const char* slot, int index, int count);
int zm_frame_filter(zm_ctx* ctx, int nx, int ny, int mesh, int fsize, int nmode, float** nodes_dev,
                    float** stats_dev, int* nbx_out, int* nby_out, const char* slot, int index,
                    int count);
int zm_get_sync_events(zm_ctx* ctx, int n, hipEvent_t** out);
hipStream_t zm_ctx_aux(zm_ctx* ctx);
int zm_launch_var_scale(zm_ctx* ctx, const float* bstats, const float* vstats, float* out);
int zm_launch_resample(zm_ctx* ctx, const float2* src, int nx, int ny, int spitch,
                       const double2* lat, int lnx, int lny, int kernel, float fscale,
                       float2* dst, int onx, int ony, int lds_elems, const int32_t* mask,
                       int32_t* macc, int mop, int mkind, int mfirst,
                       float* plane_a = nullptr, float* plane_b = nullptr, float pair_scale = 0.f);
int zm_launch_prep_pair(zm_ctx* ctx, const float* a, const float* b, int nx, int ny, float2* dst, int spitch);
int zm_launch_resample_mask(zm_ctx* ctx, const int32_t* mask, int nx, int ny,
                            const double2* lat, int lnx, int lny, int kernel,
                            int32_t* dst, int onx, int ony, int32_t fill);
int zm_launch_combine(zm_ctx* ctx, int n, const float2* stack, int64_t frame_stride,
                      int64_t npix, int kind, float clip_sigma, float clip_ampfrac,
                      float* out_img, float* out_wgt, int partial);
int zm_launch_resample_rim(zm_ctx* ctx, const float2* src, int nx, int ny, int spitch, const double2* lat, int lnx,
                           int lny, int kernel, float fscale, float2* dst, float* plane_a, float* plane_b, int onx,
                           int ony, const int32_t* mask, int32_t* macc, int mop, int mkind);
int zm_launch_resample_mask_opts(zm_ctx* ctx, const int32_t* mask, int nx, int ny, const double2* lat, int lnx, int lny,
                                 int kernel, int32_t* dst, int onx, int ony, int32_t fill, int lanczos, int trunc);
int zm_launch_mask_accum(zm_ctx* ctx, int32_t* acc, const int32_t* m, int64_t npix, int kind,
                         int first);
int zm_launch_mask_finalize(zm_ctx* ctx, int32_t* acc, float* cov, int64_t npix);
int zm_launch_split_pairs(zm_ctx* ctx, const float2* src, int64_t npix, float* a, float* b);
int zm_launch_mask_widen(zm_ctx* ctx, const int16_t* in, int64_t n, int32_t* out);
```

### zuds-pipeline_amd/device.py

```python
import ctypes as C
import os

import numpy as np

from . import _lib
from ._lib import check, wcs_struct
from .engine import coadd_params, get_engine


def _torch():
    import torch
    return torch


class DeviceFrames(object):

    def __init__(self, frames, device):
        torch = _torch()
        self.n = len(frames)
        self.tensors = []
        self.arr = (_lib.zm_dframe * self.n)()
        for i, f in enumerate(frames):
            img = self._dev(f['img'], torch.float32, device)
            wgt = self._dev(f.get('wgt'), torch.float32, device)
# ... 183 lines not shown
            cut = rb_cut_for(fid, rb_cut)
        tab, nfound, _ = self.extract(wcs=wcs, max_objects=max_objects, **extract_params)
        tab = tab[((tab['IMAFLAGS_ISO'] & self.BAD_SUM) == 0) & (tab['FLAGS_WEIGHT'] == 0)]
        self.engine.set_stream(self.stream.cuda_stream)
        with self.torch.cuda.stream(self.stream):
            pix = pixel_cuts_dev(self.engine, self.diff, self.noise, self.submask, tab['X_IMAGE'], tab['Y_IMAGE'],
                                 bad_bits=self.BAD_SUM)
        if rb_model is None:
            return filter_table(tab, float(seeing), pix), nfound
        rows = tab[good_before_ml(tab, float(seeing), pix) > 0]
        rb = np.zeros(0)
        if len(rows):
            blocks, norms, _, _ = self.stamps(np.asarray(rows['X_WORLD'], np.float64), np.asarray(rows['Y_WORLD'], np.float64),
                                              sci, ref, size=rb_model.in_size, sci_flxscale=sci_flxscale, device_out=True)
            with self.torch.cuda.stream(self.stream):
                rb_dev = rb_model.score_dev(blocks, norms, order=('sub', 'new', 'ref'), engine=self.engine, stream=self.stream)
                rb_host = rb_dev.cpu()
            self.stream.synchronize()
            rb = rb_host.numpy().astype(np.float64)
        return filter_table(tab, float(seeing), pix, rb=rb, rb_cut=cut), nfound

    def stamps(self, ra, dec, sci, ref, size=63, ref_flxscale=1.0, sci_flxscale=1.0, kernel='LANCZOS3', device_out=False):
        self.result()
        fs = self.engine.flux_scale(self.wsci, self.wref, float(sci_flxscale))
        self.engine.set_stream(self.stream.cuda_stream)
        self.stream.wait_stream(self.torch.cuda.current_stream(self.device))
        planes = [dict(img=self.diff, wcs=self.wsci, fscale=fs), dict(img=sci.contiguous(), wcs=self.wsci, fscale=fs),
                  dict(img=ref.contiguous(), wcs=self.wref, on_grid=True)]
        return self.engine.stamps(planes, self.wref, ra, dec, size=size, kernel=kernel, stream=self.stream,
                                  device_out=device_out)

    def release_overlap(self):
        if self._bk_engine is not None:
            self._bk_stream.synchronize()
            self._bk_engine.close()
        self._bk_engine = self._bk_stream = None

    def job(self, scim, sci_rms, p):
        return _lib.zm_sub_job(scim.data_ptr(), sci_rms.data_ptr(), self.ref_al.data_ptr(),
                               self.refrms_al.data_ptr(), self.bpm.data_ptr(), C.pointer(p),
                               self.diff.data_ptr(), self.noise.data_ptr())

    def finish(self):
        return self.diff, self.noise, self.submask

    def prepare(self, sci, sci_rms, sci_mask, sci_wgt, ref, ref_rms, ref_mask, seeing,
                nreg_side=3, subtract_back=True, hotpants_kws=None, ref_flxscale=1.0,
                ref_rms_flxscale=None, sci_ready=None):
        from .engine import hp_params
        from .hotpants import job_params
        L, ctx = self.engine.L, self.engine.ctx
        ny, nx = self.shape
        LAN = _lib.RESAMPLE['LANCZOS3']
        fs = C.c_double()
        check(L.zm_flux_scale(C.byref(self.wref), C.byref(self.wsci), float(ref_flxscale),
                              C.byref(fs)), 'zm_flux_scale')
        fs_rms = C.c_double()
        check(L.zm_flux_scale(C.byref(self.wref), C.byref(self.wsci),
                              float(ref_flxscale if ref_rms_flxscale is None else ref_rms_flxscale),
                              C.byref(fs_rms)), 'zm_flux_scale')
        self.engine.set_stream(self.stream.cuda_stream)
        self.stream.wait_stream(self.torch.cuda.current_stream(self.device))
        side = self.overlap and subtract_back
        bk_done = None
        if side:
            if self._bk_engine is None:
                from .engine import Engine
                self._bk_stream = self.torch.cuda.Stream(self.device)
                self._bk_engine = Engine(self.device.index, stream=self._bk_stream.cuda_stream)
            e2 = self._bk_engine
            if sci_ready is None:
                self._bk_stream.wait_stream(self.stream)
            else:
                if sci_ready is not False:
                    self._bk_stream.wait_event(sci_ready)
                if self._last_done is not None:
                    self._bk_stream.wait_event(self._last_done)
            with self.torch.cuda.stream(self._bk_stream):
                check(L.zm_background_dev(e2.ctx, sci.data_ptr(), sci_wgt.data_ptr() if sci_wgt is not None else None,
                                          nx, ny, 128, 3, None, None, self.scibkgsub.data_ptr(), None), 'sci background')
                check(L.zm_add_scalar_dev(e2.ctx, self.scibkgsub.data_ptr(), self.BKG_VAL, self.n), 'pedestal')
                bk_done = self._bk_stream.record_event()
        with self.torch.cuda.stream(self.stream):
            if sci_mask.dtype == self.torch.int16:
                if getattr(self, '_scimask32', None) is None:
                    self._scimask32 = self.torch.empty(self.shape, dtype=self.torch.int32, device=self.device)
                check(L.zm_mask_widen_dev(ctx, sci_mask.data_ptr(), self.n, self._scimask32.data_ptr()),
                      'zm_mask_widen_dev')
                sci_mask = self._scimask32
            pair = os.environ.get('ZM_ALIGN_PAIR', '1') != '0' and int(self.engine.query('edge')) == 0 and \
                int(self.engine.query('mask_resample')) == 0
            if pair:
                check(L.zm_align_pair_dev(ctx, ref.data_ptr(), ref_rms.data_ptr(), ref_mask.data_ptr(),
                                          C.byref(self.wref), C.byref(self.wsci), LAN, fs.value, fs_rms.value,
                                          self.ref_al.data_ptr(), self.refrms_al.data_ptr(),
                                          self.refmask_al.data_ptr()), 'align ref + rms')
            else:
                check(L.zm_resample_dev(ctx, ref.data_ptr(), None, ref_mask.data_ptr(),
                                        C.byref(self.wref), C.byref(self.wsci), LAN, fs.value,
                                        self.ref_al.data_ptr(), self.ref_al_w.data_ptr(),
                                        self.refmask_al.data_ptr()), 'align ref')
            check(L.zm_mask_bad_dev(ctx, self.refmask_al.data_ptr(), sci_mask.data_ptr(),
                                    self.BAD_SUM, self.n, self.submask.data_ptr(),
                                    self.bpm.data_ptr()), 'submask')
            if subtract_back and not side:
                check(L.zm_background_dev(ctx, sci.data_ptr(),
                                          sci_wgt.data_ptr() if sci_wgt is not None else None,
                                          nx, ny, 128, 3, None, None, self.scibkgsub.data_ptr(),
                                          None), 'sci background')
                check(L.zm_add_scalar_dev(ctx, self.scibkgsub.data_ptr(), self.BKG_VAL, self.n),
                      'pedestal')
                scim = self.scibkgsub
            elif subtract_back:
                self.stream.wait_event(bk_done)
                scim = self.scibkgsub
            else:
                scim = sci
            if not pair:
                check(L.zm_resample_dev(ctx, ref_rms.data_ptr(), None, None, C.byref(self.wref),
                                        C.byref(self.wsci), LAN, fs_rms.value, self.refrms_al.data_ptr(),
                                        self.refrms_al_w.data_ptr(), None), 'align ref rms')
            kws = dict(hotpants_kws or {})
            user_limits = 'il' in kws or 'tl' in kws
            if os.environ.get('ZM_HOST_LIMITS') == '1' or user_limits:
                mm = (C.c_double * 4)()
                check(L.zm_median_mad2_dev(ctx, scim.data_ptr(), sci_mask.data_ptr(),
                                           self.ref_al.data_ptr(), self.refmask_al.data_ptr(),
                                           self.n, mm), 'sci / ref bkg')
                m1, s1, m2, s2 = (float(v) for v in mm)
                self._limits = dict(il=m1 - 10 * s1, tl=m2 - 10 * s2)
                p = hp_params(**job_params(seeing, nx, ny, nreg_side, self._limits['il'],
                                           self._limits['tl'], hotpants_kws))
            else:
                if getattr(self, '_lim_dev', None) is None:
                    self._lim_dev = self.torch.zeros(6, dtype=self.torch.float64, device=self.device)
                check(L.zm_median_mad2_async_dev(ctx, scim.data_ptr(), sci_mask.data_ptr(),
                                                 self.ref_al.data_ptr(), self.refmask_al.data_ptr(),
                                                 self.n, self._lim_dev.data_ptr()), 'sci / ref bkg')
                if getattr(self, '_lim_host', None) is None:
                    self._lim_host = self.torch.zeros(6, dtype=self.torch.float64).pin_memory()
                self._lim_host.copy_(self._lim_dev, non_blocking=True)
                self._limits = None
                p = hp_params(**job_params(seeing, nx, ny, nreg_side, 0.0, 0.0, hotpants_kws))
                p.limits_dev = self._lim_dev.data_ptr()
                p.limits_nsigma = 10.0
        p.flag_mask_dev = self.submask.data_ptr()
        p.flag_bit = 1 << 17
        self._sci_rms = sci_rms
        return scim, p

    @property
    def limits(self):
        if getattr(self, '_limits', None) is None:
            self.stream.synchronize()
            self.check_limits()
            m1, s1, _, m2, s2, _ = (float(v) for v in self._lim_host)
            self._limits = dict(il=m1 - 10 * s1, tl=m2 - 10 * s2)
        return self._limits

    def check_limits(self):
        if getattr(self, '_limits', None) is None and getattr(self, '_lim_host', None) is not None:
            if not (float(self._lim_host[2]) > 0 and float(self._lim_host[5]) > 0):
                raise _lib.ZMError('zm_median_mad2: every pixel is masked')


_KIND = {'f32': 0, 'i32': 1, 'u8': 2, 'i16': 3}


class FITSDeviceIO(object):

    def __init__(self, device=0, engine=None, stream=None):
        torch = _torch()
        self.torch = torch
        self.device = torch.device('cuda', device)
        self.engine = engine or get_engine(device)
        if stream is None:
            stream = torch.cuda.Stream(self.device)
            self.engine.set_stream(stream.cuda_stream)
        self.stream = stream
        self._pin = [None, None]
        self._busy = [None, None]
        self._turn = 0

    def _staging(self, nbytes):
        torch = self.torch
        k = self._turn
        self._turn ^= 1
# ... 151 lines not shown
```

Baseline: 49080 Mpix/s.

## Fuse submask OR into pair resample, merge colany launches, flag in apply

The science-mask OR and bad-pixel-map computation is folded into the paired Lanczos resample kernel, so the separate mask_bad pass no longer runs. The two column-any dilation launches become one launch over a z dimension of two. The zero-value flag marking moves into the hotpants apply kernel, which removes the standalone flag kernel. Together these cut several full-frame memory passes and kernel launches in the subtraction stage. In exchange the resample and apply kernels carry more template variants and more arguments, and the old split path stays available behind an env var.

```diff
diff --git a/include/zudsmi.h b/include/zudsmi.h
--- a/include/zudsmi.h
+++ b/include/zudsmi.h
@@ -236,6 +236,10 @@
 int zm_align_pair_dev(zm_ctx* ctx, const float* img_a, const float* img_b, const int32_t* mask,
                       const zm_wcs* win, const zm_wcs* wout, int kernel, double fscale_a, double fscale_b,
                       float* out_a, float* out_b, int32_t* out_mask);
+int zm_align_pair_bad_dev(zm_ctx* ctx, const float* img_a, const float* img_b, const int32_t* mask,
+                          const zm_wcs* win, const zm_wcs* wout, int kernel, double fscale_a, double fscale_b,
+                          float* out_a, float* out_b, int32_t* out_mask, const void* sci_mask, int sci_mask_type,
+                          int32_t badsum, int32_t* out_or, uint8_t* out_bpm);
 int zm_resample_i16(zm_ctx* ctx, const float* img, const float* wgt,
                     const int16_t* mask, const zm_wcs* win, const zm_wcs* wout,
                     int kernel, double fscale, float* out_img, float* out_wgt,
diff --git a/zuds-pipeline_amd/_lib.py b/zuds-pipeline_amd/_lib.py
--- a/zuds-pipeline_amd/_lib.py
+++ b/zuds-pipeline_amd/_lib.py
@@ -167,6 +167,8 @@
                               _P, _P, _P]),
     'zm_align_pair_dev': (C.c_int, [_P, _P, _P, _P, C.POINTER(zm_wcs), C.POINTER(zm_wcs), C.c_int, C.c_double,
                                     C.c_double, _P, _P, _P]),
+    'zm_align_pair_bad_dev': (C.c_int, [_P, _P, _P, _P, C.POINTER(zm_wcs), C.POINTER(zm_wcs), C.c_int, C.c_double,
+                                        C.c_double, _P, _P, _P, _P, C.c_int, C.c_int32, _P, _P]),
     'zm_resample_dev': (C.c_int, [_P, _P, _P, _P, C.POINTER(zm_wcs),
                                   C.POINTER(zm_wcs), C.c_int, C.c_double,
                                   _P, _P, _P]),
@@ -271,13 +273,16 @@
     'zm_timing_read': (C.c_int, [_P, C.c_char_p, C.POINTER(C.c_double),
                                  C.POINTER(C.c_int64)]),
     'zm_debug_lanczos3': (None, [C.c_float, _P]),
+    'zm_hp_flag_standalone': (C.c_int, [C.c_int, C.c_int]),
+    'zm_debug_hp_apply_flag': (C.c_int, [_P, _P, _P, _P, _P, C.c_int, C.c_int, C.POINTER(zm_hp_params), _P, _P, C.c_int32,
+                                         _P, _P]),
 }
 
 _lib = None
 
 
 def exported_symbols():
-    return [k for k in _SIGS if k != 'zm_debug_lanczos3']
+    return [k for k in _SIGS if k not in ('zm_debug_lanczos3', 'zm_hp_flag_standalone', 'zm_debug_hp_apply_flag')]
 
 
 def _one_hip_runtime():
diff --git a/zuds-pipeline_amd/csrc/api_coadd.hip b/zuds-pipeline_amd/csrc/api_coadd.hip
--- a/zuds-pipeline_amd/csrc/api_coadd.hip
+++ b/zuds-pipeline_amd/csrc/api_coadd.hip
@@ -478,9 +478,9 @@
     return 0;
 }
 
-extern "C" int zm_align_pair_dev(zm_ctx* ctx, const float* img_a, const float* img_b, const int32_t* mask,
-                                 const zm_wcs* win, const zm_wcs* wout, int kernel, double fscale_a, double fscale_b,
-                                 float* out_a, float* out_b, int32_t* out_mask) {
+static int align_pair(zm_ctx* ctx, const float* img_a, const float* img_b, const int32_t* mask,
+                      const zm_wcs* win, const zm_wcs* wout, int kernel, double fscale_a, double fscale_b,
+                      float* out_a, float* out_b, int32_t* out_mask, const zm_rs_bad* bad) {
     ZM_CHECK(ctx && img_a && img_b && win && wout && out_a && out_b, "zm_align_pair_dev: null argument");
     ZM_CHECK(!mask || out_mask, "zm_align_pair_dev: out_mask required");
     ZM_CHECK(kernel == ZM_RESAMPLE_LANCZOS3 || kernel == ZM_RESAMPLE_BILINEAR, "zm_align_pair_dev: LANCZOS3 or BILINEAR (got %d)", kernel);
@@ -503,7 +503,21 @@
     ZM_TRY(ctx->get("prep", sizeof(float2) * (size_t)spitch * ny, (void**)&src));
     ZM_TRY(zm_launch_prep_pair(ctx, img_a, img_b, nx, ny, src, spitch));
     return zm_launch_resample(ctx, src, nx, ny, spitch, lat, lnx, lny, kernel, (float)fscale_a, nullptr, onx, ony, lds,
-                              mask, out_mask, mask ? 1 : 0, 0, 1, out_a, out_b, (float)fscale_b);
+                              mask, out_mask, mask ? 1 : 0, 0, 1, out_a, out_b, (float)fscale_b, bad);
+}
+extern "C" int zm_align_pair_dev(zm_ctx* ctx, const float* img_a, const float* img_b, const int32_t* mask,
+                                 const zm_wcs* win, const zm_wcs* wout, int kernel, double fscale_a, double fscale_b,
+                                 float* out_a, float* out_b, int32_t* out_mask) {
+    return align_pair(ctx, img_a, img_b, mask, win, wout, kernel, fscale_a, fscale_b, out_a, out_b, out_mask, nullptr);
+}
+extern "C" int zm_align_pair_bad_dev(zm_ctx* ctx, const float* img_a, const float* img_b, const int32_t* mask,
+                                     const zm_wcs* win, const zm_wcs* wout, int kernel, double fscale_a, double fscale_b,
+                                     float* out_a, float* out_b, int32_t* out_mask, const void* sci_mask,
+                                     int sci_mask_type, int32_t badsum, int32_t* out_or, uint8_t* out_bpm) {
+    ZM_CHECK(mask && out_mask && sci_mask && out_or && out_bpm, "zm_align_pair_bad_dev: null argument");
+    ZM_CHECK(sci_mask_type == ZM_MASKTYPE_I32 || sci_mask_type == ZM_MASKTYPE_I16, "zm_align_pair_bad_dev: unknown mask type %d", sci_mask_type);
+    const zm_rs_bad bad = {sci_mask, sci_mask_type, badsum, out_or, out_bpm};
+    return align_pair(ctx, img_a, img_b, mask, win, wout, kernel, fscale_a, fscale_b, out_a, out_b, out_mask, &bad);
 }
 
 extern "C" int zm_resample_i16_dev(zm_ctx* ctx, const float* img, const float* wgt, const int16_t* mask,
diff --git a/zuds-pipeline_amd/csrc/ctx.hip b/zuds-pipeline_amd/csrc/ctx.hip
--- a/zuds-pipeline_amd/csrc/ctx.hip
+++ b/zuds-pipeline_amd/csrc/ctx.hip
@@ -165,6 +165,7 @@
     else if (!strcmp(what, "dev_build")) *out = ZM_DEV_BUILD;
     else if (!strcmp(what, "edge")) *out = ctx->edge;
     else if (!strcmp(what, "mask_resample")) *out = ctx->mask_resample;
+    else if (!strcmp(what, "sub_passes_split")) *out = ctx->sub_split ? 1 : 0;
     else ZM_CHECK(false, "zm_ctx_query: unknown item \"%s\"", what);
     return 0;
 }
diff --git a/zuds-pipeline_amd/csrc/hotpants.hip b/zuds-pipeline_amd/csrc/hotpants.hip
--- a/zuds-pipeline_amd/csrc/hotpants.hip
+++ b/zuds-pipeline_amd/csrc/hotpants.hip
@@ -130,8 +130,12 @@
 }
 
 #define HP_COLSTRIP4 32
-__global__ __launch_bounds__(256) void k_hp_colany4(const uint8_t* __restrict__ in, int nx, int ny, int hw,
-                                                    int edge, uint8_t* __restrict__ out) {
+__global__ __launch_bounds__(256) void k_hp_colany4(const uint8_t* __restrict__ in0, int hw0, uint8_t* __restrict__ out0,
+                                                    const uint8_t* __restrict__ in1, int hw1, uint8_t* __restrict__ out1,
+                                                    int nx, int ny, int edge) {
+    const uint8_t* __restrict__ in = blockIdx.z ? in1 : in0;
+    uint8_t* __restrict__ out = blockIdx.z ? out1 : out0;
+    const int hw = blockIdx.z ? hw1 : hw0;
     const int x = (blockIdx.x * blockDim.x + threadIdx.x) * 4;
     const int y0 = blockIdx.y * HP_COLSTRIP4, y1 = min(y0 + HP_COLSTRIP4, ny);
     if (x >= nx) return;
@@ -2314,6 +2318,8 @@
     if (img[p] == value) mask[p] |= bit;
 }
 
+extern "C" int zm_hp_flag_standalone(int want_flag, int apply_has_mask) { return (want_flag && !apply_has_mask) ? 1 : 0; }
+
 extern "C" void zm_hp_params_default(zm_hp_params* p) {
     if (!p) return;
     memset(p, 0, sizeof(*p));
@@ -2477,9 +2483,11 @@
     if (!split && (((uintptr_t)tmp8b & 3) == 0)) {
         hipLaunchKernelGGL(k_hp_valid_rows, dim3(ny), b256, rsh, st, sci, ref, bpm, nx, ny, (float)P.il, (float)P.iu,
                            (float)P.tl, (float)P.tu, hp->limits_dev, hp->limits_nsigma, P.hw, P.hwk, bad, tmp8, tmp8b);
-        if (col4) {
-            hipLaunchKernelGGL(k_hp_colany4, gc4, b256, 0, st, tmp8, nx, ny, P.hw, 1, dirty);
-            hipLaunchKernelGGL(k_hp_colany4, gc4, b256, 0, st, tmp8b, nx, ny, P.hwk, 1, outbad);
+        if (col4 && !ctx->sub_split) {
+            hipLaunchKernelGGL(k_hp_colany4, dim3(gc4.x, gc4.y, 2), b256, 0, st, tmp8, P.hw, dirty, tmp8b, P.hwk, outbad, nx, ny, 1);
+        } else if (col4) {
+            hipLaunchKernelGGL(k_hp_colany4, gc4, b256, 0, st, tmp8, P.hw, dirty, nullptr, 0, nullptr, nx, ny, 1);
+            hipLaunchKernelGGL(k_hp_colany4, gc4, b256, 0, st, tmp8b, P.hwk, outbad, nullptr, 0, nullptr, nx, ny, 1);
         } else {
             hipLaunchKernelGGL(k_hp_colany, gc, b256, 0, st, tmp8, nx, ny, P.hw, 1, dirty);
             hipLaunchKernelGGL(k_hp_colany, gc, b256, 0, st, tmp8b, nx, ny, P.hwk, 1, outbad);
@@ -2488,10 +2496,10 @@
         hipLaunchKernelGGL(k_hp_valid, dim3((unsigned)((np + 255) / 256)), b256, 0, st, sci, ref, bpm, np,
                            (float)P.il, (float)P.iu, (float)P.tl, (float)P.tu, bad, hp->limits_dev, hp->limits_nsigma);
         hipLaunchKernelGGL(k_hp_rowany, dim3(ny), b256, rsh, st, bad, nx, ny, P.hw, tmp8);
-        if (col4) hipLaunchKernelGGL(k_hp_colany4, gc4, b256, 0, st, tmp8, nx, ny, P.hw, 1, dirty);
+        if (col4) hipLaunchKernelGGL(k_hp_colany4, gc4, b256, 0, st, tmp8, P.hw, dirty, nullptr, 0, nullptr, nx, ny, 1);
         else hipLaunchKernelGGL(k_hp_colany, gc, b256, 0, st, tmp8, nx, ny, P.hw, 1, dirty);
         hipLaunchKernelGGL(k_hp_rowany, dim3(ny), b256, rsh, st, bad, nx, ny, P.hwk, tmp8);
-        if (col4) hipLaunchKernelGGL(k_hp_colany4, gc4, b256, 0, st, tmp8, nx, ny, P.hwk, 1, outbad);
+        if (col4) hipLaunchKernelGGL(k_hp_colany4, gc4, b256, 0, st, tmp8, P.hwk, outbad, nullptr, 0, nullptr, nx, ny, 1);
         else hipLaunchKernelGGL(k_hp_colany, gc, b256, 0, st, tmp8, nx, ny, P.hwk, 1, outbad);
     }
     ZM_HIP(hipGetLastError());
@@ -2904,16 +2912,18 @@
         tmo_seen = tmo_seen || (flag & HP_RFLAG_TMO);
         if ((flag & ~HP_RFLAG_TMO) == 0 || tmo_seen) break;
     }
+    const bool flag_in_apply = hp->flag_mask_dev != nullptr && !ctx->sub_split;
     {
         zm_scope_timer t(ctx, "hp_apply");
         unsigned long long* smask = nullptr;
         ZM_TRY(ctx->get("hp_smask", sizeof(unsigned long long), (void**)&smask));
         hipLaunchKernelGGL(k_hp_solved, dim3(1), dim3(64), 0, st, P.nreg, P.nunk, stats, fail, tmo, rhs, smask, x0sum);
         {
-            ZM_TRY(zm_hp_launch_apply(ctx, P, smask, sci, ref, sci_rms, ref_rms, outbad, d_filt, rhs, out_diff, out_rms, nmasked));
-        }
-    }
-    if (hp->flag_mask_dev) {
+            ZM_TRY(zm_hp_launch_apply(ctx, P, smask, sci, ref, sci_rms, ref_rms, outbad, d_filt, rhs, out_diff, out_rms, nmasked,
+                                      flag_in_apply ? hp->flag_mask_dev : nullptr, hp->flag_bit, 1e-30f, tmo));
+        }
+    }
+    if (zm_hp_flag_standalone(hp->flag_mask_dev != nullptr, flag_in_apply)) {
         hipLaunchKernelGGL(k_hp_flag, dim3((unsigned)((np + 255) / 256)), b256, 0, st, hp->flag_mask_dev, out_diff, 1e-30f,
                            hp->flag_bit, np, tmo, P.nreg);
         ZM_HIP(hipGetLastError());
@@ -2966,6 +2976,36 @@
     for (int reg = 0; reg < ctx->hp_pend_nreg; ++reg)
         ZM_CHECK(h_int[3 * HP_MAXREG + 4 + reg] == 0, "zm_subtract_info: a barrier time-out went unnoticed (region %d)", reg);
     hp_fill_info(h_sum, ctx->hp_pend_nreg, ctx->hp_pend_nunk, ctx->hp_pend_rounds, ctx->hp_pend_retries, info);
+    return 0;
+}
+
+extern "C" int zm_debug_hp_apply_flag(zm_ctx* ctx, const float* sci, const float* sci_rms, const float* ref,
+                                      const float* ref_rms, int nx, int ny, const zm_hp_params* hp, const int* tmo_dev,
+                                      int32_t* mask_dev, int32_t bit, float* out_diff, float* out_rms) {
+    ZM_CHECK(ctx && sci && sci_rms && ref && ref_rms && hp && tmo_dev && mask_dev && out_diff && out_rms && nx > 0 && ny > 0,
+             "zm_debug_hp_apply_flag: bad argument");
+    ZM_HIP(hipSetDevice(ctx->device));
+    hp_plan P;
+    std::vector<double> filt, basis;
+    ZM_TRY(make_plan(hp, nx, ny, &P, &filt, &basis));
+    const size_t np = (size_t)nx * ny;
+    hipStream_t st = ctx->stream;
+    uint8_t* outbad = nullptr;
+    double *d_filt = nullptr, *xsol = nullptr;
+    char* words = nullptr;
+    ZM_TRY(ctx->get("dbg_outbad", np, (void**)&outbad));
+    ZM_TRY(ctx->get("dbg_filt", sizeof(double) * filt.size(), (void**)&d_filt));
+    ZM_TRY(ctx->get("dbg_xsol", sizeof(double) * (size_t)P.nreg * P.nunk, (void**)&xsol));
+    ZM_TRY(ctx->get("dbg_words", 16, (void**)&words));
+    ZM_HIP(hipStreamSynchronize(st));
+    ZM_HIP(hipMemcpy(d_filt, filt.data(), sizeof(double) * filt.size(), hipMemcpyHostToDevice));
+    ZM_HIP(hipMemsetAsync(outbad, 0, np, st));
+    ZM_HIP(hipMemsetAsync(xsol, 0, sizeof(double) * (size_t)P.nreg * P.nunk, st));
+    ZM_HIP(hipMemsetAsync(words, 0, 16, st));
+    ZM_TRY(zm_hp_launch_apply(ctx, P, reinterpret_cast<const unsigned long long*>(words), sci, ref, sci_rms, ref_rms, outbad,
+                              d_filt, xsol, out_diff, out_rms, reinterpret_cast<int*>(words + 8), mask_dev, bit, 1e-30f,
+                              tmo_dev));
+    ZM_HIP(hipStreamSynchronize(st));
     return 0;
 }
 
diff --git a/zuds-pipeline_amd/csrc/hp_apply.hip b/zuds-pipeline_amd/csrc/hp_apply.hip
--- a/zuds-pipeline_amd/csrc/hp_apply.hip
+++ b/zuds-pipeline_amd/csrc/hp_apply.hip
@@ -58,7 +58,9 @@
                                                   const double* __restrict__ xsol,
                                                   float* __restrict__ diff,
                                                   float* __restrict__ noise,
-                                                  int* __restrict__ nmasked) {
+                                                  int* __restrict__ nmasked,
+                                                  int32_t* __restrict__ fmask, int32_t fbit, float fval,
+                                                  const int* __restrict__ tmo) {
     const int reg = blockIdx.z;
     const int solved = (int)((*solved_mask >> reg) & 1ull);
     typedef apply_cfg<HWK> C;
@@ -217,6 +219,11 @@
             if (strip * R + q < STEP) tTV[row * OW + ox0 + q] = acc2[q];
     }
     __syncthreads();
+    if (fmask) {
+        int gaveup = 0;
+        for (int r = 0; r < P.nreg; ++r) gaveup |= tmo[r];
+        if (gaveup) fmask = nullptr;
+    }
     int masked = 0;
     {
         constexpr int NE = (STEP * OW + 255) / 256;
@@ -261,6 +268,7 @@
             }
             diff[idx] = d;
             noise[idx] = nz;
+            if (fmask && d == fval) fmask[idx] |= fbit;
         }
     }
 #pragma unroll
@@ -382,7 +390,9 @@
                                                     const float2* __restrict__ kcg, int maxbx, int maxby,
                                                     float* __restrict__ diff,
                                                     float* __restrict__ noise,
-                                                    int* __restrict__ nmasked) {
+                                                    int* __restrict__ nmasked,
+                                                    int32_t* __restrict__ fmask, int32_t fbit, float fval,
+                                                    const int* __restrict__ tmo) {
     const int reg = blockIdx.z;
     const int solved = (int)((*solved_mask >> reg) & 1ull);
     typedef applyw_cfg<HWK> C;
@@ -462,6 +472,11 @@
             if (strip * R + q < STEP) tTV[row * OW + ox0 + q] = acc2[q];
     }
     __syncthreads();
+    if (fmask) {
+        int gaveup = 0;
+        for (int r = 0; r < P.nreg; ++r) gaveup |= tmo[r];
+        if (gaveup) fmask = nullptr;
+    }
     int masked = 0;
     {
         constexpr int NE = (STEP * OW + 255) / 256;
@@ -506,6 +521,7 @@
             }
             diff[idx] = d;
             noise[idx] = nz;
+            if (fmask && d == fval) fmask[idx] |= fbit;
         }
     }
 #pragma unroll
@@ -522,7 +538,7 @@
 static int launch_apply(zm_ctx* ctx, const hp_plan& P, const unsigned long long* solved_mask, const float* sci,
                         const float* ref, const float* srms, const float* trms, const uint8_t* outbad,
                         const double* filt, const double* xsol, float* diff, float* noise,
-                        int* nmasked) {
+                        int* nmasked, int32_t* fmask, int32_t fbit, float fval, const int* tmo) {
     typedef apply_cfg<HWK> C;
     constexpr int STEP = C::STEP, NB = C::NB;
     constexpr int TP = C::TP, TH = STEP + 2 * HWK;
@@ -560,13 +576,14 @@
             wset[HWK][ctx->device & 63] = true;
         }
         hipLaunchKernelGGL(k_hp_apply_w<HWK>, dim3(zm_div_up(maxbx, CW::NBW), maxby, P.nreg), dim3(256), wsh, ctx->stream,
-                           P, solved_mask, sci, ref, srms, trms, outbad, xsol, kcg, maxbx, maxby, diff, noise, nmasked);
+                           P, solved_mask, sci, ref, srms, trms, outbad, xsol, kcg, maxbx, maxby, diff, noise, nmasked, fmask, fbit, fval,
+                           tmo);
         ZM_HIP(hipGetLastError());
         return 0;
     }
     dim3 grd(zm_div_up(zm_div_up(W, STEP), NB), zm_div_up(H, STEP), P.nreg);
     hipLaunchKernelGGL(k_hp_apply<HWK>, grd, dim3(256), shmem, ctx->stream, P, solved_mask, sci, ref, srms,
-                       trms, outbad, filt, xsol, diff, noise, nmasked);
+                       trms, outbad, filt, xsol, diff, noise, nmasked, fmask, fbit, fval, tmo);
     ZM_HIP(hipGetLastError());
     return 0;
 }
@@ -574,8 +591,10 @@
 
 int zm_hp_launch_apply(zm_ctx* ctx, const hp_plan& P, const unsigned long long* solved_mask, const float* sci,
                        const float* ref, const float* srms, const float* trms, const uint8_t* outbad,
-                       const double* filt, const double* xsol, float* diff, float* noise, int* nmasked) {
-#define C(H) case H: return launch_apply<H>(ctx, P, solved_mask, sci, ref, srms, trms, outbad, filt, xsol, diff, noise, nmasked);
+                       const double* filt, const double* xsol, float* diff, float* noise, int* nmasked,
+                       int32_t* fmask, int32_t fbit, float fval, const int* tmo) {
+    ZM_CHECK(!fmask || tmo, "zm_hp_launch_apply: a mask to flag needs the give-up words of the fit");
+#define C(H) case H: return launch_apply<H>(ctx, P, solved_mask, sci, ref, srms, trms, outbad, filt, xsol, diff, noise, nmasked, fmask, fbit, fval, tmo);
     switch (P.hwk) {
         C(1) C(2) C(3) C(4) C(5) C(6) C(7) C(8) C(9) C(10) C(11) C(12) C(13) C(14) C(15) C(16) C(17) C(18) C(19) C(20)
         default: zm_set_error("zm_subtract: unsupported kernel half width %d", P.hwk); return 2;
diff --git a/zuds-pipeline_amd/csrc/hp_dev.h b/zuds-pipeline_amd/csrc/hp_dev.h
--- a/zuds-pipeline_amd/csrc/hp_dev.h
+++ b/zuds-pipeline_amd/csrc/hp_dev.h
@@ -109,4 +109,5 @@
                            const hp_job* d_tab, const double* filt, int round);
 int zm_hp_launch_apply(zm_ctx* ctx, const hp_plan& P, const unsigned long long* solved_mask, const float* sci,
                        const float* ref, const float* srms, const float* trms, const uint8_t* outbad,
-                       const double* filt, const double* xsol, float* diff, float* noise, int* nmasked);
+                       const double* filt, const double* xsol, float* diff, float* noise, int* nmasked,
+                       int32_t* fmask = nullptr, int32_t fbit = 0, float fval = 0.f, const int* tmo = nullptr);
diff --git a/zuds-pipeline_amd/csrc/resample.hip b/zuds-pipeline_amd/csrc/resample.hip
--- a/zuds-pipeline_amd/csrc/resample.hip
+++ b/zuds-pipeline_amd/csrc/resample.hip
@@ -283,13 +283,16 @@
     return 0;
 }
 
-template <int KIND, int MASKOP>
+template <int KIND, int MASKOP, int SCI = 0>
 __global__ __launch_bounds__(256, 4) void k_resample(
     const float2* __restrict__ src, int nx, int ny, int spitch, const double2* __restrict__ lat,
     int lnx, int lny, float fscale, float2* __restrict__ dst, int onx, int ony, int lds_cap,
     const int32_t* __restrict__ mask, const uint16_t* __restrict__ mbox, int32_t* __restrict__ macc,
     int mkind, int mfirst, int ntx, int ntiles, const float* __restrict__ taptab,
-    float* __restrict__ plane_a, float* __restrict__ plane_b, float pair_scale) {
+    float* __restrict__ plane_a, float* __restrict__ plane_b, float pair_scale,
+    const void* __restrict__ sci_mask = nullptr, int32_t badsum = 0, int32_t* __restrict__ out_or = nullptr,
+    uint8_t* __restrict__ out_bpm = nullptr) {
+    static_assert(SCI == 0 || MASKOP == 1, "the science mask joins the stage that stores the aligned mask");
     extern __shared__ float4 smem4[];
     rs_hdr* HR = reinterpret_cast<rs_hdr*>(smem4);
     constexpr int TABF = (KIND == ZM_RESAMPLE_LANCZOS3) ? LZ_FLOATS : 0;
@@ -389,6 +392,9 @@
             const int ty = tyb + 4 * q;
             const int oy = oy0 + ty;
             if (ox >= onx || oy >= ony) continue;
+            int32_t scim = 0;
+            if (SCI == 1) scim = static_cast<const int32_t*>(sci_mask)[(size_t)oy * onx + ox];
+            if (SCI == 2) scim = static_cast<const int16_t*>(sci_mask)[(size_t)oy * onx + ox];
             const int cr = q >> 2;
             const float fy = (float)(ty & 15) * (1.f / LSTEP);
             const float xa = cr ? xr[1] : xr[0], xb = cr ? xr[2] : xr[1];
@@ -552,6 +558,11 @@
             }
             if (MASKOP == 1) {
                 macc[oidx] = mres;
+                if (SCI) {
+                    const int32_t m = mres | scim;
+                    out_or[oidx] = m;
+                    out_bpm[oidx] = (m & badsum) != 0;
+                }
             } else if (MASKOP == 2) {
                 int32_t a = aprev[0];
 #pragma unroll
@@ -604,7 +615,7 @@
                                 int spitch, const double2* lat, int lnx, int lny, float fscale,
                                 float2* dst, int onx, int ony, int lds_elems, const int32_t* mask,
                                 int32_t* macc, int mop, int mkind, int mfirst, float* plane_a, float* plane_b,
-                                float pair_scale) {
+                                float pair_scale, const zm_rs_bad* bad) {
     dim3 blk(256, 1, 1);
     const int ntx = grd.x, ntiles = grd.x * grd.y;
     uint16_t* mbox = nullptr;
@@ -628,6 +639,14 @@
     if (mop == 0)
         hipLaunchKernelGGL((k_resample<KIND, 0>), pgrd, blk, shmem, ctx->stream, src, nx, ny, spitch, lat,
                            lnx, lny, fscale, dst, onx, ony, lds_elems, mask, mbox, macc, mkind, mfirst, ntx, ntiles, taptab, plane_a, plane_b, pair_scale);
+    else if (mop == 1 && bad && bad->type == ZM_MASKTYPE_I16)
+        hipLaunchKernelGGL((k_resample<KIND, 1, 2>), pgrd, blk, shmem, ctx->stream, src, nx, ny, spitch, lat,
+                           lnx, lny, fscale, dst, onx, ony, lds_elems, mask, mbox, macc, mkind, mfirst, ntx, ntiles, taptab, plane_a, plane_b, pair_scale,
+                           bad->sci, bad->badsum, bad->out_or, bad->out_bpm);
+    else if (mop == 1 && bad)
+        hipLaunchKernelGGL((k_resample<KIND, 1, 1>), pgrd, blk, shmem, ctx->stream, src, nx, ny, spitch, lat,
+                           lnx, lny, fscale, dst, onx, ony, lds_elems, mask, mbox, macc, mkind, mfirst, ntx, ntiles, taptab, plane_a, plane_b, pair_scale,
+                           bad->sci, bad->badsum, bad->out_or, bad->out_bpm);
     else if (mop == 1)
         hipLaunchKernelGGL((k_resample<KIND, 1>), pgrd, blk, shmem, ctx->stream, src, nx, ny, spitch, lat,
                            lnx, lny, fscale, dst, onx, ony, lds_elems, mask, mbox, macc, mkind, mfirst, ntx, ntiles, taptab, plane_a, plane_b, pair_scale);
@@ -641,8 +660,13 @@
 int zm_launch_resample(zm_ctx* ctx, const float2* src, int nx, int ny, int spitch,
                        const double2* lat, int lnx, int lny, int kernel, float fscale,
                        float2* dst, int onx, int ony, int lds_elems, const int32_t* mask,
-                       int32_t* macc, int mop, int mkind, int mfirst, float* plane_a, float* plane_b, float pair_scale) {
+                       int32_t* macc, int mop, int mkind, int mfirst, float* plane_a, float* plane_b, float pair_scale,
+                       const zm_rs_bad* bad) {
     dim3 blk(256, 1, 1), grd(zm_div_up(onx, TW), zm_div_up(ony, TH), 1);
+    ZM_CHECK(!bad || (mask && macc && mop == 1 && kernel != ZM_RESAMPLE_NEAREST && ctx->edge == ZM_EDGE_ZERO &&
+                      ctx->mask_resample == ZM_MASKRES_OR && bad->sci && bad->out_or && bad->out_bpm &&
+                      (bad->type == ZM_MASKTYPE_I32 || bad->type == ZM_MASKTYPE_I16)),
+             "zm_launch_resample: the OR with a science mask joins a stored, OR-resampled mask under the default conventions");
     ZM_CHECK(pair_scale == 0.f || (kernel != ZM_RESAMPLE_NEAREST && plane_a && plane_b && ctx->edge == ZM_EDGE_ZERO && mop != 2),
              "zm_launch_resample: a pair of images takes LANCZOS3 / BILINEAR, two output planes, the default edge rule and no mask accumulation");
     dim3 rgrd(zm_div_up(onx, TW), zm_div_up(ony, RTH), 1);
@@ -655,11 +679,11 @@
         if (kernel == ZM_RESAMPLE_LANCZOS3)
             ZM_TRY(launch_resample_kind<ZM_RESAMPLE_LANCZOS3>(ctx, rgrd, shmem, src, nx, ny, spitch, lat, lnx,
                                                               lny, fscale, dst, onx, ony, lds_elems, mask,
-                                                              macc, mop_img, mkind, mfirst, plane_a, plane_b, pair_scale));
+                                                              macc, mop_img, mkind, mfirst, plane_a, plane_b, pair_scale, bad));
         else
             ZM_TRY(launch_resample_kind<ZM_RESAMPLE_BILINEAR>(ctx, rgrd, shmem, src, nx, ny, spitch, lat, lnx,
                                                               lny, fscale, dst, onx, ony, lds_elems, mask,
-                                                              macc, mop_img, mkind, mfirst, plane_a, plane_b, pair_scale));
+                                                              macc, mop_img, mkind, mfirst, plane_a, plane_b, pair_scale, bad));
         if (trunc)
             ZM_TRY(zm_launch_resample_rim(ctx, src, nx, ny, spitch, lat, lnx, lny, kernel, fscale, dst, plane_a, plane_b, onx,
                                           ony, mask, macc, mop_img, mkind));
diff --git a/zuds-pipeline_amd/csrc/zm_internal.h b/zuds-pipeline_amd/csrc/zm_internal.h
--- a/zuds-pipeline_amd/csrc/zm_internal.h
+++ b/zuds-pipeline_amd/csrc/zm_internal.h
@@ -2,6 +2,7 @@
 #include <hip/hip_runtime.h>
 #include <cstdint>
 #include <cstdio>
+#include <cstdlib>
 #include <cstring>
 #include <map>
 #include <string>
@@ -54,8 +55,14 @@
     std::vector<std::pair<hipEvent_t, hipEvent_t>> pending;
 };
 
+static inline bool zm_env_sub_split() {
+    const char* e = getenv("ZM_SUB_PASSES");
+    return e && !strcmp(e, "split");
+}
+
 struct zm_ctx {
     int device = 0;
+    const bool sub_split = zm_env_sub_split();
     hipStream_t stream = nullptr;
     bool own_stream = true;
     std::map<std::string, std::pair<void*, size_t>> scratch;
@@ -189,11 +196,19 @@
 int zm_get_sync_events(zm_ctx* ctx, int n, hipEvent_t** out);
 hipStream_t zm_ctx_aux(zm_ctx* ctx);
 int zm_launch_var_scale(zm_ctx* ctx, const float* bstats, const float* vstats, float* out);
+struct zm_rs_bad {
+    const void* sci;
+    int type;
+    int32_t badsum;
+    int32_t* out_or;
+    uint8_t* out_bpm;
+};
 int zm_launch_resample(zm_ctx* ctx, const float2* src, int nx, int ny, int spitch,
                        const double2* lat, int lnx, int lny, int kernel, float fscale,
                        float2* dst, int onx, int ony, int lds_elems, const int32_t* mask,
                        int32_t* macc, int mop, int mkind, int mfirst,
-                       float* plane_a = nullptr, float* plane_b = nullptr, float pair_scale = 0.f);
+                       float* plane_a = nullptr, float* plane_b = nullptr, float pair_scale = 0.f,
+                       const zm_rs_bad* bad = nullptr);
 int zm_launch_prep_pair(zm_ctx* ctx, const float* a, const float* b, int nx, int ny, float2* dst, int spitch);
 int zm_launch_resample_mask(zm_ctx* ctx, const int32_t* mask, int nx, int ny,
                             const double2* lat, int lnx, int lny, int kernel,
diff --git a/zuds-pipeline_amd/device.py b/zuds-pipeline_amd/device.py
--- a/zuds-pipeline_amd/device.py
+++ b/zuds-pipeline_amd/device.py
@@ -289,6 +289,7 @@
                 check(L.zm_add_scalar_dev(e2.ctx, self.scibkgsub.data_ptr(), self.BKG_VAL, self.n), 'pedestal')
                 bk_done = self._bk_stream.record_event()
         with self.torch.cuda.stream(self.stream):
+            sci_mask_stored = sci_mask
             if sci_mask.dtype == self.torch.int16:
                 if getattr(self, '_scimask32', None) is None:
                     self._scimask32 = self.torch.empty(self.shape, dtype=self.torch.int32, device=self.device)
@@ -297,7 +298,15 @@
                 sci_mask = self._scimask32
             pair = os.environ.get('ZM_ALIGN_PAIR', '1') != '0' and int(self.engine.query('edge')) == 0 and \
                 int(self.engine.query('mask_resample')) == 0
-            if pair:
+            fused_bad = pair and not int(self.engine.query('sub_passes_split'))
+            if fused_bad:
+                check(L.zm_align_pair_bad_dev(ctx, ref.data_ptr(), ref_rms.data_ptr(), ref_mask.data_ptr(),
+                                              C.byref(self.wref), C.byref(self.wsci), LAN, fs.value, fs_rms.value,
+                                              self.ref_al.data_ptr(), self.refrms_al.data_ptr(),
+                                              self.refmask_al.data_ptr(), sci_mask_stored.data_ptr(),
+                                              1 if sci_mask_stored.dtype == self.torch.int16 else 0, self.BAD_SUM,
+                                              self.submask.data_ptr(), self.bpm.data_ptr()), 'align ref + rms + submask')
+            elif pair:
                 check(L.zm_align_pair_dev(ctx, ref.data_ptr(), ref_rms.data_ptr(), ref_mask.data_ptr(),
                                           C.byref(self.wref), C.byref(self.wsci), LAN, fs.value, fs_rms.value,
                                           self.ref_al.data_ptr(), self.refrms_al.data_ptr(),
@@ -307,9 +316,10 @@
                                         C.byref(self.wref), C.byref(self.wsci), LAN, fs.value,
                                         self.ref_al.data_ptr(), self.ref_al_w.data_ptr(),
                                         self.refmask_al.data_ptr()), 'align ref')
-            check(L.zm_mask_bad_dev(ctx, self.refmask_al.data_ptr(), sci_mask.data_ptr(),
-                                    self.BAD_SUM, self.n, self.submask.data_ptr(),
-                                    self.bpm.data_ptr()), 'submask')
+            if not fused_bad:
+                check(L.zm_mask_bad_dev(ctx, self.refmask_al.data_ptr(), sci_mask.data_ptr(),
+                                        self.BAD_SUM, self.n, self.submask.data_ptr(),
+                                        self.bpm.data_ptr()), 'submask')
             if subtract_back and not side:
                 check(L.zm_background_dev(ctx, sci.data_ptr(),
                                           sci_wgt.data_ptr() if sci_wgt is not None else None,
```

After: 49180 Mpix/s, median of 3. No clear change (+0.2%).
